# robotseu/ORB_Line_SLAM

Hardware: AMD Instinct MI355X
Metric: stereo frames/s extract+match (ORB+LBD), KITTI 1242x375 (higher is better)
Workload: dtype u8; 1 GPU; C3: 1242x375 stereo, 2000 ORB + 500 LBD per image, extract + stereo point/line match + f2f LBD match + SearchByBoW vs the previous frame (synthetic k=10 L=6 vocabulary, ComputeBoW included); parallelism=frame-sharded x1, distinct_pairs=512, order=shuffled, scene=default

## Files before the change

include/orbline.h:

```cpp
#ifndef ORBLINE_H
#define ORBLINE_H

#include "orbline_types.h"

#ifdef __cplusplus
extern "C" {
#endif

typedef struct olf_ctx olf_ctx;

const char* olf_last_error(void);
int olf_device_count(void);
int olf_default_params(olf_params* p);

int  olf_ctx_create(const olf_params* p, int width, int height, int max_images, olf_ctx** out);
void olf_ctx_destroy(olf_ctx* ctx);
int  olf_ctx_synchronize(olf_ctx* ctx);
int  olf_ctx_set_input_event(olf_ctx* ctx, void* hip_event);
int  olf_ctx_set_deferred_join(olf_ctx* ctx, int on);
int  olf_stereo_frames_join_dev(olf_ctx* ctx, void* stream);
int  olf_ctx_poll_status(olf_ctx* ctx);

int olf_profile_enable(olf_ctx* ctx, int on);
int olf_profile_reset(olf_ctx* ctx);
int olf_profile_stage_count(void);
const char* olf_profile_stage_name(int stage);
int olf_profile_read(olf_ctx* ctx, double* total_ms, int32_t* calls);

enum { OLF_RGB2GRAY = 0, OLF_BGR2GRAY = 1, OLF_RGBA2GRAY = 2, OLF_BGRA2GRAY = 3 };
int olf_cvt_gray_dev(olf_ctx* ctx, const uint8_t* d_src, int code, int n_images, uint8_t* d_gray, void* stream);
int olf_remap_linear_dev(olf_ctx* ctx, const uint8_t* d_src, int src_w, int src_h, const float* d_mapx, const float* d_mapy, int dst_w,
                         int dst_h, int n_images, uint8_t* d_dst, void* stream);
int olf_init_undistort_rectify_map_dev(olf_ctx* ctx, const double* K, const double* D, int n_dist, const double* R, const double* P, int w, int h,
                                       float* d_map1, float* d_map2, void* stream);
int olf_init_undistort_rectify_map(olf_ctx* ctx, const double* K, const double* D, int n_dist, const double* R, const double* P, int w, int h,
                                   float* map1, float* map2);
int olf_cvt_gray(olf_ctx* ctx, const uint8_t* src, int code, int n_images, uint8_t* gray);
int olf_remap_linear(olf_ctx* ctx, const uint8_t* src, int src_w, int src_h, const float* mapx, const float* mapy, int dst_w, int dst_h,
                     int n_images, uint8_t* dst);

int olf_distinctive_descriptors(olf_ctx* ctx, const uint8_t* desc, const int32_t* offs, int n_points, int32_t* best);

size_t olf_kf_record_bytes(int n_keys, int n_lines);
int olf_kf_record_pack(uint64_t frame_id, uint64_t kf_id, double timestamp, const float* t3, const float* quat4, int n_keys,
                       const olf_keypoint* keys, const float* uright, const float* depth, const uint8_t* desc, const uint64_t* mappoint_ids,
                       int n_lines, const olf_keyline* lines, const float* disparity2, const double* le3, const uint8_t* ldesc,
                       const uint64_t* mapline_ids, uint8_t* out, size_t capacity, size_t* written);
int olf_kf_record_counts(const uint8_t* buf, size_t len, int32_t* n_keys, int32_t* n_lines, size_t* record_bytes);
int olf_kf_record_unpack(const uint8_t* buf, size_t len, uint64_t* frame_id, uint64_t* kf_id, double* timestamp, float* t3, float* quat4,
                         olf_keypoint* keys, float* uright, float* depth, uint8_t* desc, uint64_t* mappoint_ids, olf_keyline* lines,
                         float* disparity2, double* le3, uint8_t* ldesc, uint64_t* mapline_ids);

typedef struct olf_voc olf_voc;
int olf_voc_create(int k, int L, int scoring, int weighting, int n_nodes, const int32_t* parent, const uint8_t* is_leaf, const uint8_t* desc,
                   const double* weight, olf_voc** out);
int olf_voc_load_text(const char* path, olf_voc** out);
void olf_voc_destroy(olf_voc* voc);
int olf_voc_info(const olf_voc* voc, int* k, int* L, int* scoring, int* weighting, int* n_nodes, int* n_words);
int olf_bow_words_dev(olf_ctx* ctx, const olf_voc* voc, const uint8_t* d_desc, int n, int levelsup, int32_t* d_word, double* d_weight,
                      int32_t* d_node, void* stream);
int olf_bow_assemble(const olf_voc* voc, const int32_t* word, const double* weight, const int32_t* node, int n, int32_t* bow_ids,
                     double* bow_vals, int* n_bow, int32_t* fv_nodes, int32_t* fv_offs, int32_t* fv_idx, int* n_fv);
int olf_bow_transform(olf_ctx* ctx, const olf_voc* voc, const uint8_t* desc, int n, int levelsup, int32_t* bow_ids, double* bow_vals,
                      int* n_bow, int32_t* fv_nodes, int32_t* fv_offs, int32_t* fv_idx, int* n_fv);
int olf_search_by_bow_batch_dev(olf_ctx* ctx, const olf_voc* voc, int n_frames, int img_stride, const olf_keypoint* d_kps, const uint8_t* d_desc,
                                const int32_t* d_counts, const uint8_t* d_mp_valid, const uint8_t* d_mp_bad, float nnratio, int check_orientation,
                                int levelsup, int32_t* d_matches, int32_t* d_nmatches, void* stream);

int olf_orb_scale_tables(const olf_ctx* ctx, float* scale, float* inv_scale, float* sigma2, float* inv_sigma2,
                         int32_t* features_per_level);
int olf_orb_level_sizes(const olf_ctx* ctx, int32_t* widths, int32_t* heights);
int olf_orb_capacity(const olf_ctx* ctx);
int olf_orb_extract_strided(olf_ctx* ctx, const uint8_t* image, size_t row_stride, olf_keypoint* kps, uint8_t* desc, int32_t* count);
int olf_orb_extract_dev(olf_ctx* ctx, const uint8_t* d_images, int n_images, olf_keypoint* d_kps, uint8_t* d_desc,
                        int32_t* d_counts, void* stream);
int olf_orb_extract(olf_ctx* ctx, const uint8_t* images, int n_images, olf_keypoint* kps, uint8_t* desc, int32_t* counts);
int olf_orb_pyramid_level(olf_ctx* ctx, int image, int level, int blurred, uint8_t* dst);
int olf_orb_debug_candidates(olf_ctx* ctx, int image, int level, int32_t* xys, int cap, int32_t* count);
int olf_debug_status(olf_ctx* ctx, int32_t* out64);
int olf_debug_status_n(olf_ctx* ctx, int32_t* out, int n);
int olf_debug_lsd_owner(olf_ctx* ctx, int image, uint32_t* out);
int olf_debug_lsd_regions(olf_ctx* ctx, int image, int32_t* start_n, double* angle, int cap, int32_t* count);
int olf_debug_lsd_waves(olf_ctx* ctx, int waves_per_image, int rob_entries);
int olf_debug_lsd_groups(olf_ctx* ctx, int groups);
int olf_debug_lsd_scatter(olf_ctx* ctx, int on);
int olf_debug_lsd_log_cap(olf_ctx* ctx, int entries);
int olf_debug_seed_sort(olf_ctx* ctx, const uint32_t* keys, int n, int kthr, int depth_limit, uint32_t* out, int32_t* out_n);
int olf_debug_seed_sort_mode(olf_ctx* ctx, int mode);
int olf_debug_seed_sort_wide(olf_ctx* ctx, const uint64_t* keys, int n, int64_t kthr, int depth_limit, int full, uint32_t* out, int32_t* out_n);
int olf_debug_lsd_pool(olf_ctx* ctx, int pool_chunks);
int olf_debug_fdiv_sweep(olf_ctx* ctx, uint64_t seed, int blocks, int per_thread, uint64_t* mismatches);
int olf_debug_sqrtq_sweep(olf_ctx* ctx, int count, uint64_t* mismatches);
int olf_debug_align_sweep(olf_ctx* ctx, uint64_t seed, int blocks, int per_thread, uint64_t* out3);

int olf_stereo_points_dev(olf_ctx* ctx, int n_pairs, const olf_keypoint* d_kps, const uint8_t* d_desc, const int32_t* d_counts,
                          float* d_uright, float* d_depth, void* stream);
int olf_stereo_points(olf_ctx* ctx, const uint8_t* images, int n_pairs, olf_keypoint* kps, uint8_t* desc, int32_t* counts,
                      float* uright, float* depth);

int olf_match_bf_dev(olf_ctx* ctx, const uint8_t* d_descA, const int32_t* d_nA, int strideA, int a_step, const uint8_t* d_descB,
                     const int32_t* d_nB, int strideB, int b_step, int n_sets, float nnr, int best_lr, int32_t* d_m12, void* stream);
int olf_match_bf(olf_ctx* ctx, const uint8_t* descA, int nA, const uint8_t* descB, int nB, float nnr, int best_lr, int32_t* m12);
int olf_knn2(olf_ctx* ctx, const uint8_t* descQ, int nQ, const uint8_t* descT, int nT, int32_t* idx0, int32_t* dist0, int32_t* dist1);
int olf_match_candidates_dev(olf_ctx* ctx, const uint8_t* d_descQ, int nQ, const uint8_t* d_descT, int nT, const int32_t* d_cand_offsets,
                             const int32_t* d_cand_idx, uint16_t* d_dist, void* stream);
int olf_match_candidates(olf_ctx* ctx, const uint8_t* descQ, int nQ, const uint8_t* descT, int nT, const int32_t* cand_offsets,
                         const int32_t* cand_idx, uint16_t* dist);
typedef struct olf_frame_view {
    const olf_keypoint* keys;
    const uint8_t* desc;
    const float*   uright;
    int32_t        n;
    uint8_t*       mp_valid;
    uint8_t*       mp_obs;
    const uint8_t* mp_bad;
    const float*   mp_world;
    const uint8_t* mp_desc;
    const uint8_t* outlier;
    const float*   Tcw;
    float fx, fy, cx, cy, mbf, minX, maxX, minY, maxY;
    const float*   scale_factors;
    int32_t        n_levels;
    const float*   mp_maxd;
    const float*   mp_mind;
    const int32_t* fv_nodes;
    const int32_t* fv_offsets;
    const int32_t* fv_features;
    int32_t        fv_n;
    const int32_t* grid_offsets;
    const int32_t* grid_index;
} olf_frame_view;
int olf_search_by_projection(olf_ctx* ctx, const olf_frame_view* cur, const olf_frame_view* last, float th, int bMono, int check_orientation,
                             int32_t* matches, int32_t* nmatches);
int olf_search_by_projection_match12(olf_ctx* ctx, const olf_frame_view* cur, const olf_frame_view* last, float th, int bMono, int check_orientation,
                                     int32_t* matches, int32_t* match12, int32_t* nmatches);
int olf_search_for_initialization(olf_ctx* ctx, const olf_frame_view* f1, const olf_frame_view* f2, float* prev_matched, int window_size,
                                  float nnratio, int check_orientation, int32_t* matches12, int32_t* nmatches);
int olf_search_by_bow(olf_ctx* ctx, const olf_frame_view* kf, const olf_frame_view* f, float nnratio, int check_orientation, int32_t* matched,
                      int32_t* nmatches);
int olf_search_local_map(olf_ctx* ctx, const olf_frame_view* f, int n_mp, const uint8_t* track_in_view, const uint8_t* bad,
                         const int32_t* track_scale_level, const float* track_view_cos, const float* track_proj3, const uint8_t* mp_desc,
                         const uint8_t* mp_obs, float th, float nnratio, int32_t* matches, int32_t* nmatches);

int olf_is_in_frustum(const olf_frame_view* f, int n_mp, const float* world, const float* normal, const float* maxd, const float* mind,
                      float viewing_cos_limit, uint8_t* track_in_view, int32_t* track_scale_level, float* track_view_cos, float* track_proj3);

int olf_search_by_projection_kf(olf_ctx* ctx, const olf_frame_view* cur, const olf_frame_view* kf, const uint8_t* already_found, float th,
                                int orb_dist, int check_orientation, int32_t* matches, int32_t* nmatches);
int olf_search_by_bow_kf(olf_ctx* ctx, const olf_frame_view* kf1, const olf_frame_view* kf2, float nnratio, int check_orientation,
                         int32_t* matches12, int32_t* nmatches);
int olf_search_for_triangulation(olf_ctx* ctx, const olf_frame_view* kf1, const olf_frame_view* kf2, const float* F12, const float* Cw,
                                 int only_stereo, int check_orientation, int32_t* matches12, int32_t* nmatches);
int olf_fuse_search(olf_ctx* ctx, const olf_frame_view* kf, int n_mp, const uint8_t* skip, const float* world, const float* normal,
                    const float* maxd, const float* mind, const uint8_t* desc, float th, const float* Ow, int32_t* best_idx, int32_t* best_dist);
int olf_fuse_search_sim3(olf_ctx* ctx, const olf_frame_view* kf, const float* Scw, int n_mp, const uint8_t* skip, const float* world,
                         const float* normal, const float* maxd, const float* mind, const uint8_t* desc, float th, int32_t* best_idx,
                         int32_t* best_dist);
int olf_search_by_projection_sim3(olf_ctx* ctx, const olf_frame_view* kf, const float* Scw, int n_mp, const uint8_t* skip, const float* world,
                                  const float* normal, const float* maxd, const float* mind, const uint8_t* desc, float th, uint8_t* matched,
                                  int32_t* matches, int32_t* nmatches);
int olf_search_by_sim3(olf_ctx* ctx, const olf_frame_view* kf1, const olf_frame_view* kf2, int32_t* matches12, float s12, const float* R12,
                       const float* t12, float th, int32_t* vn_match1, int32_t* vn_match2, int32_t* nfound);

int olf_hamming_matrix(olf_ctx* ctx, const uint8_t* descA, int nA, const uint8_t* descB, int nB, uint16_t* out);

int olf_line_capacity(const olf_ctx* ctx);
int olf_line_extract_strided(olf_ctx* ctx, const uint8_t* image, size_t row_stride, olf_keyline* kls, uint8_t* ldesc, int32_t* lcount);
int olf_line_extract_dev(olf_ctx* ctx, const uint8_t* d_images, int n_images, olf_keyline* d_kls, uint8_t* d_ldesc, int32_t* d_lcounts,
                         void* stream);
int olf_line_extract(olf_ctx* ctx, const uint8_t* images, int n_images, olf_keyline* kls, uint8_t* ldesc, int32_t* lcounts);
int olf_lbd_compute(olf_ctx* ctx, const uint8_t* images, int n_images, const olf_keyline* kls, const int32_t* lcounts, uint8_t* ldesc);
int olf_lsd_debug_scaled(olf_ctx* ctx, int image, uint8_t* dst, int32_t* ws, int32_t* hs);

int olf_stereo_lines_dev(olf_ctx* ctx, int n_pairs, const olf_keyline* d_kls, const uint8_t* d_ldesc, const int32_t* d_lcounts,
                         int32_t* d_matches12, float* d_disp, double* d_le, void* stream);
int olf_stereo_lines(olf_ctx* ctx, int n_pairs, const olf_keyline* kls, const uint8_t* ldesc, const int32_t* lcounts, int32_t* matches12,
                     float* disp, double* le);

typedef struct olf_frame_buffers {
    olf_keypoint* kps;
    uint8_t*  desc;
    int32_t*  counts;
    float*    uright;
    float*    depth;
    olf_keyline* kls;
    uint8_t*  ldesc;
    int32_t*  lcounts;
    int32_t*  lmatches12;
    float*    ldisp;
    double*   lle;
} olf_frame_buffers;
int olf_stereo_frames_dev(olf_ctx* ctx, const uint8_t* d_images, int n_pairs, const olf_frame_buffers* out, void* stream);
int olf_stereo_frames(olf_ctx* ctx, const uint8_t* images, int n_pairs, const olf_frame_buffers* out);

int olf_frame_grid_dev(olf_ctx* ctx, int n_frames, int img_stride, const olf_keypoint* d_kps, const int32_t* d_counts, float minX, float maxX,
                       float minY, float maxY, int32_t* d_cell_offsets, int32_t* d_cell_index, void* stream);
int olf_frame_grid(olf_ctx* ctx, const olf_keypoint* keys, int n, float minX, float maxX, float minY, float maxY, int32_t* cell_offsets,
                   int32_t* cell_index);
int olf_features_in_area_dev(olf_ctx* ctx, const olf_keypoint* d_keys, const int32_t* d_cell_offsets, const int32_t* d_cell_index, float minX, float maxX,
                             float minY, float maxY, int n_queries, const olf_area_query* d_queries, int32_t* d_cand_offsets, int32_t* d_cand_idx,
                             int cand_capacity, void* stream);
int olf_features_in_area(olf_ctx* ctx, const olf_keypoint* keys, int n_keys, const int32_t* cell_offsets, const int32_t* cell_index, float minX,
                         float maxX, float minY, float maxY, int n_queries, const olf_area_query* queries, int32_t* cand_offsets, int32_t* cand_idx,
                         int cand_capacity);
int olf_ctx_device_buffers(const olf_ctx* ctx, olf_frame_buffers* out);

int olf_line_coords(double x1, double y1, double x2, double y2, int32_t* xy, int cap, int32_t* n);

size_t olf_frames_pack_bound(const olf_ctx* ctx, int n_pairs);
int olf_frames_pack_dev(olf_ctx* ctx, const olf_frame_buffers* out, int n_pairs, uint8_t* d_dst, size_t dst_capacity, uint64_t* d_bytes, void* stream);
int olf_stereo_points_mask_dev(olf_ctx* ctx, const float* d_depth, size_t n, uint8_t* d_mask, void* stream);

typedef struct olf_track_batch {
    const olf_keypoint* kps; const uint8_t* desc; const int32_t* counts; int32_t img_stride;
    const float*   uright;
    const int32_t* cell_offsets;
    const int32_t* cell_index;
    const float*   Tcw;
    const float*   mp_world;
    const uint8_t* mp_valid;
    const uint8_t* mp_obs;
    const uint8_t* outlier;
    const uint8_t* mp_desc;
    float fx, fy, cx, cy, mbf, minX, maxX, minY, maxY;
} olf_track_batch;
int olf_search_by_projection_batch_dev(olf_ctx* ctx, const olf_track_batch* in, int n_frames, float th, const float* d_th, int bMono,
                                       int check_orientation, int32_t* d_matches, int32_t* d_match12, int32_t* d_nmatches, void* stream);
int olf_unproject_stereo_dev(olf_ctx* ctx, int n_frames, int img_stride, const olf_keypoint* d_kps, const int32_t* d_counts, const float* d_depth,
                             float fx, float fy, float cx, float cy, const float* d_Twc, float* d_world, void* stream);

typedef struct olf_local_map {
    const float*   world;
    const float*   normal;
    const float*   maxd;
    const float*   mind;
    const uint8_t* desc;
    const uint8_t* obs;
    const uint8_t* bad;
    int32_t        n_mp;
    const int32_t* list_offsets;
    const int32_t* list_index;
    int32_t        n_entries;
} olf_local_map;
int olf_predict_scale_thresholds(const float* scale_factors, int n_levels, float* thr);
int olf_is_in_frustum_batch_dev(olf_ctx* ctx, const olf_track_batch* in, int n_frames, const olf_local_map* map, const int32_t* d_frame_mp,
                                float viewing_cos_limit, uint8_t* d_in_view, int32_t* d_level, float* d_view_cos, float* d_proj3, void* stream);
int olf_search_local_map_batch_dev(olf_ctx* ctx, const olf_track_batch* in, int n_frames, const olf_local_map* map, const int32_t* d_frame_mp,
                                   float viewing_cos_limit, float th, const float* d_th, float nnratio, int32_t* d_matches, int32_t* d_nmatches,
                                   void* stream);

int olf_search_for_triangulation_batch_dev(olf_ctx* ctx, const olf_voc* voc, const olf_track_batch* in, int n_frames, int n_pairs,
                                           const int32_t* d_pairs, const float* d_F12, const float* d_Cw, int only_stereo, int check_orientation,
                                           int levelsup, int32_t* d_matches12, int32_t* d_nmatches, void* stream);

#define OLF_BOW_KF_FRAME 0
#define OLF_BOW_KF_KF    1
int olf_search_by_bow_pairs_dev(olf_ctx* ctx, const olf_voc* voc, const olf_track_batch* in, int n_frames, int n_pairs, const int32_t* d_pairs,
                                const uint8_t* d_mp_bad, int form, float nnratio, int check_orientation, int levelsup,
                                int32_t* d_matches, int32_t* d_nmatches, void* stream);

int olf_fuse_search_batch_dev(olf_ctx* ctx, const olf_track_batch* in, int n_frames, const olf_local_map* map, const int32_t* d_frame_mp,
                              const float* d_Scw, const float* d_Ow, float th, int32_t* d_best_idx, int32_t* d_best_dist, int32_t* d_nfused,
                              void* stream);

int olf_search_by_sim3_pairs_dev(olf_ctx* ctx, const olf_track_batch* in, int n_frames, const uint8_t* d_mp_bad, const float* d_mp_maxd,
                                 const float* d_mp_mind, int n_pairs, const int32_t* d_pairs, const float* d_s12, const float* d_R12, const float* d_t12,
                                 float th, int32_t* d_matches12, int32_t* d_vn_match1, int32_t* d_vn_match2, int32_t* d_nfound, void* stream);

int olf_is_in_frustum_l(const olf_frame_view* f, int n_ml, const float* world6, uint8_t* in_view, float* proj4);
int olf_local_lines_assign(int n_in_view, int32_t* m12, const int32_t* map_index, const float* proj4, const olf_keyline* kls, int n_lines, const float* ldisp,
                           float minX, float maxX, float minY, float maxY, int n_ml, const uint8_t* obs, int32_t* frame_ml, int32_t* n_inliers);
int olf_track_lines_assign(int n_last, int32_t* m12, const olf_keyline* kls_last, const int32_t* last_ml, int n_cur, const olf_keyline* kls_cur,
                           const float* ldisp_cur, float minX, float maxX, float minY, float maxY, int skip_null, int gates, double delta_angle, double pos_frac,
                           int32_t* cur_ml, int32_t* n_inliers);

typedef struct olf_line_batch {
    const olf_keyline* kls; const uint8_t* ldesc; const int32_t* lcounts; int32_t img_stride;
    const float*   ldisp;
    const float*   Tcw;
    float fx, fy, cx, cy, minX, maxX, minY, maxY;
} olf_line_batch;
typedef struct olf_local_line_map {
    const float*   world;
    const uint8_t* desc;
    const uint8_t* obs;
    const uint8_t* bad;
    int32_t        n_ml;
    const int32_t* list_offsets;
    const int32_t* list_index;
    int32_t        n_entries;
} olf_local_line_map;
int olf_is_in_frustum_l_batch_dev(olf_ctx* ctx, const olf_line_batch* in, int n_frames, const olf_local_line_map* map, const int32_t* d_frame_ml,
                                  uint8_t* d_in_view, float* d_proj4, void* stream);
int olf_search_local_lines_batch_dev(olf_ctx* ctx, const olf_line_batch* in, int n_frames, const olf_local_line_map* map, const int32_t* d_frame_ml, float nnr,
                                     uint8_t* d_in_view, float* d_proj4, int32_t* d_m12, int32_t* d_frame_ml_out, int32_t* d_ninliers, void* stream);
int olf_track_lines_batch_dev(olf_ctx* ctx, const olf_line_batch* in, int n_frames, const int32_t* d_last_ml, float nnr, int best_lr, int skip_null, int gates,
                              double delta_angle, double pos_frac, const int32_t* d_enable, int32_t* d_m12, int32_t* d_cur_ml, int32_t* d_ninliers, void* stream);

int olf_debug_copy_bandwidth(olf_ctx* ctx, size_t bytes, int reps, double* gbytes_per_s);

#ifdef __cplusplus
}
#endif
#endif
```

orb_line_slam_amd/_lib.py:

```python
import ctypes as C
import os
import numpy as np

_HERE = os.path.dirname(os.path.abspath(__file__))
LIB_PATH = os.environ.get("OLF_LIB_PATH", os.path.join(_HERE, "csrc", "liborbline_hip.so"))
SYNTH_PATH = os.path.join(_HERE, "csrc", "libolf_synth.so")

OLF_OK, OLF_ERR_INVALID, OLF_ERR_CAPACITY, OLF_ERR_HIP, OLF_ERR_NODEVICE = 0, -1, -2, -3, -4
DESC_BYTES = 32

KEYPOINT_DTYPE = np.dtype([("x", "<f4"), ("y", "<f4"), ("size", "<f4"), ("angle", "<f4"), ("response", "<f4"),
                           ("octave", "<i4"), ("class_id", "<i4")])
KEYLINE_DTYPE = np.dtype([("angle", "<f4"), ("class_id", "<i4"), ("octave", "<i4"), ("pt_x", "<f4"), ("pt_y", "<f4"),
                          ("response", "<f4"), ("size", "<f4"), ("startPointX", "<f4"), ("startPointY", "<f4"),
                          ("endPointX", "<f4"), ("endPointY", "<f4"), ("sPointInOctaveX", "<f4"),
                          ("sPointInOctaveY", "<f4"), ("ePointInOctaveX", "<f4"), ("ePointInOctaveY", "<f4"),
                          ("lineLength", "<f4"), ("numOfPixels", "<i4")])
assert KEYPOINT_DTYPE.itemsize == 28 and KEYLINE_DTYPE.itemsize == 68


class OrbParams(C.Structure):
    _fields_ = [("nfeatures", C.c_int32), ("scale_factor", C.c_float), ("nlevels", C.c_int32),
                ("ini_th_fast", C.c_int32), ("min_th_fast", C.c_int32), ("conv_gauss_sum256", C.c_int32)]


class LineParams(C.Structure):
    _fields_ = [("lsd_nfeatures", C.c_int32), ("min_line_length", C.c_double), ("lsd_refine", C.c_int32),
                ("lsd_scale", C.c_double), ("lsd_sigma_scale", C.c_double), ("lsd_quant", C.c_double),
                ("lsd_ang_th", C.c_double), ("lsd_log_eps", C.c_double), ("lsd_density_th", C.c_double),
                ("lsd_n_bins", C.c_int32), ("conv_gauss_sum256", C.c_int32), ("conv_resize_exact", C.c_int32), ("conv_seed_order", C.c_int32),
                ("conv_libm_float", C.c_int32)]


class StereoParams(C.Structure):
    _fields_ = [("fx", C.c_float), ("bf", C.c_float), ("matching_s_ws", C.c_int32), ("line_sim_th", C.c_double),
                ("min_ratio_12_l", C.c_double), ("min_disp", C.c_double), ("line_horiz_th", C.c_double),
                ("stereo_overlap_th", C.c_double), ("ls_min_disp_ratio", C.c_double), ("best_lr_matches", C.c_int32),
                ("conv_eigen_recip", C.c_int32)]


class OlfParams(C.Structure):
    _fields_ = [("abi_version", C.c_uint32), ("struct_size", C.c_uint32), ("orb", OrbParams), ("line", LineParams), ("stereo", StereoParams)]


class FrameBuffers(C.Structure):
    _fields_ = [(n, C.c_void_p) for n in ("kps", "desc", "counts", "uright", "depth", "kls", "ldesc", "lcounts", "lmatches12",
                                          "ldisp", "lle")]


class FrameViewC(C.Structure):
    _fields_ = ([(n, C.c_void_p) for n in ("keys", "desc", "uright")] + [("n", C.c_int32)] +
                [(n, C.c_void_p) for n in ("mp_valid", "mp_obs", "mp_bad", "mp_world", "mp_desc", "outlier", "Tcw")] +
                [(n, C.c_float) for n in ("fx", "fy", "cx", "cy", "mbf", "minX", "maxX", "minY", "maxY")] +
                [("scale_factors", C.c_void_p), ("n_levels", C.c_int32)] +
                [(n, C.c_void_p) for n in ("mp_maxd", "mp_mind", "fv_nodes", "fv_offsets", "fv_features")] + [("fv_n", C.c_int32)] +
                [(n, C.c_void_p) for n in ("grid_offsets", "grid_index")])


class TrackBatchC(C.Structure):
    _fields_ = ([(n, C.c_void_p) for n in ("kps", "desc", "counts")] + [("img_stride", C.c_int32)] +
                [(n, C.c_void_p) for n in ("uright", "cell_offsets", "cell_index", "Tcw", "mp_world", "mp_valid", "mp_obs", "outlier", "mp_desc")] +
                [(n, C.c_float) for n in ("fx", "fy", "cx", "cy", "mbf", "minX", "maxX", "minY", "maxY")])


class LocalMapC(C.Structure):
    _fields_ = ([(n, C.c_void_p) for n in ("world", "normal", "maxd", "mind", "desc", "obs", "bad")] + [("n_mp", C.c_int32)] +
                [(n, C.c_void_p) for n in ("list_offsets", "list_index")] + [("n_entries", C.c_int32)])


class LineBatchC(C.Structure):
    _fields_ = ([(n, C.c_void_p) for n in ("kls", "ldesc", "lcounts")] + [("img_stride", C.c_int32)] + [(n, C.c_void_p) for n in ("ldisp", "Tcw")] +
                [(n, C.c_float) for n in ("fx", "fy", "cx", "cy", "minX", "maxX", "minY", "maxY")])


class LocalLineMapC(C.Structure):
    _fields_ = ([(n, C.c_void_p) for n in ("world", "desc", "obs", "bad")] + [("n_ml", C.c_int32)] +
                [(n, C.c_void_p) for n in ("list_offsets", "list_index")] + [("n_entries", C.c_int32)])


GRID_COLS, GRID_ROWS, GRID_CELLS, GRID_MAX_KEYS = 64, 48, 3072, 8192
AREA_QUERY_DTYPE = np.dtype([("x", "<f4"), ("y", "<f4"), ("r", "<f4"), ("min_level", "<i4"), ("max_level", "<i4")])
assert AREA_QUERY_DTYPE.itemsize == 20


class OlfError(RuntimeError):
    def __init__(self, code, where):
        self.code = code
        super().__init__(f"{where}: status {code}: {last_error()}")


_lib = None


def _torch_runtime_first():
    import importlib.util
    if os.environ.get("OLF_NO_TORCH") or importlib.util.find_spec("torch") is None:
        return
    try:
        import torch
        if torch.cuda.is_available():
            torch.cuda.init()
    except Exception:
        pass


def lib():
    global _lib
    if _lib is None:
        if not os.path.exists(LIB_PATH):
            raise ImportError(f"{LIB_PATH} is missing: build it with `make -C orb_line_slam_amd/csrc` "
                              "(python -c 'import __graft_entry__ as g; g.build()'). There is no CPU fallback.")
        _torch_runtime_first()
        L = C.CDLL(LIB_PATH)
        L.olf_last_error.restype = C.c_char_p
        L.olf_ctx_create.argtypes = [C.POINTER(OlfParams), C.c_int, C.c_int, C.c_int, C.POINTER(C.c_void_p)]
        L.olf_ctx_destroy.argtypes = [C.c_void_p]
        L.olf_ctx_destroy.restype = None
        L.olf_ctx_synchronize.argtypes = [C.c_void_p]
        L.olf_ctx_poll_status.argtypes = [C.c_void_p]
        L.olf_orb_scale_tables.argtypes = [C.c_void_p] + [C.c_void_p] * 5
        L.olf_orb_level_sizes.argtypes = [C.c_void_p, C.c_void_p, C.c_void_p]
        L.olf_orb_capacity.argtypes = [C.c_void_p]
        L.olf_orb_extract_dev.argtypes = [C.c_void_p, C.c_void_p, C.c_int, C.c_void_p, C.c_void_p, C.c_void_p, C.c_void_p]
        L.olf_orb_extract.argtypes = [C.c_void_p, C.c_void_p, C.c_int, C.c_void_p, C.c_void_p, C.c_void_p]
        L.olf_orb_pyramid_level.argtypes = [C.c_void_p, C.c_int, C.c_int, C.c_int, C.c_void_p]
        L.olf_orb_debug_candidates.argtypes = [C.c_void_p, C.c_int, C.c_int, C.c_void_p, C.c_int, C.c_void_p]
        L.olf_stereo_points_dev.argtypes = [C.c_void_p, C.c_int] + [C.c_void_p] * 6
        L.olf_stereo_points.argtypes = [C.c_void_p, C.c_void_p, C.c_int] + [C.c_void_p] * 5
        L.olf_match_bf_dev.argtypes = [C.c_void_p, C.c_void_p, C.c_void_p, C.c_int, C.c_int, C.c_void_p, C.c_void_p, C.c_int, C.c_int,
                                       C.c_int, C.c_float, C.c_int, C.c_void_p, C.c_void_p]
        L.olf_match_bf.argtypes = [C.c_void_p, C.c_void_p, C.c_int, C.c_void_p, C.c_int, C.c_float, C.c_int, C.c_void_p]
        L.olf_knn2.argtypes = [C.c_void_p, C.c_void_p, C.c_int, C.c_void_p, C.c_int, C.c_void_p, C.c_void_p, C.c_void_p]
        L.olf_hamming_matrix.argtypes = [C.c_void_p, C.c_void_p, C.c_int, C.c_void_p, C.c_int, C.c_void_p]
        L.olf_line_capacity.argtypes = [C.c_void_p]
        L.olf_line_extract_dev.argtypes = [C.c_void_p, C.c_void_p, C.c_int] + [C.c_void_p] * 4
        L.olf_line_extract.argtypes = [C.c_void_p, C.c_void_p, C.c_int] + [C.c_void_p] * 3
        L.olf_lbd_compute.argtypes = [C.c_void_p, C.c_void_p, C.c_int] + [C.c_void_p] * 3
        L.olf_lsd_debug_scaled.argtypes = [C.c_void_p, C.c_int] + [C.c_void_p] * 3
        L.olf_stereo_lines_dev.argtypes = [C.c_void_p, C.c_int] + [C.c_void_p] * 7
        L.olf_stereo_lines.argtypes = [C.c_void_p, C.c_int] + [C.c_void_p] * 6
        L.olf_stereo_frames_dev.argtypes = [C.c_void_p, C.c_void_p, C.c_int, C.POINTER(FrameBuffers), C.c_void_p]
        L.olf_stereo_frames.argtypes = [C.c_void_p, C.c_void_p, C.c_int, C.POINTER(FrameBuffers)]
        L.olf_match_candidates.argtypes = [C.c_void_p, C.c_void_p, C.c_int, C.c_void_p, C.c_int, C.c_void_p, C.c_void_p, C.c_void_p]
        L.olf_search_by_projection.argtypes = [C.c_void_p, C.POINTER(FrameViewC), C.POINTER(FrameViewC), C.c_float, C.c_int, C.c_int, C.c_void_p, C.c_void_p]
        L.olf_search_by_projection_match12.argtypes = [C.c_void_p, C.POINTER(FrameViewC), C.POINTER(FrameViewC), C.c_float, C.c_int, C.c_int, C.c_void_p, C.c_void_p, C.c_void_p]
        L.olf_search_by_bow.argtypes = [C.c_void_p, C.POINTER(FrameViewC), C.POINTER(FrameViewC), C.c_float, C.c_int, C.c_void_p, C.c_void_p]
        L.olf_search_for_initialization.argtypes = [C.c_void_p, C.POINTER(FrameViewC), C.POINTER(FrameViewC), C.c_void_p, C.c_int, C.c_float, C.c_int,
                                                    C.c_void_p, C.c_void_p]
        V = C.POINTER(FrameViewC)
        L.olf_is_in_frustum.argtypes = [V, C.c_int, C.c_void_p, C.c_void_p, C.c_void_p, C.c_void_p, C.c_float] + [C.c_void_p] * 4
        L.olf_search_by_projection_kf.argtypes = [C.c_void_p, V, V, C.c_void_p, C.c_float, C.c_int, C.c_int, C.c_void_p, C.c_void_p]
        L.olf_search_by_bow_kf.argtypes = [C.c_void_p, V, V, C.c_float, C.c_int, C.c_void_p, C.c_void_p]
        L.olf_search_for_triangulation.argtypes = [C.c_void_p, V, V, C.c_void_p, C.c_void_p, C.c_int, C.c_int, C.c_void_p, C.c_void_p]
        L.olf_fuse_search.argtypes = [C.c_void_p, V, C.c_int] + [C.c_void_p] * 6 + [C.c_float, C.c_void_p, C.c_void_p, C.c_void_p]
        L.olf_fuse_search_sim3.argtypes = [C.c_void_p, V, C.c_void_p, C.c_int] + [C.c_void_p] * 6 + [C.c_float, C.c_void_p, C.c_void_p]
        L.olf_search_by_projection_sim3.argtypes = [C.c_void_p, V, C.c_void_p, C.c_int] + [C.c_void_p] * 6 + [C.c_float, C.c_void_p, C.c_void_p, C.c_void_p]
        L.olf_search_by_sim3.argtypes = [C.c_void_p, V, V, C.c_void_p, C.c_float, C.c_void_p, C.c_void_p, C.c_float, C.c_void_p, C.c_void_p, C.c_void_p]
        L.olf_search_local_map.argtypes = [C.c_void_p, C.POINTER(FrameViewC), C.c_int, C.c_void_p, C.c_void_p, C.c_void_p, C.c_void_p, C.c_void_p,
                                           C.c_void_p, C.c_void_p, C.c_float, C.c_float, C.c_void_p, C.c_void_p]
        L.olf_match_candidates_dev.argtypes = [C.c_void_p, C.c_void_p, C.c_int, C.c_void_p, C.c_int, C.c_void_p, C.c_void_p, C.c_void_p, C.c_void_p]
        L.olf_frame_grid_dev.argtypes = [C.c_void_p, C.c_int, C.c_int, C.c_void_p, C.c_void_p] + [C.c_float] * 4 + [C.c_void_p] * 3
        L.olf_frame_grid.argtypes = [C.c_void_p, C.c_void_p, C.c_int] + [C.c_float] * 4 + [C.c_void_p] * 2
        L.olf_features_in_area_dev.argtypes = ([C.c_void_p] * 4 + [C.c_float] * 4 + [C.c_int, C.c_void_p, C.c_void_p, C.c_void_p, C.c_int, C.c_void_p])
        L.olf_features_in_area.argtypes = ([C.c_void_p, C.c_void_p, C.c_int, C.c_void_p, C.c_void_p] + [C.c_float] * 4 +
                                           [C.c_int, C.c_void_p, C.c_void_p, C.c_void_p, C.c_int])
        L.olf_ctx_device_buffers.argtypes = [C.c_void_p, C.POINTER(FrameBuffers)]
        L.olf_cvt_gray.argtypes = [C.c_void_p, C.c_void_p, C.c_int, C.c_int, C.c_void_p]
        L.olf_remap_linear.argtypes = [C.c_void_p, C.c_void_p, C.c_int, C.c_int, C.c_void_p, C.c_void_p, C.c_int, C.c_int, C.c_int, C.c_void_p]
        L.olf_debug_lsd_waves.argtypes = [C.c_void_p, C.c_int, C.c_int]
        L.olf_debug_lsd_pool.argtypes = [C.c_void_p, C.c_int]
        L.olf_debug_lsd_groups.argtypes = [C.c_void_p, C.c_int]
        L.olf_debug_lsd_scatter.argtypes = [C.c_void_p, C.c_int]
        L.olf_debug_lsd_log_cap.argtypes = [C.c_void_p, C.c_int]
        L.olf_debug_seed_sort_mode.argtypes = [C.c_void_p, C.c_int]
        L.olf_debug_seed_sort.argtypes = [C.c_void_p, C.c_void_p, C.c_int, C.c_int, C.c_int, C.c_void_p, C.POINTER(C.c_int32)]
        L.olf_frames_pack_bound.argtypes = [C.c_void_p, C.c_int]
        L.olf_frames_pack_bound.restype = C.c_size_t
        L.olf_frames_pack_dev.argtypes = [C.c_void_p, C.POINTER(FrameBuffers), C.c_int, C.c_void_p, C.c_size_t, C.c_void_p, C.c_void_p]
        L.olf_ctx_set_input_event.argtypes = [C.c_void_p, C.c_void_p]
        L.olf_ctx_set_deferred_join.argtypes = [C.c_void_p, C.c_int]
        L.olf_stereo_frames_join_dev.argtypes = [C.c_void_p, C.c_void_p]
        L.olf_stereo_points_mask_dev.argtypes = [C.c_void_p, C.c_void_p, C.c_size_t, C.c_void_p, C.c_void_p]
        L.olf_search_by_projection_batch_dev.argtypes = [C.c_void_p, C.POINTER(TrackBatchC), C.c_int, C.c_float, C.c_void_p, C.c_int, C.c_int,
                                                         C.c_void_p, C.c_void_p, C.c_void_p, C.c_void_p]
        L.olf_unproject_stereo_dev.argtypes = [C.c_void_p, C.c_int, C.c_int, C.c_void_p, C.c_void_p, C.c_void_p] + [C.c_float] * 4 + [C.c_void_p] * 3
        L.olf_predict_scale_thresholds.argtypes = [C.c_void_p, C.c_int, C.c_void_p]
        L.olf_is_in_frustum_batch_dev.argtypes = [C.c_void_p, C.POINTER(TrackBatchC), C.c_int, C.POINTER(LocalMapC), C.c_void_p, C.c_float] + [C.c_void_p] * 5
        L.olf_search_local_map_batch_dev.argtypes = [C.c_void_p, C.POINTER(TrackBatchC), C.c_int, C.POINTER(LocalMapC), C.c_void_p, C.c_float, C.c_float,
                                                     C.c_void_p, C.c_float, C.c_void_p, C.c_void_p, C.c_void_p]
        L.olf_is_in_frustum_l.argtypes = [V, C.c_int, C.c_void_p, C.c_void_p, C.c_void_p]
        L.olf_local_lines_assign.argtypes = ([C.c_int, C.c_void_p, C.c_void_p, C.c_void_p, C.c_void_p, C.c_int, C.c_void_p] + [C.c_float] * 4 +
                                             [C.c_int, C.c_void_p, C.c_void_p, C.c_void_p])
        L.olf_track_lines_assign.argtypes = ([C.c_int, C.c_void_p, C.c_void_p, C.c_void_p, C.c_int, C.c_void_p, C.c_void_p] + [C.c_float] * 4 +
                                             [C.c_int, C.c_int, C.c_double, C.c_double, C.c_void_p, C.c_void_p])
        L.olf_is_in_frustum_l_batch_dev.argtypes = [C.c_void_p, C.POINTER(LineBatchC), C.c_int, C.POINTER(LocalLineMapC)] + [C.c_void_p] * 4
        L.olf_search_local_lines_batch_dev.argtypes = [C.c_void_p, C.POINTER(LineBatchC), C.c_int, C.POINTER(LocalLineMapC), C.c_void_p, C.c_float] + [C.c_void_p] * 6
        L.olf_track_lines_batch_dev.argtypes = ([C.c_void_p, C.POINTER(LineBatchC), C.c_int, C.c_void_p, C.c_float, C.c_int, C.c_int, C.c_int, C.c_double, C.c_double] +
                                                [C.c_void_p] * 5)
        L.olf_debug_copy_bandwidth.argtypes =[C.c_void_p, C.c_size_t, C.c_int, C.POINTER(C.c_double)]
        L.olf_debug_fdiv_sweep.argtypes = [C.c_void_p, C.c_uint64, C.c_int, C.c_int, C.POINTER(C.c_uint64)]
        L.olf_debug_sqrtq_sweep.argtypes = [C.c_void_p, C.c_int, C.POINTER(C.c_uint64)]
        L.olf_debug_align_sweep.argtypes = [C.c_void_p, C.c_uint64, C.c_int, C.c_int, C.POINTER(C.c_uint64)]
        L.olf_debug_seed_sort_wide.argtypes = [C.c_void_p, C.c_void_p, C.c_int, C.c_int64, C.c_int, C.c_int, C.c_void_p, C.POINTER(C.c_int32)]
        L.olf_distinctive_descriptors.argtypes = [C.c_void_p, C.c_void_p, C.c_void_p, C.c_int, C.c_void_p]
        L.olf_voc_create.argtypes = [C.c_int, C.c_int, C.c_int, C.c_int, C.c_int, C.c_void_p, C.c_void_p, C.c_void_p, C.c_void_p, C.POINTER(C.c_void_p)]
        L.olf_voc_load_text.argtypes = [C.c_char_p, C.POINTER(C.c_void_p)]
        L.olf_voc_destroy.argtypes = [C.c_void_p]
        L.olf_voc_destroy.restype = None
        L.olf_voc_info.argtypes = [C.c_void_p] + [C.POINTER(C.c_int)] * 6
        L.olf_bow_words_dev.argtypes = [C.c_void_p, C.c_void_p, C.c_void_p, C.c_int, C.c_int, C.c_void_p, C.c_void_p, C.c_void_p, C.c_void_p]
        L.olf_bow_assemble.argtypes = [C.c_void_p, C.c_void_p, C.c_void_p, C.c_void_p, C.c_int, C.c_void_p, C.c_void_p, C.POINTER(C.c_int), C.c_void_p,
                                       C.c_void_p, C.c_void_p, C.POINTER(C.c_int)]
        L.olf_search_by_bow_batch_dev.argtypes = [C.c_void_p, C.c_void_p, C.c_int, C.c_int, C.c_void_p, C.c_void_p, C.c_void_p, C.c_void_p, C.c_void_p, C.c_float, C.c_int, C.c_int, C.c_void_p, C.c_void_p, C.c_void_p]
        L.olf_search_for_triangulation_batch_dev.argtypes = ([C.c_void_p, C.c_void_p, C.POINTER(TrackBatchC), C.c_int, C.c_int] + [C.c_void_p] * 3 + [C.c_int] * 3 +
                                                             [C.c_void_p] * 3)
        L.olf_search_by_bow_pairs_dev.argtypes = ([C.c_void_p, C.c_void_p, C.POINTER(TrackBatchC), C.c_int, C.c_int, C.c_void_p, C.c_void_p, C.c_int, C.c_float,
                                                   C.c_int, C.c_int] + [C.c_void_p] * 3)
        L.olf_fuse_search_batch_dev.argtypes = ([C.c_void_p, C.POINTER(TrackBatchC), C.c_int, C.POINTER(LocalMapC)] + [C.c_void_p] * 3 + [C.c_float] +
                                                [C.c_void_p] * 4)
        L.olf_search_by_sim3_pairs_dev.argtypes = ([C.c_void_p, C.POINTER(TrackBatchC), C.c_int] + [C.c_void_p] * 3 + [C.c_int] + [C.c_void_p] * 4 + [C.c_float] +
                                                   [C.c_void_p] * 5)
        L.olf_bow_transform.argtypes = [C.c_void_p, C.c_void_p, C.c_void_p, C.c_int, C.c_int, C.c_void_p, C.c_void_p, C.POINTER(C.c_int), C.c_void_p,
                                        C.c_void_p, C.c_void_p, C.POINTER(C.c_int)]
        L.olf_profile_enable.argtypes = [C.c_void_p, C.c_int]
        L.olf_profile_reset.argtypes = [C.c_void_p]
        L.olf_profile_stage_name.restype = C.c_char_p
        L.olf_profile_stage_name.argtypes = [C.c_int]
        L.olf_profile_read.argtypes = [C.c_void_p, C.c_void_p, C.c_void_p]
        _lib = L
    return _lib


def last_error():
    return lib().olf_last_error().decode()


def device_count():
    return int(lib().olf_device_count())


def default_params():
    p = OlfParams()
    rc = lib().olf_default_params(C.byref(p))
    if rc != OLF_OK:
        raise OlfError(rc, "olf_default_params")
    return p


def check(rc, where):
    if rc != OLF_OK:
        raise OlfError(rc, where)


def ptr(a):
    if a is None:
        return None
    assert a.flags["C_CONTIGUOUS"]
    return a.ctypes.data_as(C.c_void_p)


class Context:

    def __init__(self, params, width, height, max_images):
        self.params, self.width, self.height, self.max_images = params, int(width), int(height), int(max_images)
        h = C.c_void_p()
        check(lib().olf_ctx_create(C.byref(params), self.width, self.height, self.max_images, C.byref(h)), "olf_ctx_create")
        self.handle = h
        self.nlevels = params.orb.nlevels
        self.orb_capacity = int(lib().olf_orb_capacity(self.handle))
        self.line_capacity = int(lib().olf_line_capacity(self.handle))

    def close(self):
        if getattr(self, "handle", None):
            lib().olf_ctx_destroy(self.handle)
            self.handle = None

    def __del__(self):
        try:
            self.close()
        except Exception:
            pass

    def profile(self, on=True):
        check(lib().olf_profile_enable(self.handle, int(on)), "olf_profile_enable")
        check(lib().olf_profile_reset(self.handle), "olf_profile_reset")

    def profile_read(self):
        n = lib().olf_profile_stage_count()
        ms = np.zeros(n, np.float64)
        calls = np.zeros(n, np.int32)
        check(lib().olf_profile_read(self.handle, ptr(ms), ptr(calls)), "olf_profile_read")
        return {lib().olf_profile_stage_name(i).decode(): (float(ms[i]), int(calls[i])) for i in range(n)}

    def synchronize(self):
        check(lib().olf_ctx_synchronize(self.handle), "olf_ctx_synchronize")

    def set_input_event(self, event):
        check(lib().olf_ctx_set_input_event(self.handle, C.c_void_p(event.cuda_event) if event is not None else None), "olf_ctx_set_input_event")

    def poll_status(self):
        check(lib().olf_ctx_poll_status(self.handle), "olf_ctx_poll_status")
```

orb_line_slam_amd/csrc/api_debug.cpp:

```cpp
#include "ctx.hpp"
#include "staging.hpp"

namespace olf {
int launch_copy16(const void* src, void* dst, size_t bytes, hipStream_t s);
}

using namespace olf;

static int sweep_counters(HostCall& h, unsigned long long** st, int n)
{
    h.add(st, n);
    OLF_TRY(h.bind(SCRATCH_STAGE));
    OLF_HIP_CHECK(hipMemsetAsync(*st, 0, (size_t)n * 8, h.stream()));
    return OLF_OK;
}

extern "C" {

int olf_orb_pyramid_level(olf_ctx* c, int image, int level, int blurred, uint8_t* dst)
{
    if (!c || !dst || image < 0 || image >= c->max_images || level < 0 || level >= c->orb.geom.nlevels) return OLF_ERR_INVALID;
    const LevelGeom& L = c->orb.geom.lv[level];
    const uint8_t* src = (blurred ? c->ob.blur : c->ob.pyr) + (size_t)image * c->orb.geom.pyrBytes + L.offset;
    OLF_HIP_CHECK(hipStreamSynchronize(c->stream));
    OLF_HIP_CHECK(hipMemcpy2D(dst, L.w, src, L.pitch, L.w, L.h, hipMemcpyDeviceToHost));
    return OLF_OK;
}

int olf_debug_status(olf_ctx* c, int32_t* out64)
{
    if (!c || !out64) return OLF_ERR_INVALID;
    OLF_HIP_CHECK(hipDeviceSynchronize());
    OLF_HIP_CHECK(hipMemcpy(out64, c->ob.status, 256, hipMemcpyDeviceToHost));
    return OLF_OK;
}

int olf_debug_copy_bandwidth(olf_ctx* c, size_t bytes, int reps, double* gbytes_per_s)
{
    if (!c || !gbytes_per_s || bytes < 16 || reps < 1) { set_error("olf_debug_copy_bandwidth: bad argument"); return OLF_ERR_INVALID; }
    OLF_TRY(check_device(c, "olf_debug_copy_bandwidth"));
    void *a = nullptr, *b = nullptr;
    OLF_HIP_CHECK(hipMalloc(&a, bytes));
    if (hipMalloc(&b, bytes) != hipSuccess) { (void)hipFree(a); set_error("olf_debug_copy_bandwidth: hipMalloc failed"); return OLF_ERR_HIP; }
    hipEvent_t e0, e1;
    (void)hipEventCreate(&e0); (void)hipEventCreate(&e1);
    (void)hipMemsetAsync(a, 1, bytes, c->stream);
    int rc = olf::launch_copy16(a, b, bytes, c->stream);
    (void)hipEventRecord(e0, c->stream);
    for (int i = 0; i < reps && rc == OLF_OK; ++i) rc = olf::launch_copy16(i & 1 ? b : a, i & 1 ? a : b, bytes, c->stream);
    (void)hipEventRecord(e1, c->stream);
    const hipError_t se = hipEventSynchronize(e1);
    float ms = 0.f;
    (void)hipEventElapsedTime(&ms, e0, e1);
    (void)hipEventDestroy(e0); (void)hipEventDestroy(e1); (void)hipFree(a); (void)hipFree(b);
    if (rc != OLF_OK || se != hipSuccess || !(ms > 0)) { set_error("olf_debug_copy_bandwidth: copy failed"); return OLF_ERR_HIP; }
    *gbytes_per_s = 2.0 * (double)(bytes / 16 * 16) * reps / (ms * 1e-3) / 1e9;
    return OLF_OK;
}

int olf_debug_lsd_waves(olf_ctx* c, int waves_per_image, int rob_entries)
{
    const bool pow2 = rob_entries > 0 && (rob_entries & (rob_entries - 1)) == 0;
    if (!c || waves_per_image > 16 || waves_per_image < -1 || (rob_entries != 0 && (!pow2 || rob_entries < 128 || rob_entries > 1024))) {
        set_error("olf_debug_lsd_waves: bad argument"); return OLF_ERR_INVALID;
    }
    c->lsd_force.waves = waves_per_image;
    c->lsd_force.robEntries = rob_entries;
    return OLF_OK;
}

int olf_debug_lsd_groups(olf_ctx* c, int groups)
{
    if (!c || !(groups == 0 || groups == 1 || groups == 2 || groups == 4)) { set_error("olf_debug_lsd_groups: bad argument"); return OLF_ERR_INVALID; }
    c->lsd_force.groups = groups > 0 ? groups : -1;
    return OLF_OK;
}

int olf_debug_lsd_log_cap(olf_ctx* c, int entries)
{
    if (!c || entries < 0) { set_error("olf_debug_lsd_log_cap: bad argument"); return OLF_ERR_INVALID; }
    OLF_TRY(check_device(c, "olf_debug_lsd_log_cap"));
    LineGeom& g = c->line.geom;
    if (entries > 0 && !g.spillArena) {
        const size_t blocks = std::max<size_t>(2, (size_t)c->max_images - (size_t)c->max_images / 4);
        void* q = nullptr;
        OLF_HIP_CHECK(hipMalloc(&q, blocks * 8 * (size_t)g.Ps));
        c->allocs.push_back(q);
        g.spillArena = static_cast<uint32_t*>(q); g.spillBlocks = (int)blocks;
    }
    g.logCap = entries > 0 ? std::min(entries, g.regionStride / 2) : g.regionStride / 2;
    OLF_HIP_CHECK(hipDeviceSynchronize());
    OLF_HIP_CHECK(hipMemcpy(c->lb.geom, &g, sizeof(LineGeom), hipMemcpyHostToDevice));
    return OLF_OK;
}

int olf_debug_lsd_scatter(olf_ctx* c, int on)
{
    if (!c) { set_error("olf_debug_lsd_scatter: bad argument"); return OLF_ERR_INVALID; }
    c->lsd_force.scatter = on ? 1 : 0;
    return OLF_OK;
}

int olf_debug_seed_sort(olf_ctx* c, const uint32_t* keys, int n, int kthr, int depth_limit, uint32_t* out, int32_t* out_n)
{
    if (!c || !keys || !out || !out_n || n < 0 || n > c->line.geom.Ps || kthr < 0 || kthr > 1023) { set_error("olf_debug_seed_sort: bad argument"); return OLF_ERR_INVALID; }
    HostCall h(c, "olf_debug_seed_sort");
    OLF_TRY(h.begin());
    OLF_TRY(h.up(c->lb.keysA, keys, (size_t)n * 4));
    OLF_TRY(launch_lsd_seedsort(c->line.geom, c->lb, lsd_plan(c->line.geom, c->lb, c->lsd_force, c->limits, 1), 1, h.stream(), n, kthr, depth_limit));
    OLF_TRY(h.down_counted(out_n, c->lb.keyCount, 1, out, c->lb.keysB, n, out_n));
    OLF_TRY(h.finish());
    if (*out_n < 0 || *out_n > n) { set_error("olf_debug_seed_sort: count out of range"); return OLF_ERR_HIP; }
    return OLF_OK;
}

int olf_debug_seed_sort_wide(olf_ctx* c, const uint64_t* keys, int n, int64_t kthr, int depth_limit, int full, uint32_t* out, int32_t* out_n)
{
    if (!c || !keys || !out || !out_n || n < 0 || n > c->line.geom.Ps || kthr < 0 || kthr > 0xffffffffll || !c->line.geom.wide) {
        set_error("olf_debug_seed_sort_wide: bad argument (the context must be a wide one: lsd_n_bins > 1024 or 2^22 pixels and more)"); return OLF_ERR_INVALID; }
    HostCall h(c, "olf_debug_seed_sort_wide");
    OLF_TRY(h.begin());
    OLF_TRY(h.up(c->lb.keysA, keys, (size_t)n * 8));
    OLF_TRY(launch_lsd_sort_wide(c->line.geom, c->lb, 1, h.stream(), n, (long long)kthr, depth_limit, full ? 1 : 0));
    OLF_TRY(h.down_counted(out_n, c->lb.keyCount, 1, out, c->lb.keysB, n, out_n));
    OLF_TRY(h.finish());
    if (*out_n < 0 || *out_n > n) { set_error("olf_debug_seed_sort_wide: count out of range"); return OLF_ERR_HIP; }
    return check_status(c);
}

int olf_debug_seed_sort_mode(olf_ctx* c, int mode)
{
    if (!c || mode < -1 || mode == 3 || mode == 4 || mode > 5) { set_error("olf_debug_seed_sort_mode: bad argument"); return OLF_ERR_INVALID; }
    c->lsd_force.sortMode = mode;
    return OLF_OK;
}

int olf_debug_lsd_pool(olf_ctx* c, int pool_chunks)
{
    if (!c || pool_chunks < 0) { set_error("olf_debug_lsd_pool: bad argument"); return OLF_ERR_INVALID; }
    c->lsd_force.poolChunks = pool_chunks;
    return OLF_OK;
}

int olf_debug_lsd_regions(olf_ctx* c, int image, int32_t* start_n , double* angle, int cap, int32_t* count)
{
    if (!c || !start_n || !angle || !count || image < 0 || image >= c->max_images) return OLF_ERR_INVALID;
    OLF_HIP_CHECK(hipDeviceSynchronize());
    int nr = 0;
    OLF_HIP_CHECK(hipMemcpy(&nr, c->lb.regCount + image, sizeof(int), hipMemcpyDeviceToHost));
    *count = nr;
    struct Rec { int start, n; double angle; };
    std::vector<Rec> r((size_t)std::min(nr, cap));
    if (!r.empty())
        OLF_HIP_CHECK(hipMemcpy(r.data(), reinterpret_cast<const Rec*>(c->lb.keysA) + (size_t)image * c->line.geom.maxRegions, r.size() * sizeof(Rec), hipMemcpyDeviceToHost));
    for (size_t i = 0; i < r.size(); ++i) { start_n[2 * i] = r[i].start; start_n[2 * i + 1] = r[i].n; angle[i] = r[i].angle; }
    return OLF_OK;
}

int olf_debug_lsd_owner(olf_ctx* c, int image, uint32_t* out)
{
    if (!c || !out || image < 0 || image >= c->lb.ownerImages) return OLF_ERR_INVALID;
    OLF_HIP_CHECK(hipDeviceSynchronize());
    OLF_HIP_CHECK(hipMemcpy(out, c->lb.owner + (size_t)image * c->line.geom.Ps, (size_t)c->line.geom.Ps * 4, hipMemcpyDeviceToHost));
    return OLF_OK;
}

int olf_debug_status_n(olf_ctx* c, int32_t* out, int n)
{
    if (!c || !out || n < 1 || n > 256) return OLF_ERR_INVALID;
    OLF_HIP_CHECK(hipDeviceSynchronize());
    OLF_HIP_CHECK(hipMemcpy(out, c->ob.status, (size_t)n * 4, hipMemcpyDeviceToHost));
    return OLF_OK;
}

int olf_debug_fdiv_sweep(olf_ctx* c, uint64_t seed, int blocks, int per_thread, uint64_t* mismatches)
{
    if (!c || !mismatches || blocks < 1 || per_thread < 1) { set_error("olf_debug_fdiv_sweep: bad argument"); return OLF_ERR_INVALID; }
    HostCall h(c, "olf_debug_fdiv_sweep");
    unsigned long long* st;
    OLF_TRY(sweep_counters(h, &st, 1));
    OLF_TRY(launch_fdiv_sweep((unsigned long long)seed, blocks, per_thread, st, h.stream()));
    OLF_TRY(h.down(mismatches, st, 8));
    return h.finish();
}

int olf_debug_sqrtq_sweep(olf_ctx* c, int count, uint64_t* mismatches)
{
    if (!c || !mismatches || count < 1) { set_error("olf_debug_sqrtq_sweep: bad argument"); return OLF_ERR_INVALID; }
    HostCall h(c, "olf_debug_sqrtq_sweep");
    unsigned long long* st;
    OLF_TRY(sweep_counters(h, &st, 1));
    OLF_TRY(launch_sqrtq_sweep(count, st, h.stream()));
    OLF_TRY(h.down(mismatches, st, 8));
    return h.finish();
}

int olf_debug_align_sweep(olf_ctx* c, uint64_t seed, int blocks, int per_thread, uint64_t* out3)
{
    if (!c || !out3 || blocks < 1 || per_thread < 1) { set_error("olf_debug_align_sweep: bad argument"); return OLF_ERR_INVALID; }
    if (c->line.geom.alignTanLo < 0.f) { set_error("olf_debug_align_sweep: the cheap alignment test is off for lsd_ang_th > 80 degrees"); return OLF_ERR_INVALID; }
    HostCall h(c, "olf_debug_align_sweep");
    unsigned long long* st;
    OLF_TRY(sweep_counters(h, &st, 3));
    OLF_TRY(launch_align_sweep(c->lb, (unsigned long long)seed, blocks, per_thread, st, h.stream()));
    OLF_TRY(h.down(out3, st, 24));
    return h.finish();
}

int olf_orb_debug_candidates(olf_ctx* c, int image, int level, int32_t* xys, int cap, int32_t* count)
{
    if (!c || !xys || !count || image < 0 || image >= c->max_images || level < 0 || level >= c->orb.geom.nlevels) return OLF_ERR_INVALID;
    const OrbGeom& g = c->orb.geom;
    OLF_HIP_CHECK(hipStreamSynchronize(c->stream));
    int n = 0;
    OLF_HIP_CHECK(hipMemcpy(&n, c->ob.candCount + image * g.nlevels + level, sizeof(int), hipMemcpyDeviceToHost));
    *count = n;
    std::vector<uint32_t> tmp(std::max(n, 1));
    OLF_HIP_CHECK(hipMemcpy(tmp.data(), c->ob.cand + (size_t)image * g.candTotal + g.lv[level].candBase, n * sizeof(uint32_t), hipMemcpyDeviceToHost));
    for (int i = 0; i < std::min(n, cap); ++i) {
        xys[3 * i] = tmp[i] >> 20; xys[3 * i + 1] = (tmp[i] >> 8) & 0xfff; xys[3 * i + 2] = tmp[i] & 0xff;
    }
    return OLF_OK;
}

int olf_lsd_debug_scaled(olf_ctx* c, int image, uint8_t* dst, int32_t* ws, int32_t* hs)
{
    if (!c || !dst || image < 0 || image >= c->max_images) return OLF_ERR_INVALID;
    if (c->scaled_aliased) { set_error("olf_lsd_debug_scaled: a batch context does not keep the enlarged image (use a context of at most 2048 images)"); return OLF_ERR_INVALID; }
    const LineGeom& g = c->line.geom;
    OLF_HIP_CHECK(hipDeviceSynchronize());
    OLF_HIP_CHECK(hipMemcpy2D(dst, g.Ws, c->lb.scaled + (size_t)image * g.pitchS * g.Hs, g.pitchS, g.Ws, g.Hs, hipMemcpyDeviceToHost));
    if (ws) *ws = g.Ws;
    if (hs) *hs = g.Hs;
    return OLF_OK;
}

}
```

orb_line_slam_amd/csrc/filters.hip:

```cpp
#include "olf_internal.hpp"
#include <algorithm>

namespace olf {

constexpr int SF_TW = 128, SF_TH = 32;
constexpr int SF_INW = (SF_TW + 8) / 4;
constexpr int SF_INH = SF_TH + 6;

__device__ __forceinline__ int sf_reflect(int p, int n)
{
    if (p < 0) p = -p;
    if (p >= n) p = 2 * (n - 1) - p;
    return p;
}

__global__ __launch_bounds__(256) void k_sep7(const uint8_t* __restrict__ src, size_t srcImgStride, int srcPitch, uint8_t* __restrict__ dst,
                                              size_t dstImgStride, int dstPitch, int W, int H, Taps7 taps)
{
    __shared__ uint32_t s_in[SF_INH * SF_INW];
    constexpr int HS = (SF_INH + 1) / 2 + ((((SF_INH + 1) / 2) & 1) ? 0 : 1);
    __shared__ uint32_t s_h[SF_TW * HS];
    const int img = blockIdx.z, x0 = blockIdx.x * SF_TW, y0 = blockIdx.y * SF_TH;
    const uint8_t* s = src + (size_t)img * srcImgStride;
    const bool plain = x0 >= 4 && x0 + SF_TW + 4 <= W && y0 >= 3 && y0 + SF_TH + 3 <= H && ((srcPitch | (int)srcImgStride) & 3) == 0 &&
                       (reinterpret_cast<uintptr_t>(src) & 3) == 0;
    const uint8_t* tile = s + (ptrdiff_t)(y0 - 3) * srcPitch + (x0 - 4);
    for (int i = threadIdx.x; i < SF_INH * SF_INW; i += 256) {
        const int r = i / SF_INW, j = i - r * SF_INW;
        uint32_t v;
        if (plain) v = *reinterpret_cast<const uint32_t*>(tile + (size_t)r * srcPitch + 4 * j);
        else {
            const int gy = sf_reflect(min(y0 - 3 + r, H + 2), H);
            const int xw = x0 - 4 + 4 * j;
            const uint8_t* row = s + (size_t)gy * srcPitch;
            const uintptr_t addr = reinterpret_cast<uintptr_t>(row + xw);
            const int sh = (int)(addr & 3) * 8;
            if (xw >= 0 && (sh ? xw + 7 < W : xw + 3 < W)) {
                const uint32_t* p4 = reinterpret_cast<const uint32_t*>(row + xw - (int)(addr & 3));
                v = sh ? __funnelshift_r(p4[0], p4[1], sh) : p4[0];
            } else {
                v = 0;
#pragma unroll
                for (int b = 0; b < 4; ++b) v |= (uint32_t)row[sf_reflect(min(xw + b, W + 2), W)] << (8 * b);
            }
        }
        s_in[i] = v;
    }
    __syncthreads();
    const uint32_t tlo = (uint32_t)taps.t[0] | ((uint32_t)taps.t[1] << 8) | ((uint32_t)taps.t[2] << 16) | ((uint32_t)taps.t[3] << 24);
    const uint32_t thi = (uint32_t)taps.t[4] | ((uint32_t)taps.t[5] << 8) | ((uint32_t)taps.t[6] << 16);
    uint16_t* s_h16 = reinterpret_cast<uint16_t*>(s_h);
    for (int i = threadIdx.x; i < SF_INH * (SF_TW / 4); i += 256) {
        const int r = i / (SF_TW / 4), q = i - r * (SF_TW / 4);
        const uint32_t w0 = s_in[r * SF_INW + q], w1 = s_in[r * SF_INW + q + 1], w2 = s_in[r * SF_INW + q + 2];
        const uint32_t o0 = __builtin_amdgcn_udot4(__builtin_amdgcn_alignbyte(w2, w1, 1u), thi, __builtin_amdgcn_udot4(__builtin_amdgcn_alignbyte(w1, w0, 1u), tlo, 0u, false), false);
        const uint32_t o1 = __builtin_amdgcn_udot4(__builtin_amdgcn_alignbyte(w2, w1, 2u), thi, __builtin_amdgcn_udot4(__builtin_amdgcn_alignbyte(w1, w0, 2u), tlo, 0u, false), false);
        const uint32_t o2 = __builtin_amdgcn_udot4(__builtin_amdgcn_alignbyte(w2, w1, 3u), thi, __builtin_amdgcn_udot4(__builtin_amdgcn_alignbyte(w1, w0, 3u), tlo, 0u, false), false);
        const uint32_t o3 = __builtin_amdgcn_udot4(w2, thi, __builtin_amdgcn_udot4(w1, tlo, 0u, false), false);
        uint16_t* col = s_h16 + (size_t)(4 * q) * (2 * HS) + r;
        col[0] = (uint16_t)o0; col[2 * HS] = (uint16_t)o1; col[4 * HS] = (uint16_t)o2; col[6 * HS] = (uint16_t)o3;
    }
    __syncthreads();
    const int q = threadIdx.x & 31, ry0 = (threadIdx.x >> 5) * 4;
    const int gx = x0 + 4 * q;
    if (gx >= W) return;
    const uint32_t t01 = (uint32_t)taps.t[0] | ((uint32_t)taps.t[1] << 16), t23 = (uint32_t)taps.t[2] | ((uint32_t)taps.t[3] << 16);
    const uint32_t t45 = (uint32_t)taps.t[4] | ((uint32_t)taps.t[5] << 16), t6lo = (uint32_t)taps.t[6], t6hi = (uint32_t)taps.t[6] << 16;
    typedef unsigned short us2 __attribute__((ext_vector_type(2)));
    auto dot2 = [](uint32_t a, uint32_t b, uint32_t c) -> uint32_t {
        us2 va, vb;
        __builtin_memcpy(&va, &a, 4); __builtin_memcpy(&vb, &b, 4);
        return __builtin_amdgcn_udot2(va, vb, c, false);
    };
    uint32_t res[4][4];
#pragma unroll
    for (int c = 0; c < 4; ++c) {
        const uint32_t* hp = s_h + (size_t)(4 * q + c) * HS + (ry0 >> 1);
        const uint32_t D0 = hp[0], D1 = hp[1], D2 = hp[2], D3 = hp[3], D4 = hp[4];
        const uint32_t E0 = __builtin_amdgcn_alignbyte(D1, D0, 2u), E1 = __builtin_amdgcn_alignbyte(D2, D1, 2u);
        const uint32_t E2 = __builtin_amdgcn_alignbyte(D3, D2, 2u), E3 = __builtin_amdgcn_alignbyte(D4, D3, 2u);
        res[0][c] = dot2(D3, t6lo, dot2(D2, t45, dot2(D1, t23, dot2(D0, t01, 32768u))));
        res[1][c] = dot2(D3, t6hi, dot2(E2, t45, dot2(E1, t23, dot2(E0, t01, 32768u))));
        res[2][c] = dot2(D4, t6lo, dot2(D3, t45, dot2(D2, t23, dot2(D1, t01, 32768u))));
        res[3][c] = dot2(D4, t6hi, dot2(E3, t45, dot2(E2, t23, dot2(E1, t01, 32768u))));
    }
    uint8_t* d = dst + (size_t)img * dstImgStride;
#pragma unroll
    for (int rr = 0; rr < 4; ++rr) {
        const int gy = y0 + ry0 + rr;
        if (gy >= H) break;
        const uint32_t a0 = min(res[rr][0] >> 16, 255u), a1 = min(res[rr][1] >> 16, 255u), a2 = min(res[rr][2] >> 16, 255u), a3 = min(res[rr][3] >> 16, 255u);
        uint8_t* o = d + (size_t)gy * dstPitch + gx;
        if (gx + 3 < W && ((reinterpret_cast<uintptr_t>(o) & 3) == 0))
            *reinterpret_cast<uint32_t*>(o) = a0 | (a1 << 8) | (a2 << 16) | (a3 << 24);
        else {
            o[0] = (uint8_t)a0;
            if (gx + 1 < W) o[1] = (uint8_t)a1;
            if (gx + 2 < W) o[2] = (uint8_t)a2;
            if (gx + 3 < W) o[3] = (uint8_t)a3;
        }
    }
}

constexpr int SS_ROWS = 16;
constexpr int SS_BROWS = 8;

__device__ __forceinline__ int ss_reflect(int p, int n) { p = p < 0 ? -p : p; return p >= n ? 2 * (n - 1) - p : p; }

template <bool BORDER, int ROWS>
__device__ __forceinline__ void sep7_strip_body(const int t, const uint8_t* __restrict__ src, size_t srcImgStride, int srcPitch, uint8_t* __restrict__ dst,
                                                size_t dstImgStride, int dstPitch, int W, int H, const Taps7& taps, int nsx, int nsy)
{
    const int nb = BORDER ? 1 + ((W + 3) / 4 - (nsx + 1)) : nsx;
    if (t >= nb * nsy) return;
    const int sy = t / nb, si = t - sy * nb;
    const int sx = BORDER ? (si == 0 ? 0 : nsx + si) : si + 1;
    const int x0 = 4 * sx, y0 = sy * ROWS;
    const uint8_t* s = src + (size_t)blockIdx.y * srcImgStride + (x0 - 4);
    uint8_t* d = dst + (size_t)blockIdx.y * dstImgStride + x0;
    const uint32_t tlo = (uint32_t)taps.t[0] | ((uint32_t)taps.t[1] << 8) | ((uint32_t)taps.t[2] << 16) | ((uint32_t)taps.t[3] << 24);
    const uint32_t thi = (uint32_t)taps.t[4] | ((uint32_t)taps.t[5] << 8) | ((uint32_t)taps.t[6] << 16);
    const uint32_t t01 = (uint32_t)taps.t[0] | ((uint32_t)taps.t[1] << 16), t23 = (uint32_t)taps.t[2] | ((uint32_t)taps.t[3] << 16);
    const uint32_t t45 = (uint32_t)taps.t[4] | ((uint32_t)taps.t[5] << 16), t6lo = (uint32_t)taps.t[6], t6hi = (uint32_t)taps.t[6] << 16;
    typedef unsigned short us2 __attribute__((ext_vector_type(2)));
    auto dot2 = [](uint32_t a, uint32_t b, uint32_t c) -> uint32_t {
        us2 va, vb;
        __builtin_memcpy(&va, &a, 4); __builtin_memcpy(&vb, &b, 4);
        return __builtin_amdgcn_udot2(va, vb, c, false);
    };
    struct Raw { uint32_t w[3]; };
    auto load_row = [&](int y) -> Raw {
        Raw r;
        const uint8_t* row = s + (size_t)ss_reflect(min(y, H + 2), H) * srcPitch;
        if (!BORDER) __builtin_memcpy(r.w, row, 12);
        else {
#pragma unroll
            for (int k = 0; k < 3; ++k) {
                uint32_t v = 0;
#pragma unroll
                for (int b = 0; b < 4; ++b) {
                    const int x = x0 - 4 + 4 * k + b;
                    v |= (uint32_t)row[ss_reflect(min(x, W + 2), W) - (x0 - 4)] << (8 * b);
                }
                r.w[k] = v;
            }
        }
        return r;
    };
    auto hrow = [&](const Raw& r, uint32_t* o) {
        const uint32_t* w = r.w;
        o[0] = __builtin_amdgcn_udot4(__builtin_amdgcn_alignbyte(w[2], w[1], 1u), thi, __builtin_amdgcn_udot4(__builtin_amdgcn_alignbyte(w[1], w[0], 1u), tlo, 0u, false), false);
        o[1] = __builtin_amdgcn_udot4(__builtin_amdgcn_alignbyte(w[2], w[1], 2u), thi, __builtin_amdgcn_udot4(__builtin_amdgcn_alignbyte(w[1], w[0], 2u), tlo, 0u, false), false);
        o[2] = __builtin_amdgcn_udot4(__builtin_amdgcn_alignbyte(w[2], w[1], 3u), thi, __builtin_amdgcn_udot4(__builtin_amdgcn_alignbyte(w[1], w[0], 3u), tlo, 0u, false), false);
        o[3] = __builtin_amdgcn_udot4(w[2], thi, __builtin_amdgcn_udot4(w[1], tlo, 0u, false), false);
    };
    auto pair = [&](const Raw& ra, const Raw& rb, uint32_t* Pj) {
        uint32_t a[4], b[4];
        hrow(ra, a); hrow(rb, b);
#pragma unroll
        for (int c = 0; c < 4; ++c) Pj[c] = a[c] | (b[c] << 16);
    };
    uint32_t P[ROWS / 2 + 3][4];
    Raw nx[4];
    {
        Raw r0 = load_row(y0 - 3), r1 = load_row(y0 - 2), r2 = load_row(y0 - 1), r3 = load_row(y0), r4 = load_row(y0 + 1), r5 = load_row(y0 + 2);
#pragma unroll
        for (int k = 0; k < 4; ++k) nx[k] = load_row(y0 + 3 + k);
        pair(r0, r1, P[0]); pair(r2, r3, P[1]); pair(r4, r5, P[2]);
    }
#pragma unroll
    for (int g = 0; g < ROWS / 4; ++g) {
        const Raw c0 = nx[0], c1 = nx[1], c2 = nx[2], c3 = nx[3];
        if (g + 1 < ROWS / 4) {
#pragma unroll
            for (int k = 0; k < 4; ++k) nx[k] = load_row(y0 + 4 * (g + 1) + 3 + k);
            __builtin_amdgcn_sched_barrier(0);
        }
        pair(c0, c1, P[2 * g + 3]); pair(c2, c3, P[2 * g + 4]);
        uint32_t res[4][4];
#pragma unroll
        for (int c = 0; c < 4; ++c) {
            const uint32_t D0 = P[2 * g][c], D1 = P[2 * g + 1][c], D2 = P[2 * g + 2][c], D3 = P[2 * g + 3][c], D4 = P[2 * g + 4][c];
            const uint32_t E0 = __builtin_amdgcn_alignbyte(D1, D0, 2u), E1 = __builtin_amdgcn_alignbyte(D2, D1, 2u);
            const uint32_t E2 = __builtin_amdgcn_alignbyte(D3, D2, 2u), E3 = __builtin_amdgcn_alignbyte(D4, D3, 2u);
            res[0][c] = dot2(D3, t6lo, dot2(D2, t45, dot2(D1, t23, dot2(D0, t01, 32768u))));
            res[1][c] = dot2(D3, t6hi, dot2(E2, t45, dot2(E1, t23, dot2(E0, t01, 32768u))));
            res[2][c] = dot2(D4, t6lo, dot2(D3, t45, dot2(D2, t23, dot2(D1, t01, 32768u))));
            res[3][c] = dot2(D4, t6hi, dot2(E3, t45, dot2(E2, t23, dot2(E1, t01, 32768u))));
        }
#pragma unroll
        for (int rr = 0; rr < 4; ++rr) {
            const int gy = y0 + 4 * g + rr;
            if (gy < H) {
                const uint32_t a0 = min(res[rr][0] >> 16, 255u), a1 = min(res[rr][1] >> 16, 255u), a2 = min(res[rr][2] >> 16, 255u), a3 = min(res[rr][3] >> 16, 255u);
                const uint32_t v = a0 | (a1 << 8) | (a2 << 16) | (a3 << 24);
                if (!BORDER) __builtin_memcpy(d + (size_t)gy * dstPitch, &v, 4);
                else {
#pragma unroll
                    for (int b = 0; b < 4; ++b) if (x0 + b < W) d[(size_t)gy * dstPitch + b] = (uint8_t)(v >> (8 * b));
                }
            }
        }
    }
}

template <bool BORDER>
__global__ __launch_bounds__(256) void k_sep7_strip(const uint8_t* __restrict__ src, size_t srcImgStride, int srcPitch, uint8_t* __restrict__ dst,
                                                    size_t dstImgStride, int dstPitch, int W, int H, Taps7 taps, int nsx, int nsy)
{
    sep7_strip_body<BORDER, BORDER ? SS_BROWS : SS_ROWS>(blockIdx.x * 256 + threadIdx.x, src, srcImgStride, srcPitch, dst, dstImgStride, dstPitch, W, H, taps, nsx, nsy);
}

int launch_sep7(const uint8_t* src, size_t srcImgStride, int srcPitch, uint8_t* dst, size_t dstImgStride, int dstPitch, int W, int H,
                const int* taps7, int n_images, hipStream_t s)
{
    Taps7 t;
    for (int i = 0; i < 7; ++i) t.t[i] = taps7[i];
    if (t.t[3] == 256) {
        for (int i = 0; i < n_images; ++i)
            OLF_HIP_CHECK(hipMemcpy2DAsync(dst + (size_t)i * dstImgStride, dstPitch, src + (size_t)i * srcImgStride, srcPitch, W, H, hipMemcpyDeviceToDevice, s));
        return OLF_OK;
    }
    for (int i = 0; i < 7; ++i)
        if (t.t[i] < 0 || t.t[i] > 255) { set_error("launch_sep7: taps must be 8-bit fractions"); return OLF_ERR_INVALID; }
    if (W >= 16 && H >= 8 && (dstPitch & 3) == 0 && (dstImgStride & 3) == 0 && (reinterpret_cast<uintptr_t>(dst) & 3) == 0) {
        const int nsx = (W - 7) / 4, nsy = (H + SS_ROWS - 1) / SS_ROWS, nb = 1 + ((W + 3) / 4 - (nsx + 1));
        const int nsyB = (H + SS_BROWS - 1) / SS_BROWS;
        hipLaunchKernelGGL(k_sep7_strip<false>, dim3((nsx * nsy + 255) / 256, n_images), dim3(256), 0, s, src, srcImgStride, srcPitch, dst, dstImgStride, dstPitch, W, H, t, nsx, nsy);
        hipLaunchKernelGGL(k_sep7_strip<true>, dim3((nb * nsyB + 255) / 256, n_images), dim3(256), 0, s, src, srcImgStride, srcPitch, dst, dstImgStride, dstPitch, W, H, t, nsx, nsyB);
        OLF_HIP_CHECK(hipGetLastError());
        return OLF_OK;
    }
    hipLaunchKernelGGL(k_sep7, dim3((W + SF_TW - 1) / SF_TW, (H + SF_TH - 1) / SF_TH, n_images), dim3(256), 0, s, src, srcImgStride, srcPitch,
                       dst, dstImgStride, dstPitch, W, H, t);
    OLF_HIP_CHECK(hipGetLastError());
    return OLF_OK;
}

struct TapsWide { int r; int t[15]; };
__global__ __launch_bounds__(256) void k_sep_wide(const uint8_t* __restrict__ src, size_t srcImgStride, int srcPitch, uint8_t* __restrict__ dst,
                                                  size_t dstImgStride, int dstPitch, int W, int H, TapsWide taps)
{
    constexpr int TW = 64, TH = 16, RMAX = 7;
    __shared__ uint32_t s_h[TH + 2 * RMAX][TW];
    const int r = taps.r, n = 2 * r + 1;
    const int x0 = blockIdx.x * TW, y0 = blockIdx.y * TH;
    const uint8_t* in = src + (size_t)blockIdx.z * srcImgStride;
    uint8_t* out = dst + (size_t)blockIdx.z * dstImgStride;
    for (int i = threadIdx.x; i < (TH + 2 * r) * TW; i += 256) {
        const int ry = i / TW, cx = i - ry * TW, x = x0 + cx;
        int yy = y0 - r + ry;
        if (yy < 0) yy = -yy;
        if (yy >= H) yy = 2 * (H - 1) - yy;
        int acc = 0;
        if (x < W && yy >= 0 && yy < H) {
            const uint8_t* row = in + (size_t)yy * srcPitch;
            for (int k = 0; k < n; ++k) {
                int xx = x + k - r;
                if (xx < 0) xx = -xx;
                if (xx >= W) xx = 2 * (W - 1) - xx;
                acc += taps.t[k] * (int)row[xx];
            }
        }
        s_h[ry][cx] = (uint32_t)acc;
    }
    __syncthreads();
    for (int i = threadIdx.x; i < TH * TW; i += 256) {
        const int ty = i / TW, cx = i - ty * TW, x = x0 + cx, y = y0 + ty;
        if (x >= W || y >= H) continue;
        int acc = 0;
        for (int k = 0; k < n; ++k) acc += taps.t[k] * (int)s_h[ty + k][cx];
        const int v = (acc + 32768) >> 16;
        out[(size_t)y * dstPitch + x] = (uint8_t)(v > 255 ? 255 : v);
    }
}

int launch_sep_wide(const uint8_t* src, size_t srcImgStride, int srcPitch, uint8_t* dst, size_t dstImgStride, int dstPitch, int W, int H,
                    const int* taps, int r, int n_images, hipStream_t s)
{
    if (r < 1 || r > 7 || 2 * r >= W || 2 * r >= H) { set_error("launch_sep_wide: radius"); return OLF_ERR_INVALID; }
    TapsWide t; t.r = r;
    for (int i = 0; i < 15; ++i) t.t[i] = i < 2 * r + 1 ? taps[i] : 0;
    hipLaunchKernelGGL(k_sep_wide, dim3((W + 63) / 64, (H + 15) / 16, n_images), dim3(256), 0, s, src, srcImgStride, srcPitch, dst, dstImgStride,
                       dstPitch, W, H, t);
    OLF_HIP_CHECK(hipGetLastError());
    return OLF_OK;
}

constexpr int RZ_TW = 256, RZ_TH = 8, RZ_SW = 96 , RZ_SH = 16;

__global__ __launch_bounds__(256) void k_resize_tiled(const uint8_t* __restrict__ src, size_t srcImgStride, int srcPitch, int sw, int sh,
                                                      uint8_t* __restrict__ dst, size_t dstImgStride, int dstPitch, int dw, int dh,
                                                      const ResizeCoef* __restrict__ rx, const ResizeCoef* __restrict__ ry)
{
    __shared__ uint32_t s_src[RZ_SH * RZ_SW];
    __shared__ uint16_t s_h[RZ_SH * RZ_TW];
    __shared__ ResizeCoef s_rx[RZ_TW];
    const int img = blockIdx.z, dx0 = blockIdx.x * RZ_TW, dy0 = blockIdx.y * RZ_TH;
    const int nx = min(RZ_TW, dw - dx0), ny = min(RZ_TH, dh - dy0);
    const uint8_t* s = src + (size_t)img * srcImgStride;
    const int ry0 = min(max((int)ry[dy0].ofs, 0), sh - 1), ry1 = min(max((int)ry[dy0 + ny - 1].ofs + 1, 0), sh - 1);
    const int cx0 = ((int)rx[dx0].ofs) & ~3;
    const int cx1 = min((int)rx[dx0 + nx - 1].ofs + 1, sw - 1);
    const int nrows = ry1 - ry0 + 1, nwords = (cx1 - cx0) / 4 + 1;
    if (threadIdx.x < nx) s_rx[threadIdx.x] = rx[dx0 + threadIdx.x];
    for (int i = threadIdx.x; i < nrows * nwords; i += 256) {
        const int r = i / nwords, j = i - r * nwords;
        s_src[r * RZ_SW + j] = *reinterpret_cast<const uint32_t*>(s + (size_t)(ry0 + r) * srcPitch + cx0 + 4 * j);
    }
    __syncthreads();
    const uint8_t* sb = reinterpret_cast<const uint8_t*>(s_src);
    if ((int)threadIdx.x < nx) {
        const int x = threadIdx.x;
        const ResizeCoef c = s_rx[x];
        const int o0 = (int)c.ofs - cx0, o1 = min((int)c.ofs + 1, sw - 1) - cx0;
        const int a0 = c.a0, a1 = c.a1;
        for (int r = 0; r < nrows; ++r) {
            const int h = (int)sb[r * RZ_SW * 4 + o0] * a0 + (int)sb[r * RZ_SW * 4 + o1] * a1;
            s_h[r * RZ_TW + x] = (uint16_t)(h >> 4);
        }
    }
    __syncthreads();
    uint8_t* d = dst + (size_t)img * dstImgStride;
    for (int i = threadIdx.x; i < ny * (RZ_TW / 4); i += 256) {
        const int yy = i >> 6, q = i & 63;
        if (4 * q >= nx) continue;
        const ResizeCoef cy = ry[dy0 + yy];
        const int r0 = min(max((int)cy.ofs, 0), sh - 1) - ry0, r1 = min(max((int)cy.ofs + 1, 0), sh - 1) - ry0;
        const int b0 = cy.a0, b1 = cy.a1;
        uint32_t out = 0;
#pragma unroll
        for (int k = 0; k < 4; ++k) {
            const int h0 = s_h[r0 * RZ_TW + 4 * q + k], h1 = s_h[r1 * RZ_TW + 4 * q + k];
            const int v = (((b0 * h0) >> 16) + ((b1 * h1) >> 16) + 2) >> 2;
            out |= (uint32_t)(v & 0xff) << (8 * k);
        }
        *reinterpret_cast<uint32_t*>(d + (size_t)(dy0 + yy) * dstPitch + dx0 + 4 * q) = out;
    }
}

constexpr int RS_ROWS = 8;

__global__ __launch_bounds__(64) void k_resize_strip(const uint8_t* __restrict__ src, size_t srcImgStride, int srcPitch, int sw, int sh,
                                                     uint8_t* __restrict__ dst, size_t dstImgStride, int dstPitch, int dw, int dh,
                                                     const ResizeCoef* __restrict__ rx, const ResizeCoef* __restrict__ ry, int nsx)
{
    const int q = blockIdx.x * 64 + threadIdx.x;
    if (q >= nsx) return;
    const int dx0 = 4 * q, dy0 = blockIdx.y * RS_ROWS;
    const uint8_t* s = src + (size_t)blockIdx.z * srcImgStride;
    uint8_t* d = dst + (size_t)blockIdx.z * dstImgStride + dx0;
    typedef unsigned short us2 __attribute__((ext_vector_type(2)));
    uint32_t sel[4], coef[4];
    const int base = min((int)rx[dx0].ofs, srcPitch - 8);
#pragma unroll
    for (int k = 0; k < 4; ++k) {
        const ResizeCoef c = rx[min(dx0 + k, dw - 1)];
        const int o0 = (int)c.ofs - base, o1 = min((int)c.ofs + 1, sw - 1) - base;
        sel[k] = (uint32_t)o0 | 0x0c00u | ((uint32_t)o1 << 16) | 0x0c000000u;
        coef[k] = (uint32_t)(uint16_t)c.a0 | ((uint32_t)(uint16_t)c.a1 << 16);
    }
    struct Raw { uint32_t w[2]; };
    auto load_row = [&](int r) -> Raw { Raw v; __builtin_memcpy(v.w, s + (size_t)r * srcPitch + base, 8); return v; };
    auto hrow = [&](const Raw& v, uint32_t* h) {
#pragma unroll
        for (int k = 0; k < 4; ++k) {
            const uint32_t pr = __builtin_amdgcn_perm(v.w[1], v.w[0], sel[k]);
            us2 va, vb;
            __builtin_memcpy(&va, &pr, 4); __builtin_memcpy(&vb, &coef[k], 4);
            h[k] = __builtin_amdgcn_udot2(va, vb, 0u, false) >> 4;
        }
    };
    auto rows_of = [&](int dy, int& r0, int& r1, uint32_t& b0, uint32_t& b1) {
        const ResizeCoef cy = ry[min(dy, dh - 1)];
        r0 = min(max((int)cy.ofs, 0), sh - 1); r1 = min(max((int)cy.ofs + 1, 0), sh - 1);
        b0 = (uint32_t)cy.a0; b1 = (uint32_t)cy.a1;
    };
    int r0, r1, ra = -1, rb = -1;
    uint32_t b0, b1;
    rows_of(dy0, r0, r1, b0, b1);
    Raw p0 = load_row(r0), p1 = load_row(r1);
    uint32_t hA[4] = {0, 0, 0, 0}, hB[4] = {0, 0, 0, 0};
#pragma unroll
    for (int rr = 0; rr < RS_ROWS; ++rr) {
        const int dy = dy0 + rr;
        if (dy >= dh) break;
        int n0, n1;
        uint32_t c0, c1;
        rows_of(dy + 1, n0, n1, c0, c1);
        Raw q0 = p0, q1 = p1;
        if (rr + 1 < RS_ROWS) {
            if (n0 != r0 && n0 != r1) q0 = load_row(n0);
            if (n1 != n0 && n1 != r1) q1 = load_row(n1);
            __builtin_amdgcn_sched_barrier(0);
        }
        uint32_t h0[4], h1[4];
        if (r0 == ra) { for (int k = 0; k < 4; ++k) h0[k] = hA[k]; }
        else if (r0 == rb) { for (int k = 0; k < 4; ++k) h0[k] = hB[k]; }
        else hrow(p0, h0);
        if (r1 == r0) { for (int k = 0; k < 4; ++k) h1[k] = h0[k]; }
        else if (r1 == rb) { for (int k = 0; k < 4; ++k) h1[k] = hB[k]; }
        else hrow(p1, h1);
        uint32_t out = 0;
#pragma unroll
        for (int k = 0; k < 4; ++k) {
            const uint32_t v = (((b0 * h0[k]) >> 16) + ((b1 * h1[k]) >> 16) + 2u) >> 2;
            out |= (v & 0xffu) << (8 * k);
        }
        __builtin_memcpy(d + (size_t)dy * dstPitch, &out, 4);
        ra = r0; rb = r1;
#pragma unroll
        for (int k = 0; k < 4; ++k) { hA[k] = h0[k]; hB[k] = h1[k]; }
        r0 = n0; r1 = n1; b0 = c0; b1 = c1; p0 = q0; p1 = q1;
    }
}

bool resize_strip_fits(const ResizeCoef* rx, int sw, int dw, int ncols)
{
    for (int x0 = 0; x0 < dw; x0 += 4) {
        const int last = std::min(x0 + ncols - 1, dw - 1);
        if (std::min((int)rx[last].ofs + 1, sw - 1) - (int)rx[x0].ofs > 7) return false;
    }
    return sw >= 8;
}

bool resize_tiled_fits(const ResizeCoef* rx, const ResizeCoef* ry, int sw, int sh, int dw, int dh)
{
    for (int x0 = 0; x0 < dw; x0 += RZ_TW) {
        const int nx = std::min(RZ_TW, dw - x0);
        const int c0 = ((int)rx[x0].ofs) & ~3, c1 = std::min((int)rx[x0 + nx - 1].ofs + 1, sw - 1);
        if ((c1 - c0) / 4 + 1 > RZ_SW) return false;
    }
    for (int y0 = 0; y0 < dh; y0 += RZ_TH) {
        const int ny = std::min(RZ_TH, dh - y0);
        const int r0 = std::min(std::max((int)ry[y0].ofs, 0), sh - 1), r1 = std::min(std::max((int)ry[y0 + ny - 1].ofs + 1, 0), sh - 1);
        if (r1 - r0 + 1 > RZ_SH) return false;
    }
    return true;
}

int launch_resize_tiled(const uint8_t* src, size_t srcImgStride, int srcPitch, int sw, int sh, uint8_t* dst, size_t dstImgStride, int dstPitch,
                        int dw, int dh, const ResizeCoef* d_rx, const ResizeCoef* d_ry, int n_images, hipStream_t s, bool strip)
{
    strip = strip && (dstPitch & 3) == 0 && (dstImgStride & 3) == 0 && srcPitch >= 8;
    if (strip) {
        const int nsx = (dw + 3) / 4;
        hipLaunchKernelGGL(k_resize_strip, dim3((nsx + 63) / 64, (dh + RS_ROWS - 1) / RS_ROWS, n_images), dim3(64), 0, s, src, srcImgStride, srcPitch, sw, sh,
                           dst, dstImgStride, dstPitch, dw, dh, d_rx, d_ry, nsx);
        OLF_HIP_CHECK(hipGetLastError());
        return OLF_OK;
    }
    hipLaunchKernelGGL(k_resize_tiled, dim3((dw + RZ_TW - 1) / RZ_TW, (dh + RZ_TH - 1) / RZ_TH, n_images), dim3(256), 0, s, src, srcImgStride,
                       srcPitch, sw, sh, dst, dstImgStride, dstPitch, dw, dh, d_rx, d_ry);
    OLF_HIP_CHECK(hipGetLastError());
    return OLF_OK;
}

}
```

orb_line_slam_amd/csrc/line_internal.hpp:

```cpp
#pragma once
#include "olf_internal.hpp"

namespace olf {

struct LineGeom {
    int W, H, pitchW;
    int Ws, Hs, pitchS, Ps;
    int nThr;
    int nBins;
    int wide;
    int minRegSize;
    double prec;
    double precWrap;
    double scale;
    double minLength;
    int maxDetect;
    int rectGrid;
    int maxRegions;
    int nFeatures;
    int outCap;
    int pitchD;
    int lsdTaps[7];
    int lsdWideR;
    int lsdWide[15];
    int lbdTaps[7];
    float gaussCoefL[21];
    float gaussCoefG[63];
    int resizeTabX, resizeTabY;
    int resizeTiled;
    int seedOrder;
    int refine;
    double densityTh;
    double logNT, logEps, pProb;
    int libmFloat;
    uint32_t divWsM; int divWsS;
    float alignTanLo, alignTanHi;
    float alignDeg;
    int regionStride;
    int resizeExact;
    int logCap;
    int spillBlocks;
    uint32_t* spillArena;
    int* spillCtl;
    int* spillOf;
};

struct LineDeviceBufs {
    uint8_t* lsdBlur = nullptr;
    uint8_t* scaled = nullptr;
    uint32_t* grad = nullptr;
    uint32_t* keysA = nullptr;
    uint32_t* keysB = nullptr;
    int* keyCount = nullptr;
    int* maxN = nullptr;
    int* chunkCnt = nullptr;
    uint32_t* region = nullptr;
    olf_keyline* rawLines = nullptr;
    int* rawCount = nullptr;
    int* regCount = nullptr;
    uint8_t* lbdBlur = nullptr;
    uint32_t* dxdy = nullptr;
    float* rowSums = nullptr;
    float* lbdStarts = nullptr;
    ResizeCoef* rx = nullptr;
    ResizeCoef* ry = nullptr;
    LineGeom* geom = nullptr;
    uint32_t* sortHist = nullptr;
    uint32_t* sortBase = nullptr;
    int* status = nullptr;
    float* angDeg = nullptr;
    void* angEnt = nullptr;
    int ownerImages = 0;
    uint32_t* owner = nullptr;
    int* links = nullptr;
    int nChunks = 0;
    int* growFmt = nullptr;
    int* topBuf = nullptr;
    unsigned char* mg = nullptr;
    size_t mgStride = 0;
    int mgImages = 0;
};

struct LsdOverrides {
    int sortMode = -1;
    int waves = -1, robEntries = 0;
    int groups = -1;
    int poolChunks = 0;
    int scatter = 0;
};

struct DeviceLimits { int nCU = 64, maxLds = 64 * 1024; };

struct LsdPlan {
    enum Resize { Upgrad, Tiled, Upsample } resize;
    enum Sort { Radix, Seed, Wide } sort;
    bool keysOwner, keysAll;
    int sortWaves;
    bool sortTop; int sortGroups;
    int growWaves;
    int robEntries, growGroups, poolChunks, scatter;
    int agentRefine, agentPF, agentLaunches;
    enum Rect { Emit, Mixed, Plain } rect;
};
LsdPlan lsd_plan(const LineGeom& g, const LineDeviceBufs& b, const LsdOverrides& o, const DeviceLimits& d, int n_images);

constexpr int kBatchCtxImages = 2048;

struct LineHostTables {
    LineGeom geom;
    std::vector<ResizeCoef> rx, ry;
    int build(const olf_line_params& p, int W, int H, int max_images = 2);
};

int launch_lsd_dense(const LineGeom& g, const LineDeviceBufs& b, const LsdPlan& p, const uint8_t* d_in, int in_pitch, int n_images, hipStream_t s, bool writeScaled);
int launch_lsd_seed_order(const LineGeom& g, const LineDeviceBufs& b, const LsdPlan& p, int n_images, hipStream_t s);
int launch_lsd_grow(const LineGeom& g, const LineDeviceBufs& b, const LsdPlan& p, int n_images, hipStream_t s);
int launch_lsd_rect(const LineGeom& g, const LineDeviceBufs& b, const LsdPlan& p, int n_images, hipStream_t s);
int launch_line_select(const LineGeom& g, const LineDeviceBufs& b, int n_images, olf_keyline* d_kls, int* d_counts, hipStream_t s);
int launch_lbd_dense(const LineGeom& g, const LineDeviceBufs& b, const uint8_t* d_in, int in_pitch, int n_images, hipStream_t s);
int launch_lbd_desc(const LineGeom& g, const LineDeviceBufs& b, int n_images, const olf_keyline* d_kls, uint8_t* d_desc, const int* d_counts, hipStream_t s);
int launch_gauss7_img(const uint8_t* src, int srcPitch, size_t srcStride, uint8_t* dst, int dstPitch, size_t dstStride, int W, int H,
                      const LineGeom& g, int which, int n_images, hipStream_t s);
int launch_lsd_angle_table(LineDeviceBufs& b, int libmFloat, hipStream_t s);
int launch_fdiv_sweep(unsigned long long seed, int blocks, int per_thread, unsigned long long* d_mismatches, hipStream_t s);
int launch_sqrtq_sweep(int count, unsigned long long* d_mismatches, hipStream_t s);
int launch_align_sweep(const LineDeviceBufs& b, unsigned long long seed, int blocks, int per_thread, unsigned long long* d_out, hipStream_t s);
int lsd_sort_max_chunks(int Ps);
size_t lsd_grow_mg_stride(int maxRegions);
constexpr int kMwMaxImages = 3072;
constexpr int kMgMaxImages = 64;
int launch_lsd_grow_mw(const LineGeom& g, const LineDeviceBufs& b, const LsdPlan& p, int n_images, hipStream_t s);
int lsd_seedsort_top_words();
int launch_lsd_sort(const LineGeom& g, const LineDeviceBufs& b, int n_images, hipStream_t s);
int launch_lsd_seedsort(const LineGeom& g, const LineDeviceBufs& b, const LsdPlan& p, int n_images, hipStream_t s, int nOverride, int kthrOverride, int depthOverride);
int launch_lsd_sort_wide(const LineGeom& g, const LineDeviceBufs& b, int n_images, hipStream_t s, int nOverride, long long kthrOverride, int depthOverride, int fullOverride);

size_t stereo_lines_prep_bytes(int n_images, int cap);
int launch_stereo_lines(int W, int H, const olf_stereo_params& P, int n_pairs, const olf_keyline* d_kls, const uint8_t* d_desc,
                        const int* d_counts, int cap, void* d_prep, uint16_t* d_dist , int* d_m21, int* d_m12,
                        float* d_disp, double* d_le, hipStream_t s);

}
```

orb_line_slam_amd/csrc/lsd.hip:

```cpp
#include "lsd_device.hpp"

namespace olf {


__device__ __forceinline__ int refl101(int p, int n)
{
    if (p < 0) p = -p;
    if (p >= n) p = 2 * (n - 1) - p;
    return p;
}

int launch_gauss7_img(const uint8_t* src, int srcPitch, size_t srcStride, uint8_t* dst, int dstPitch, size_t dstStride, int W, int H,
                      const LineGeom& g, int which, int n_images, hipStream_t s)
{
    if (!which && g.lsdWideR > 3) return launch_sep_wide(src, srcStride, srcPitch, dst, dstStride, dstPitch, W, H, g.lsdWide, g.lsdWideR, n_images, s);
    return launch_sep7(src, srcStride, srcPitch, dst, dstStride, dstPitch, W, H, which ? g.lbdTaps : g.lsdTaps, n_images, s);
}

__global__ __launch_bounds__(256) void k_lsd_upsample(const uint8_t* __restrict__ src, uint8_t* __restrict__ dst,
                                                      const LineGeom* __restrict__ gp, const ResizeCoef* __restrict__ rx,
                                                      const ResizeCoef* __restrict__ ry)
{
    const LineGeom& g = *gp;
    const int img = blockIdx.y;
    const int quads = (g.Ws + 3) >> 2;
    const int idx = blockIdx.x * 256 + threadIdx.x;
    if (idx >= quads * g.Hs) return;
    const int dy = idx / quads, dx0 = (idx - dy * quads) * 4;
    const uint8_t* s = src + (size_t)img * g.pitchW * g.H;
    const ResizeCoef cy = ry[dy];
    const int y0 = min(max((int)cy.ofs, 0), g.H - 1), y1 = min(max((int)cy.ofs + 1, 0), g.H - 1);
    const uint8_t* S0 = s + (size_t)y0 * g.pitchW;
    const uint8_t* S1 = s + (size_t)y1 * g.pitchW;
    const int b0 = cy.a0, b1 = cy.a1;
    uint32_t out = 0;
#pragma unroll
    for (int k = 0; k < 4; ++k) {
        const int dx = dx0 + k;
        if (dx < g.Ws) {
            const ResizeCoef cx = rx[dx];
            const int sx = cx.ofs, sx1 = min(sx + 1, g.W - 1);
            const int h0 = S0[sx] * cx.a0 + S0[sx1] * cx.a1;
            const int h1 = S1[sx] * cx.a0 + S1[sx1] * cx.a1;
            const int v = g.resizeExact ? (h0 * b0 + h1 * b1 + 32768) >> 16 : (((b0 * (h0 >> 4)) >> 16) + ((b1 * (h1 >> 4)) >> 16) + 2) >> 2;
            out |= (uint32_t)(v & 0xff) << (8 * k);
        }
    }
    *reinterpret_cast<uint32_t*>(dst + (size_t)img * g.pitchS * g.Hs + (size_t)dy * g.pitchS + dx0) = out;
}

constexpr int LG_CHUNK = 4096;
__global__ __launch_bounds__(256) void k_lsd_grad(const uint8_t* __restrict__ scaled, uint32_t* __restrict__ grad,
                                                  const LineGeom* __restrict__ gp, int* __restrict__ maxN, int* __restrict__ chunkCnt)
{
    __shared__ int s_max[4], s_def[4];
    const LineGeom& g = *gp;
    const int img = blockIdx.y;
    int n = 0, ndef = 0;
    const uint8_t* sc = scaled + (size_t)img * g.pitchS * g.Hs;
    uint32_t* gout = grad + (size_t)img * g.Ps;
#pragma unroll 2
    for (int k = 0; k < LG_CHUNK / 1024; ++k) {
        const int idx0 = blockIdx.x * LG_CHUNK + (k * 256 + threadIdx.x) * 4;
        if (idx0 >= g.Ps) break;
        const int y = idx0 / g.Ws, x = idx0 - y * g.Ws;
        uint32_t packed[4] = {kNotDef, kNotDef, kNotDef, kNotDef};
        if (idx0 + 3 < g.Ps && x + 8 <= g.Ws && y < g.Hs - 1) {
            const uint8_t* r0 = sc + (size_t)y * g.pitchS + x;
            unsigned long long w0, w1;
            __builtin_memcpy(&w0, r0, 8);
            __builtin_memcpy(&w1, r0 + g.pitchS, 8);
#pragma unroll
            for (int p = 0; p < 4; ++p) {
                const int A = (int)((w0 >> (8 * p)) & 0xff), B = (int)((w0 >> (8 * p + 8)) & 0xff);
                const int C = (int)((w1 >> (8 * p)) & 0xff), D = (int)((w1 >> (8 * p + 8)) & 0xff);
                const int DA = D - A, BC = B - C;
                const int gx = DA + BC, gy = DA - BC;
                const int nn = gx * gx + gy * gy;
                if (nn >= g.nThr) { packed[p] = pack_g(gx, gy); n = max(n, nn); ++ndef; }
                else packed[p] = pack_g(gx, gy) | kNotDef;
            }
        } else {
            int yy = y, xx = x;
            for (int p = 0; p < 4; ++p, ++xx) {
                if (xx >= g.Ws) { xx -= g.Ws; ++yy; }
                if (idx0 + p < g.Ps && xx < g.Ws - 1 && yy < g.Hs - 1) {
                    const uint8_t* r0 = sc + (size_t)yy * g.pitchS + xx;
                    const uint8_t* r1 = r0 + g.pitchS;
                    const int DA = (int)r1[1] - (int)r0[0], BC = (int)r0[1] - (int)r1[0];
                    const int gx = DA + BC, gy = DA - BC;
                    const int nn = gx * gx + gy * gy;
                    if (nn >= g.nThr) { packed[p] = pack_g(gx, gy); n = max(n, nn); ++ndef; }
                    else packed[p] = pack_g(gx, gy) | kNotDef;
                }
            }
        }
        if (idx0 + 3 < g.Ps && ((reinterpret_cast<uintptr_t>(gout + idx0) & 15) == 0))
            *reinterpret_cast<uint4*>(gout + idx0) = make_uint4(packed[0], packed[1], packed[2], packed[3]);
        else
            for (int p = 0; p < 4 && idx0 + p < g.Ps; ++p) gout[idx0 + p] = packed[p];
    }
#pragma unroll
    for (int o = 32; o > 0; o >>= 1) { n = max(n, __shfl_xor(n, o)); ndef += __shfl_xor(ndef, o); }
    if ((threadIdx.x & 63) == 0) { s_max[threadIdx.x >> 6] = n; s_def[threadIdx.x >> 6] = ndef; }
    __syncthreads();
    if (threadIdx.x == 0) {
        n = max(max(s_max[0], s_max[1]), max(s_max[2], s_max[3]));
        if (n > 0) atomicMax(&maxN[img * 32], n);
        chunkCnt[(size_t)img * gridDim.x + blockIdx.x] = s_def[0] + s_def[1] + s_def[2] + s_def[3];
    }
}

constexpr int UG_ROWS = 8;
__global__ __launch_bounds__(64) void k_lsd_upgrad(const uint8_t* __restrict__ src, uint8_t* __restrict__ scaled, uint32_t* __restrict__ grad,
                                                   const LineGeom* __restrict__ gp, const ResizeCoef* __restrict__ rx, const ResizeCoef* __restrict__ ry,
                                                   int* __restrict__ maxN, int nsx, int writeScaled)
{
    const LineGeom& g = *gp;
    const int q = blockIdx.x * 64 + threadIdx.x;
    const int img = blockIdx.z;
    const int sw = g.W, sh = g.H, dw = g.Ws, dh = g.Hs, srcPitch = g.pitchW;
    int nmax = 0;
    if (q < nsx) {
        const int dx0 = 4 * q, dy0 = blockIdx.y * UG_ROWS;
        const uint8_t* s = src + (size_t)img * g.pitchW * g.H;
        uint8_t* d = scaled + (size_t)img * g.pitchS * g.Hs + dx0;
        uint32_t* gout = grad + (size_t)img * g.Ps;
        typedef unsigned short us2 __attribute__((ext_vector_type(2)));
        uint32_t sel[5], coef[5];
        const int base = min((int)rx[dx0].ofs, srcPitch - 8);
#pragma unroll
        for (int k = 0; k < 5; ++k) {
            const ResizeCoef c = rx[min(dx0 + k, dw - 1)];
            const int o0 = (int)c.ofs - base, o1 = min((int)c.ofs + 1, sw - 1) - base;
            sel[k] = (uint32_t)o0 | 0x0c00u | ((uint32_t)o1 << 16) | 0x0c000000u;
            coef[k] = (uint32_t)(uint16_t)c.a0 | ((uint32_t)(uint16_t)c.a1 << 16);
        }
        struct Raw { uint32_t w[2]; };
        auto load_row = [&](int r) -> Raw { Raw v; __builtin_memcpy(v.w, s + (size_t)r * srcPitch + base, 8); return v; };
        auto hrow = [&](const Raw& v, uint32_t* h) {
#pragma unroll
            for (int k = 0; k < 5; ++k) {
                const uint32_t pr = __builtin_amdgcn_perm(v.w[1], v.w[0], sel[k]);
                us2 va, vb;
                __builtin_memcpy(&va, &pr, 4); __builtin_memcpy(&vb, &coef[k], 4);
                h[k] = __builtin_amdgcn_udot2(va, vb, 0u, false) >> 4;
            }
        };
        auto rows_of = [&](int dy, int& r0, int& r1, uint32_t& b0, uint32_t& b1) {
            const ResizeCoef cy = ry[min(dy, dh - 1)];
            r0 = min(max((int)cy.ofs, 0), sh - 1); r1 = min(max((int)cy.ofs + 1, 0), sh - 1);
            b0 = (uint32_t)cy.a0; b1 = (uint32_t)cy.a1;
        };
        int r0, r1, ra = -1, rb = -1;
        uint32_t b0, b1;
        rows_of(dy0, r0, r1, b0, b1);
        Raw p0 = load_row(r0), p1 = load_row(r1);
        uint32_t hA[5] = {0, 0, 0, 0, 0}, hB[5] = {0, 0, 0, 0, 0};
        int prev[5] = {0, 0, 0, 0, 0};
#pragma unroll
        for (int rr = 0; rr <= UG_ROWS; ++rr) {
            const int dy = dy0 + rr;
            if (dy > dh || (rr > 0 && dy - 1 >= dh)) break;
            int n0, n1;
            uint32_t c0, c1;
            rows_of(dy + 1, n0, n1, c0, c1);
            Raw q0 = p0, q1 = p1;
            if (rr < UG_ROWS) {
                if (n0 != r0 && n0 != r1) q0 = load_row(n0);
                if (n1 != n0 && n1 != r1) q1 = load_row(n1);
                __builtin_amdgcn_sched_barrier(0);
            }
            uint32_t h0[5], h1[5];
            if (r0 == ra) { for (int k = 0; k < 5; ++k) h0[k] = hA[k]; }
            else if (r0 == rb) { for (int k = 0; k < 5; ++k) h0[k] = hB[k]; }
            else hrow(p0, h0);
            if (r1 == r0) { for (int k = 0; k < 5; ++k) h1[k] = h0[k]; }
            else if (r1 == rb) { for (int k = 0; k < 5; ++k) h1[k] = hB[k]; }
            else hrow(p1, h1);
            int cur[5];
#pragma unroll
            for (int k = 0; k < 5; ++k) cur[k] = (int)(((((b0 * h0[k]) >> 16) + ((b1 * h1[k]) >> 16) + 2u) >> 2) & 0xffu);
            if (writeScaled && rr < UG_ROWS && dy < dh) {
                const uint32_t out = (uint32_t)cur[0] | ((uint32_t)cur[1] << 8) | ((uint32_t)cur[2] << 16) | ((uint32_t)cur[3] << 24);
                __builtin_memcpy(d + (size_t)dy * g.pitchS, &out, 4);
            }
            if (rr > 0) {
                const int y = dy - 1;
                uint32_t packed[4];
#pragma unroll
                for (int k = 0; k < 4; ++k) {
                    const int A = prev[k], B = prev[k + 1], Cc = cur[k], D = cur[k + 1];
                    const int DA = D - A, BC = B - Cc;
                    const int gx = DA + BC, gy = DA - BC;
                    const int nn = gx * gx + gy * gy;
                    const bool inside = dx0 + k < dw - 1 && y < dh - 1;
                    packed[k] = inside ? (pack_g(gx, gy) | (nn >= g.nThr ? 0u : kNotDef)) : kNotDef;
                    if (inside && nn >= g.nThr) nmax = max(nmax, nn);
                }
                uint32_t* o = gout + (size_t)y * dw + dx0;
                const uintptr_t oa = reinterpret_cast<uintptr_t>(o);
                if (dx0 + 3 < dw && (oa & 15) == 0) *reinterpret_cast<uint4*>(o) = make_uint4(packed[0], packed[1], packed[2], packed[3]);
                else if (dx0 + 3 < dw && (oa & 7) == 0) {
                    reinterpret_cast<uint2*>(o)[0] = make_uint2(packed[0], packed[1]); reinterpret_cast<uint2*>(o)[1] = make_uint2(packed[2], packed[3]);
                } else {
#pragma unroll
                    for (int k = 0; k < 4; ++k) if (dx0 + k < dw) o[k] = packed[k];
                }
            }
#pragma unroll
            for (int k = 0; k < 5; ++k) prev[k] = cur[k];
            ra = r0; rb = r1;
#pragma unroll
            for (int k = 0; k < 5; ++k) { hA[k] = h0[k]; hB[k] = h1[k]; }
            r0 = n0; r1 = n1; b0 = c0; b1 = c1; p0 = q0; p1 = q1;
        }
    }
#pragma unroll
    for (int o = 32; o > 0; o >>= 1) nmax = max(nmax, __shfl_xor(nmax, o));
    if (threadIdx.x == 0 && nmax > 0) atomicMax(&maxN[img * 32], nmax);
}

constexpr int KEYS_THREADS = 512;
__device__ __forceinline__ int lsd_bin(int n, double bin_coef, float bin_coef_half_f)
{
    const float tf = __builtin_amdgcn_sqrtf((float)n) * bin_coef_half_f;
    const int b = (int)tf;
    const float fr = tf - (float)b;
    if (n != 0 && (fr < 1e-3f || fr > 0.999f)) return (int)(sqrt_quarter(n) * bin_coef);
    return b;
}

template <bool OWNER, bool ALLKEYS, int CH, bool WIDE = false>
__global__ __launch_bounds__(KEYS_THREADS) void k_lsd_keys(uint32_t* __restrict__ gradAll, const LineGeom* __restrict__ gp,
                                                  const int* __restrict__ maxN, const int* __restrict__ chunkCnt, uint32_t* __restrict__ keys,
                                                  int* __restrict__ keyCount, uint32_t* __restrict__ owner, const float* __restrict__ angDeg,
                                                  int nChunks, int total)
{
    constexpr int NWV = KEYS_THREADS / 64, SPAN = CH / NWV;
    extern __shared__ float s_deg[];
    __shared__ uint16_t s_list[CH];
    __shared__ int s_wcnt[NWV], s_base;
    const LineGeom& g = *gp;
    const int lane = threadIdx.x & 63, wv = threadIdx.x >> 6;
    const int L = blockIdx.x, per = total >> 3;
    const int V = L < per * 8 ? (L & 7) * per + (L >> 3) : L;
    const int img = V / nChunks, chunk = V - img * nChunks;
    const int Ws = g.Ws, Hs = g.Hs, Ps = g.Ps, nBins1 = g.nBins - 1;
    const uint32_t divM = g.divWsM, divS = g.divWsS;
    const float alignDeg = g.alignDeg;
    const double precG = g.prec;
    uint32_t* grad = gradAll + (size_t)img * Ps;
    const int c0 = chunk * CH;
    const int lo = c0 - Ws - 1, hi = c0 + CH + Ws + 1;
    const float kNaN = __builtin_nanf("");
    if (threadIdx.x == 0) s_base = 0;
    const double max_grad = sqrt((double)maxN[img * 32] / 4.0);
    const double bin_coef = (max_grad > 0) ? (double)nBins1 / max_grad : 0;
    const float bin_coef_half_f = 0.5f * (float)bin_coef;
    constexpr int NB = 8;
    constexpr bool SPLIT = ALLKEYS && !WIDE && CH == NB * KEYS_THREADS;
    if (SPLIT) {
        uint32_t* kall = keys + (size_t)img * Ps;
        const int keyEnd = min(Ps, (Hs - 1) * Ws);
        {
            uint32_t p[NB];
            float d[NB];
#pragma unroll
            for (int u = 0; u < NB; ++u) { const int idx = c0 + (int)threadIdx.x + u * KEYS_THREADS; p[u] = idx < Ps ? grad[idx] : kNotDef; }
#pragma unroll
            for (int u = 0; u < NB; ++u) d[u] = (p[u] & kNotDef) ? kNaN : angDeg[p[u] & 0x3fffffu];
#pragma unroll
            for (int u = 0; u < NB; ++u) s_deg[Ws + 1 + (int)threadIdx.x + u * KEYS_THREADS] = d[u];
#pragma unroll
            for (int u = 0; u < NB; ++u) {
                const int idx = c0 + (int)threadIdx.x + u * KEYS_THREADS;
                const int y = (int)(__umulhi((uint32_t)idx, divM) >> divS), x = idx - y * Ws;
                const int gx = unpack_gx(p[u]), gy = unpack_gy(p[u]);
                const int n = gx * gx + gy * gy;
                const float tf = __builtin_amdgcn_sqrtf((float)n) * bin_coef_half_f;
                int bin = (int)tf;
                const float fr = tf - (float)bin;
                const bool valid = (idx < keyEnd) & (x < Ws - 1);
                if (valid & (n != 0) & ((fr < 1e-3f) | (fr > 0.999f))) bin = (int)(sqrt_quarter(n) * bin_coef);
                if (valid) kall[(uint32_t)(idx - y)] = ((uint32_t)(nBins1 - bin) << 22) | (uint32_t)idx;
            }
        }
#pragma unroll
        for (int side = 0; side < 2; ++side) {
            const int first = side ? c0 + CH : lo, qBase = side ? CH + Ws + 1 : 0;
            constexpr int NH = 4;
            for (int h0 = (int)threadIdx.x; h0 < Ws + 1; h0 += NH * KEYS_THREADS) {
                uint32_t p[NH];
                float d[NH];
#pragma unroll
                for (int u = 0; u < NH; ++u) { const int h = h0 + u * KEYS_THREADS, idx = first + h; p[u] = (h < Ws + 1) & ((unsigned)idx < (unsigned)Ps) ? grad[idx] : kNotDef; }
#pragma unroll
                for (int u = 0; u < NH; ++u) d[u] = (p[u] & kNotDef) ? kNaN : angDeg[p[u] & 0x3fffffu];
#pragma unroll
                for (int u = 0; u < NH; ++u) if (h0 + u * KEYS_THREADS < Ws + 1) s_deg[qBase + h0 + u * KEYS_THREADS] = d[u];
            }
        }
    } else
    for (int i0 = lo + (int)threadIdx.x; i0 < hi; i0 += NB * KEYS_THREADS) {
        uint32_t p[NB];
        float d[NB];
#pragma unroll
        for (int u = 0; u < NB; ++u) { const int idx = i0 + u * KEYS_THREADS; p[u] = (unsigned)idx < (unsigned)Ps && idx < hi ? grad[idx] : kNotDef; }
#pragma unroll
        for (int u = 0; u < NB; ++u) d[u] = (p[u] & kNotDef) ? kNaN : angDeg[p[u] & 0x3fffffu];
#pragma unroll
        for (int u = 0; u < NB; ++u) if (i0 + u * KEYS_THREADS < hi) s_deg[i0 + u * KEYS_THREADS - lo] = d[u];
        if (ALLKEYS) {
            uint32_t* kall = keys + (size_t)img * Ps;
            unsigned long long* kallW = reinterpret_cast<unsigned long long*>(keys) + (size_t)img * Ps;
#pragma unroll
            for (int u = 0; u < NB; ++u) {
                const int idx = i0 + u * KEYS_THREADS;
                if (idx >= c0 && idx < min(Ps, c0 + CH)) {
                    const int y = WIDE ? idx / Ws : (int)(__umulhi((uint32_t)idx, divM) >> divS), x = idx - y * Ws;
                    if (x < Ws - 1 && y < Hs - 1) {
                        const int gx = unpack_gx(p[u]), gy = unpack_gy(p[u]);
                        if (WIDE) {
                            const int bin = (int)(sqrt_quarter(gx * gx + gy * gy) * bin_coef);
                            kallW[(size_t)y * (Ws - 1) + x] = ((unsigned long long)(uint32_t)(nBins1 - bin) << 32) | (unsigned long long)(uint32_t)idx;
                        } else {
                        const int bin = lsd_bin(gx * gx + gy * gy, bin_coef, bin_coef_half_f);
                        kall[y * (Ws - 1) + x] = ((uint32_t)(nBins1 - bin) << 22) | (uint32_t)idx;
                        }
                    }
                }
            }
        }
    }
    __syncthreads();
    if (!ALLKEYS) {
        int part = 0;
        for (int c = threadIdx.x; c < chunk; c += KEYS_THREADS) part += chunkCnt[(size_t)img * nChunks + c];
#pragma unroll
        for (int o = 32; o > 0; o >>= 1) part += __shfl_xor(part, o);
        if (lane == 0 && part) atomicAdd(&s_base, part);
    }
    unsigned long long defM[SPAN / 64];
    {
        int wc = 0;
#pragma unroll
        for (int k = 0; k < SPAN / 64; ++k) {
            const float dv = s_deg[c0 + wv * SPAN + k * 64 + lane - lo];
            defM[k] = wave_vote(dv == dv);
            wc += __popcll(defM[k]);
        }
        if (lane == 0) s_wcnt[wv] = wc;
    }
    __syncthreads();
    int n3 = 0, wbase = 0;
#pragma unroll
    for (int v = 0; v < NWV; ++v) { const int cv = s_wcnt[v]; if (v < wv) wbase += cv; n3 += cv; }
#pragma unroll
    for (int k = 0; k < SPAN / 64; ++k) {
        if (wave_bit(defM[k])) s_list[wbase + wave_rank_below(defM[k])] = (uint16_t)(wv * SPAN + k * 64 + lane);
        wbase += __popcll(defM[k]);
    }
    __syncthreads();
    uint32_t* kout = keys + (size_t)img * Ps + s_base;
    unsigned long long* koutW = reinterpret_cast<unsigned long long*>(keys) + (size_t)img * Ps + s_base;
    for (int t = threadIdx.x; t < n3; t += KEYS_THREADS) {
        const int li = s_list[t];
        const int idx = c0 + li;
        uint32_t p = 0;
        int bin = 0;
        if (!ALLKEYS) {
            p = grad[idx];
            const int gx = unpack_gx(p), gy = unpack_gy(p);
            bin = (int)(sqrt_quarter(gx * gx + gy * gy) * bin_coef);
        }
        const float* sd = s_deg + (idx - lo);
        const float deg0 = sd[0];
        float dmax = -1.f, margin = 1.0f;
#pragma unroll
        for (int q = 0; q < 9; ++q) {
            if (q == 4) continue;
            const float dn = sd[((q / 3) - 1) * Ws + (q % 3) - 1];
            const float dd = f_sub(fabsf(f_sub(fabsf(f_sub(deg0, dn)), 180.f)), alignDeg);
            dmax = fmaxf(dmax, dd);
            margin = fminf(margin, fabsf(dd));
        }
        bool iso = !(dmax >= 0.f);
        if (margin < 1e-3f || alignDeg < 0.f) {
            const double a0 = d_mul((double)deg0, kDegToRads);
            iso = true;
#pragma unroll
            for (int q = 0; q < 9; ++q) {
                if (q == 4) continue;
                const float dn = sd[((q / 3) - 1) * Ws + (q % 3) - 1];
                if (dn != dn) continue;
                double n_theta = d_sub(a0, d_mul((double)dn, kDegToRads));
                if (n_theta < 0) n_theta = -n_theta;
                if (n_theta > kM32PI) { n_theta = d_sub(n_theta, kM2PI); if (n_theta < 0) n_theta = -n_theta; }
                if (n_theta <= precG) iso = false;
            }
        }
        if (iso) grad[idx] = (ALLKEYS ? grad[idx] : p) | kIso;
        if (OWNER) owner[(size_t)img * Ps + idx] = 0xffffffffu;
        if (!ALLKEYS) { if (WIDE) koutW[t] = ((unsigned long long)(uint32_t)(nBins1 - bin) << 32) | (unsigned long long)(uint32_t)idx;
                        else kout[t] = ((uint32_t)(nBins1 - bin) << 22) | (uint32_t)idx; }
    }
    if (!ALLKEYS && chunk == nChunks - 1 && threadIdx.x == 0) keyCount[img * 32] = s_base + n3;
}


__device__ __forceinline__ double grad_angle(int gx, int gy) { return d_mul((double)dev_fastAtan2((float)gx, (float)(-gy)), kDegToRads); }

__device__ __forceinline__ bool is_aligned(double a, double theta, double prec)
{
    double n_theta = fabs(d_sub(theta, a));
    if (n_theta > kM32PI) n_theta = fabs(d_sub(n_theta, kM2PI));
    return n_theta <= prec;
}

__device__ __forceinline__ void sincos_2pi(double x, double* sn, double* cs)
{
    const int k = (int)__fma_rn(x, 0.63661977236758134308, 0.5);
    double r = __fma_rn(-(double)k, 1.57079632679489655800e+00, x);
    r = __fma_rn(-(double)k, 6.12323399573676603587e-17, r);
    const double z = r * r;
    double ps = __fma_rn(z, 1.58969099521155010221e-10, -2.50507602534068634195e-08);
    ps = __fma_rn(z, ps, 2.75573137070700676789e-06);
    ps = __fma_rn(z, ps, -1.98412698298579493134e-04);
    ps = __fma_rn(z, ps, 8.33333333332248946124e-03);
    ps = __fma_rn(z, ps, -1.66666666666666324348e-01);
    const double s0 = __fma_rn(r * z, ps, r);
    double pc = __fma_rn(z, -1.13596475577881948265e-11, 2.08757232129817482790e-09);
    pc = __fma_rn(z, pc, -2.75573143513906633035e-07);
    pc = __fma_rn(z, pc, 2.48015872894767294178e-05);
    pc = __fma_rn(z, pc, -1.38888888888741095749e-03);
    pc = __fma_rn(z, pc, 4.16666666666666019037e-02);
    const double hz = 0.5 * z;
    const double w = 1.0 - hz;
    const double c0 = w + (((1.0 - w) - hz) + z * z * pc);
    const bool sw = k & 1;
    double so = sw ? c0 : s0, co = sw ? s0 : c0;
    if (k & 2) so = -so;
    if ((k + 1) & 2) co = -co;
    *sn = so; *cs = co;
}

__global__ __launch_bounds__(256) void k_lsd_angle_table(float* __restrict__ angDeg, AngEnt* __restrict__ ent, int libmFloat)
{
    const uint32_t i = blockIdx.x * 256 + threadIdx.x;
    const int gx = unpack_gx(i), gy = unpack_gy(i);
    const float deg = dev_fastAtan2((float)gx, (float)(-gy));
    const double ang = d_mul((double)deg, kDegToRads);
    double sn, cs;
    sincos_2pi((double)(float)ang, &sn, &cs);
    if (libmFloat) { cs = (double)glibc_cosf((float)ang); sn = (double)glibc_sinf((float)ang); }
    angDeg[i] = deg;
    double s0, c0;
    sincos_2pi(ang, &s0, &c0);
    AngEnt e; e.cs = cs; e.sn = sn; e.ang = ang; e.seed = make_float2((float)c0, (float)s0);
    ent[i] = e;
}

int launch_lsd_angle_table(LineDeviceBufs& b, int libmFloat, hipStream_t s)
{
    hipLaunchKernelGGL(k_lsd_angle_table, dim3((1u << 22) / 256), dim3(256), 0, s, b.angDeg, reinterpret_cast<AngEnt*>(b.angEnt), libmFloat);
    OLF_HIP_CHECK(hipGetLastError());
    return OLF_OK;
}


__global__ __launch_bounds__(256) void k_fdiv_sweep(unsigned long long seed, int per_thread, unsigned long long* __restrict__ mismatches)
{
    unsigned long long st = seed ^ (0x9E3779B97F4A7C15ull * (unsigned long long)(blockIdx.x * 256 + threadIdx.x + 1));
    unsigned long long bad = 0;
    for (int i = 0; i < per_thread; ++i) {
        st ^= st >> 12; st ^= st << 25; st ^= st >> 27;
        const unsigned long long r = st * 0x2545F4914F6CDD1Dull;
        const int eb = (int)(r & 63) - 45;
        float b = ldexpf(1.0f + (float)((r >> 8) & 0x7fffff) * 1.1920929e-7f, eb);
        float a = ldexpf(1.0f + (float)((r >> 32) & 0x7fffff) * 1.1920929e-7f, eb - (int)((r >> 56) & 31));
        if (((r >> 61) & 7) == 0) a = b;
        if (((r >> 61) & 7) == 1) a = 0.f;
        if (a > b) a = b;
        b = __fadd_rn(b, (float)2.2204460492503131e-16);
        const float q0 = __fdiv_rn(a, b), q1 = fdiv_unscaled(a, b);
        bad += __float_as_uint(q0) != __float_as_uint(q1);
    }
    if (bad) atomicAdd(mismatches, bad);
}

__global__ __launch_bounds__(256) void k_sqrtq_sweep(int count, unsigned long long* __restrict__ mismatches)
{
    const int n = blockIdx.x * 256 + threadIdx.x;
    if (n >= count) return;
    const double a = sqrt((double)n / 4.0), b = sqrt_quarter(n);
    if (__double_as_longlong(a) != __double_as_longlong(b)) atomicAdd(mismatches, 1ull);
    int bad = 0;
    for (int c = 0; c < 97; ++c) {
        const int mN = 36 + c * 5418;
        if (n > mN) continue;
        const double bin_coef = 1023.0 / sqrt((double)mN / 4.0);
        bad += lsd_bin(n, bin_coef, 0.5f * (float)bin_coef) != (int)(a * bin_coef);
    }
    if (bad) atomicAdd(mismatches, (unsigned long long)bad);
}

__global__ __launch_bounds__(256) void k_align_sweep(const LineGeom* __restrict__ gp, const AngEnt* __restrict__ ent, unsigned long long seed, int per_thread,
                                                     unsigned long long* __restrict__ out)
{
    const LineGeom& g = *gp;
    const float tanLo = g.alignTanLo, tanHi = g.alignTanHi;
    const double prec = g.prec, precWrap = g.precWrap;
    unsigned long long x = seed ^ ((unsigned long long)(blockIdx.x * 256 + threadIdx.x) * 0x9E3779B97F4A7C15ull);
    auto next = [&]() { x ^= x << 13; x ^= x >> 7; x ^= x << 17; return x; };
    next(); next();
    unsigned long long bad = 0, und = 0;
    for (int k = 0; k < per_thread; ++k) {
        const unsigned long long r = next(), r2 = next();
        const int span = (r & 3) ? 40 : 510;
        const int gx = (int)((r >> 2) % (2 * span + 1)) - span, gy = (int)((r >> 24) % (2 * span + 1)) - span;
        const AngEnt e = ent[pack_g(gx, gy)];
        const double u = (double)(r2 & 0xfffff) / 1048576.0;
        const double len = 0.6 * exp(9.2 * (double)((r2 >> 20) & 0xfffff) / 1048576.0);
        double th;
        if ((r2 >> 40) & 3) th = e.ang + (((r2 >> 42) & 1) ? prec : -prec) + (u - 0.5) * 6e-3;
        else th = u * kM2PI;
        const float sx = (float)(len * cos(th)), sy = (float)(len * sin(th));
        const double reg_angle = d_mul((double)agent_fastAtan2(sy, sx), kDegToRads);
        const double nth = fabs(d_sub(reg_angle, e.ang));
        const bool exact = nth <= prec || nth >= precWrap;
        const float dot = __fmaf_rn(sy, e.seed.y, __fmul_rn(sx, e.seed.x));
        const float crs = __fmaf_rn(sx, e.seed.y, -__fmul_rn(sy, e.seed.x));
        const bool sa = fabsf(crs) <= __fmaf_rn(tanLo, dot, -1e-4f), sn = fabsf(crs) >= __fmaf_rn(tanHi, dot, 1e-4f);
        if (sa && sn) ++bad;
        else if (sa || sn) bad += sa != exact;
        else ++und;
    }
    atomicAdd(out, bad); atomicAdd(out + 1, und); atomicAdd(out + 2, (unsigned long long)per_thread);
}

int launch_align_sweep(const LineDeviceBufs& b, unsigned long long seed, int blocks, int per_thread, unsigned long long* d_out, hipStream_t s)
{
    hipLaunchKernelGGL(k_align_sweep, dim3(blocks), dim3(256), 0, s, b.geom, reinterpret_cast<const AngEnt*>(b.angEnt), seed, per_thread, d_out);
    OLF_HIP_CHECK(hipGetLastError());
    return OLF_OK;
}

int launch_sqrtq_sweep(int count, unsigned long long* d_mismatches, hipStream_t s)
{
    hipLaunchKernelGGL(k_sqrtq_sweep, dim3((count + 255) / 256), dim3(256), 0, s, count, d_mismatches);
    OLF_HIP_CHECK(hipGetLastError());
    return OLF_OK;
}

int launch_fdiv_sweep(unsigned long long seed, int blocks, int per_thread, unsigned long long* d_mismatches, hipStream_t s)
{
    hipLaunchKernelGGL(k_fdiv_sweep, dim3(blocks), dim3(256), 0, s, seed, per_thread, d_mismatches);
    OLF_HIP_CHECK(hipGetLastError());
    return OLF_OK;
}

struct SegCand { float e0, e1, e2, e3, length; int keep; };

__device__ __forceinline__ SegCand rect_to_cand(const LineGeom& g, double x1, double y1, double x2, double y2)
{
    x1 = d_add(x1, 0.5); y1 = d_add(y1, 0.5); x2 = d_add(x2, 0.5); y2 = d_add(y2, 0.5);
    if (g.scale != 1) { x1 = x1 / g.scale; y1 = y1 / g.scale; x2 = x2 / g.scale; y2 = y2 / g.scale; }
    float e0 = (float)x1, e1 = (float)y1, e2 = (float)x2, e3 = (float)y2;
    const int cols = g.W, rows = g.H;
    if (e0 < 0) e0 = 0;
    if (e0 >= cols) e0 = (float)cols - 1.0f;
    if (e2 < 0) e2 = 0;
    if (e2 >= cols) e2 = (float)cols - 1.0f;
    if (e1 < 0) e1 = 0;
    if (e1 >= rows) e1 = (float)rows - 1.0f;
    if (e3 < 0) e3 = 0;
    if (e3 >= rows) e3 = (float)rows - 1.0f;
    const double dxe = (double)f_sub(e0, e2), dye = (double)f_sub(e1, e3);
    const double length = (double)(float)sqrt(d_add(d_mul(dxe, dxe), d_mul(dye, dye)));
    SegCand c; c.e0 = e0; c.e1 = e1; c.e2 = e2; c.e3 = e3; c.length = (float)length; c.keep = length > g.minLength;
    return c;
}

struct AgentRect { double x1, y1, x2, y2, width, theta, dx, dy, prec, p; };

__device__ __forceinline__ double log_modgrad(uint32_t w) { const int gx = unpack_gx(w), gy = unpack_gy(w); return sqrt((double)(gx * gx + gy * gy) / 4.0); }

__device__ __forceinline__ AgentRect agent_region2rect(const uint2* lg, int n, double reg_angle, double prec)
{
    AgentRect rec;
    double x = 0, y = 0, sum = 0;
    for (int q = 0; q < n; ++q) {
        const uint2 e = lg[q];
        const double wt = log_modgrad(e.y);
        x = d_add(x, d_mul((double)(int)(e.x & 0xffffu), wt));
        y = d_add(y, d_mul((double)(int)(e.x >> 16), wt));
        sum = d_add(sum, wt);
    }
    x = x / sum; y = y / sum;
    double Ixx = 0, Iyy = 0, Ixy = 0;
    for (int q = 0; q < n; ++q) {
        const uint2 e = lg[q];
        const double wt = log_modgrad(e.y);
        const double ex = d_sub((double)(int)(e.x & 0xffffu), x), ey = d_sub((double)(int)(e.x >> 16), y);
        Ixx = d_add(Ixx, d_mul(d_mul(ey, ey), wt));
        Iyy = d_add(Iyy, d_mul(d_mul(ex, ex), wt));
        Ixy = d_sub(Ixy, d_mul(d_mul(ex, ey), wt));
    }
    const double dI = d_sub(Ixx, Iyy);
    const double lambda = d_mul(0.5, d_sub(d_add(Ixx, Iyy), sqrt(d_add(d_mul(dI, dI), d_mul(d_mul(4.0, Ixy), Ixy)))));
    double theta = (fabs(Ixx) > fabs(Iyy)) ? (double)dev_fastAtan2((float)d_sub(lambda, Ixx), (float)Ixy)
                                           : (double)dev_fastAtan2((float)Ixy, (float)d_sub(lambda, Iyy));
    theta = d_mul(theta, kDegToRads);
    {
        double diff = d_sub(theta, reg_angle);
        while (diff <= -kPI) diff = d_add(diff, kM2PI);
        while (diff > kPI) diff = d_sub(diff, kM2PI);
        if (fabs(diff) > prec) theta = d_add(theta, kPI);
    }
    double ddx, ddy;
    sincos(theta, &ddy, &ddx);
    double l_min = 0, l_max = 0, w_min = 0, w_max = 0;
    for (int q = 0; q < n; ++q) {
        const uint32_t pk = lg[q].x;
        const double rdx = d_sub((double)(int)(pk & 0xffffu), x), rdy = d_sub((double)(int)(pk >> 16), y);
        const double lq = d_add(d_mul(rdx, ddx), d_mul(rdy, ddy));
        const double wq = d_add(d_mul(-rdx, ddy), d_mul(rdy, ddx));
        l_max = fmax(l_max, lq); l_min = fmin(l_min, lq);
        w_max = fmax(w_max, wq); w_min = fmin(w_min, wq);
    }
    rec.x1 = d_add(x, d_mul(l_min, ddx)); rec.y1 = d_add(y, d_mul(l_min, ddy));
    rec.x2 = d_add(x, d_mul(l_max, ddx)); rec.y2 = d_add(y, d_mul(l_max, ddy));
    rec.width = d_sub(w_max, w_min);
    if (rec.width < 1.0) rec.width = 1.0;
    rec.theta = theta; rec.dx = ddx; rec.dy = ddy; rec.prec = prec; rec.p = 0;
    return rec;
}

__device__ __forceinline__ double agent_log_gamma(double x)
{
    if (x > 15.0) return 0.918938533204673 + (x - 0.5) * log(x) - x + 0.5 * x * log(x * sinh(1 / x) + 1 / (810.0 * pow(x, 6.0)));
    const double q[7] = {75122.6331530, 80916.6278952, 36308.2951477, 8687.24529705, 1168.92649479, 83.8676043424, 2.50662827511};
    double a = (x + 0.5) * log(x + 5.5) - (x + 5.5);
    double b = 0;
    for (int n = 0; n < 7; ++n) {
        a -= log(x + (double)n);
        b += q[n] * pow(x, (double)n);
    }
    return a + log(b);
}

__device__ __forceinline__ double agent_nfa(int n, int k, double p, double LOG_NT)
{
    if (n == 0 || k == 0) return -LOG_NT;
    if (n == k) return -LOG_NT - (double)n * log10(p);
    const double p_term = p / (1 - p);
    const double log1term = agent_log_gamma((double)n + 1) - agent_log_gamma((double)k + 1) - agent_log_gamma((double)(n - k) + 1) + (double)k * log(p) +
                            (double)(n - k) * log(1.0 - p);
    double term = exp(log1term);
    {
        bool eq = term == 0.0;
        if (!eq) { double am = fabs(term); if (am < 2.2250738585072014e-308) am = 2.2250738585072014e-308; eq = (fabs(term) / am) <= (100.0 * 2.2204460492503131e-16); }
        if (eq) {
            if (k > n * p) return -log1term / 2.30258509299404568402 - LOG_NT;
            return -LOG_NT;
        }
    }
    double bin_tail = term;
    for (int i = k + 1; i <= n; ++i) {
        const double bin_term = (double)(n - i + 1) / (double)i;
        const double mult_term = bin_term * p_term;
        term *= mult_term;
        bin_tail += term;
        if (bin_term < 1) {
            const double err = term * ((1 - pow(mult_term, (double)(n - i + 1))) / (1 - mult_term) - 1);
            if (err < 0.1 * fabs(-log10(bin_tail) - LOG_NT) * bin_tail) break;
        }
    }
    return -log10(bin_tail) - LOG_NT;
}

__device__ __forceinline__ double agent_rect_nfa(const LineGeom& g, const uint32_t* __restrict__ grad, const AngEnt* __restrict__ ent, const AgentRect& rec, int lane)
{
    const double half_width = rec.width / 2.0;
    const double dyhw = rec.dy * half_width, dxhw = rec.dx * half_width;
    int ex[4], ey[4];
    ex[0] = (int)(rec.x1 - dyhw); ey[0] = (int)(rec.y1 + dxhw);
    ex[1] = (int)(rec.x2 - dyhw); ey[1] = (int)(rec.y2 + dxhw);
    ex[2] = (int)(rec.x2 + dyhw); ey[2] = (int)(rec.y2 - dxhw);
    ex[3] = (int)(rec.x1 + dyhw); ey[3] = (int)(rec.y1 - dxhw);
    for (int i = 1; i < 4; ++i)
        for (int j = i; j > 0 && (ex[j] == ex[j - 1] ? ey[j] < ey[j - 1] : ex[j] < ex[j - 1]); --j) {
            const int tx = ex[j], ty = ey[j]; ex[j] = ex[j - 1]; ey[j] = ey[j - 1]; ex[j - 1] = tx; ey[j - 1] = ty;
        }
    int imin = 0, imax = 0;
    for (int i = 1; i < 4; ++i) {
        if (ey[imin] > ey[i]) imin = i;
        if (ey[imax] < ey[i]) imax = i;
    }
    unsigned taken = 1u << imin;
    int il = -1;
    for (int i = 0; i < 4; ++i)
        if (!((taken >> i) & 1u)) { if (il < 0) il = i; else if (ex[il] > ex[i]) il = i; }
    taken |= 1u << il;
    int ir = -1;
    for (int i = 0; i < 4; ++i)
        if (!((taken >> i) & 1u)) { if (ir < 0) ir = i; else if (ex[ir] < ex[i]) ir = i; }
    taken |= 1u << ir;
    int it = -1;
    for (int i = 0; i < 4; ++i)
// ... 544 lines not shown
            __threadfence_block();
            rec = agent_region2rect(lg, n, reg_angle, prec);
            double density = agent_density(n, rec);
            if (density >= g.densityTh) { accept = true; break; }
            {
                uint2* lw = reg + rbase;
                const uint2 e0 = lw[0];
                const double xc = (double)(int)(e0.x & 0xffffu), yc = (double)(int)(e0.x >> 16);
                const double ra1 = d_sub(rec.x1, xc), rb1 = d_sub(rec.y1, yc), ra2 = d_sub(rec.x2, xc), rb2 = d_sub(rec.y2, yc);
                const double radSq1 = d_add(d_mul(ra1, ra1), d_mul(rb1, rb1)), radSq2 = d_add(d_mul(ra2, ra2), d_mul(rb2, rb2));
                double radSq = radSq1 > radSq2 ? radSq1 : radSq2;
                bool ok = true;
                while (density < g.densityTh) {
                    radSq = d_mul(radSq, 0.5625);
                    for (int q = 0; q < n; ++q) {
                        const uint2 e = lw[q];
                        const double ax = d_sub((double)(int)(e.x & 0xffffu), xc), ay = d_sub((double)(int)(e.x >> 16), yc);
                        if (d_add(d_mul(ax, ax), d_mul(ay, ay)) > radSq) {
                            const uint2 last = lw[n - 1];
                            if (lane == 0) { grad[(int)(e.x >> 16) * Ws + (int)(e.x & 0xffffu)] = e.y; lw[q] = last; }
                            __threadfence_block();
                            --n; --q;
                        }
                    }
                    if (n < 2) { ok = false; break; }
                    rec = agent_region2rect(lw, n, reg_angle, prec);
                    density = agent_density(n, rec);
                }
                PEND_FLUSH();
                accept = ok;
            }
            break;
          }
            if (REFINE) {
                if (REFINE >= 2 && accept) {
                    rec.p = g.pProb;
                    __threadfence_block();
                    if (agent_rect_improve(g, grad, ent, rec, lane) <= g.logEps) accept = false;
                }
                if (accept) {
                    if (nreg < maxRegions) {
                        const SegCand cnd = rect_to_cand(g, rec.x1, rec.y1, rec.x2, rec.y2);
                        if (lane == 0) {
                            candAll[(size_t)img * maxRegions + nreg] = cnd;
                        }
                        ++nreg;
                    } else if (lane == 0) atomicOr(status, 8);
                }
            }
            if (!REFINE && n >= minRegSize) {
                if (nreg < maxRegions) {
                    if (lane == 0) {
                        RegionRec rr; rr.start = rbase; rr.n = n; rr.angle = reg_angle;
                        recs[nreg] = rr;
                    }
                    ++nreg;
                    rbase += n;
                } else if (lane == 0) atomicOr(status, 8);
            }
#ifdef OLF_STATS
            st_acc += n; if (n >= minRegSize) st_logged += n; if (n > 1) st_regl += __popcll(wave_vote(valid && lane > l));
#endif
            if (REFINE && maskEpoch != flushEpoch) {
                const uint32_t wnow = valid ? grad[addr] : kUsed;
                mask = wave_vote(valid && lane > l && !(wnow & (kUsed | kNotDef)) && s_pend[addr & (PEND - 1)] != addr);
                if (wave_bit(mask)) wseed = wnow;
                if (wave_bit(mask & ~tabM) && !isoSeed) { const AngEnt* t = ent + (wseed & 0x3fffffu); seedAng = t->ang; seedSum = t->seed; }
                tabM |= mask;
                maskEpoch = flushEpoch;
            }
            else if (n == 1) mask &= mask - 1;
            else if (PIPE || maskEpoch == flushEpoch) {
                mask &= ~((2ull << l) - 1ull) & wave_vote(s_pend[addr & (PEND - 1)] != addr);
            } else {
                mask = wave_vote(valid && lane > l && !(grad[addr] & (kUsed | kNotDef)) && s_pend[addr & (PEND - 1)] != addr);
                maskEpoch = flushEpoch;
            }
        }
        if (PFSEED) asm volatile("" :: "v"(pfA), "v"(pfB));
    }
#undef ALIGN_CHEAP
#undef ENSURE_ANGLE
#undef LOG_ROOM
#undef LOG_AT
#undef MARK_USED
#undef PEND_FLUSH
#undef PEND_CLEAR
#ifdef OLF_STATS
    if (lane == 0 && img == 0) { long long* o = reinterpret_cast<long long*>(status + 16); o[0] = st_rounds; o[1] = st_k; o[2] = st_t; o[3] = st_full; o[4] = st_single; o[5] = st_rounds_big; o[6] = st_k_big; o[7] = st_t_big;
        o[8] = st_flush; o[9] = st_iters; o[10] = st_deep1; o[11] = st_deep2; o[12] = st_cand; o[13] = st_regions; o[14] = st_mem;
        o[15] = nkeys; o[16] = st_win; o[17] = st_seedl; o[18] = st_regl; o[19] = st_acc; o[20] = st_isos; o[21] = st_logged; o[22] = st_winLive; o[23] = st_first; o[24] = st_cand1;
        o[25] = st_acc1; o[26] = st_wentries; o[27] = st_whand; o[28] = st_wdone; o[29] = st_wpend; }
#endif
    if (lane == 0) { regCount[img] = over ? 0 : nreg; if (growFmt) growFmt[img] = 1; if (g.spillOf && !retry) g.spillOf[img] = over ? -1 : 0; }
}


template <bool CHAINED>
__device__ __forceinline__ void lsd_rect_region(const LineGeom& g, int img, int r, const uint32_t* __restrict__ gradAll,
                                                const uint32_t* __restrict__ regionAll, const RegionRec* __restrict__ recsAll,
                                                SegCand* __restrict__ candAll, const int* __restrict__ linksAll, int nChunks, const int* __restrict__ spillOf,
                                                const uint32_t* __restrict__ spillArena)
{
    const uint32_t* grad = gradAll + (size_t)img * g.Ps;
    const RegionRec rr = recsAll[(size_t)img * g.maxRegions + r];
    const uint32_t* px_list = CHAINED ? regionAll + (size_t)img * nChunks * 32 : nullptr;
    const int sblk = CHAINED || !spillOf ? 0 : spillOf[img];
    const uint2* log2 = CHAINED ? nullptr
                      : (sblk > 0 ? reinterpret_cast<const uint2*>(spillArena) + (size_t)(sblk - 1) * g.Ps
                                  : reinterpret_cast<const uint2*>(regionAll + (size_t)img * g.regionStride)) + rr.start;
    const int* links = CHAINED ? linksAll + (size_t)img * nChunks : nullptr;
    const int n = rr.n, Ws = g.Ws;
    int cid = rr.start, nxt = -1;
#define RECT_BLOCK(q0) (px_list + (size_t)cid * 32 + ((q0) & 31))
#define RECT_STEP(q0) do { if (CHAINED) { if (((q0) & 31) == 0) { if (q0) cid = nxt; nxt = links[cid]; } } } while (0)
    constexpr int U = 16;
    double x = 0, y = 0, sum = 0;
    for (int q0 = 0; q0 < n; q0 += U) {
        uint32_t rp[U], p[U];
        if (CHAINED) {
            RECT_STEP(q0);
            const uint32_t* blk = RECT_BLOCK(q0);
#pragma unroll
            for (int u = 0; u < U; ++u) rp[u] = q0 + u < n ? blk[u] : 0u;
#pragma unroll
            for (int u = 0; u < U; ++u) p[u] = grad[(int)(rp[u] >> 16) * Ws + (int)(rp[u] & 0xffffu)];
        } else {
#pragma unroll
            for (int u = 0; u < U; u += 2) {
                uint4 e = make_uint4(0u, 0u, 0u, 0u);
                if (q0 + u + 1 < n) __builtin_memcpy(&e, log2 + q0 + u, 16);
                else if (q0 + u < n) { const uint2 e1 = log2[q0 + u]; e.x = e1.x; e.y = e1.y; }
                rp[u] = e.x; p[u] = e.y; rp[u + 1] = e.z; p[u + 1] = e.w;
            }
        }
#pragma unroll
        for (int u = 0; u < U; ++u) {
            if (q0 + u < n) {
                const int px = (int)(rp[u] & 0xffffu), py = (int)(rp[u] >> 16);
                const int gx = unpack_gx(p[u]), gy = unpack_gy(p[u]);
                const double wt = sqrt_quarter(gx * gx + gy * gy);
                x = d_add(x, d_mul((double)px, wt));
                y = d_add(y, d_mul((double)py, wt));
                sum = d_add(sum, wt);
            }
        }
    }
    x = x / sum; y = y / sum;
    double Ixx = 0, Iyy = 0, Ixy = 0;
    cid = rr.start;
    for (int q0 = 0; q0 < n; q0 += U) {
        uint32_t rp[U], p[U];
        if (CHAINED) {
            RECT_STEP(q0);
            const uint32_t* blk = RECT_BLOCK(q0);
#pragma unroll
            for (int u = 0; u < U; ++u) rp[u] = q0 + u < n ? blk[u] : 0u;
#pragma unroll
            for (int u = 0; u < U; ++u) p[u] = grad[(int)(rp[u] >> 16) * Ws + (int)(rp[u] & 0xffffu)];
        } else {
#pragma unroll
            for (int u = 0; u < U; u += 2) {
                uint4 e = make_uint4(0u, 0u, 0u, 0u);
                if (q0 + u + 1 < n) __builtin_memcpy(&e, log2 + q0 + u, 16);
                else if (q0 + u < n) { const uint2 e1 = log2[q0 + u]; e.x = e1.x; e.y = e1.y; }
                rp[u] = e.x; p[u] = e.y; rp[u + 1] = e.z; p[u + 1] = e.w;
            }
        }
#pragma unroll
        for (int u = 0; u < U; ++u) {
            if (q0 + u < n) {
                const int px = (int)(rp[u] & 0xffffu), py = (int)(rp[u] >> 16);
                const int gx = unpack_gx(p[u]), gy = unpack_gy(p[u]);
                const double wt = sqrt_quarter(gx * gx + gy * gy);
                const double ex = d_sub((double)px, x), ey = d_sub((double)py, y);
                Ixx = d_add(Ixx, d_mul(d_mul(ey, ey), wt));
                Iyy = d_add(Iyy, d_mul(d_mul(ex, ex), wt));
                Ixy = d_sub(Ixy, d_mul(d_mul(ex, ey), wt));
            }
        }
    }
    const double dI = d_sub(Ixx, Iyy);
    const double lambda = d_mul(0.5, d_sub(d_add(Ixx, Iyy), sqrt(d_add(d_mul(dI, dI), d_mul(d_mul(4.0, Ixy), Ixy)))));
    double theta = (fabs(Ixx) > fabs(Iyy)) ? (double)dev_fastAtan2((float)d_sub(lambda, Ixx), (float)Ixy)
                                           : (double)dev_fastAtan2((float)Ixy, (float)d_sub(lambda, Iyy));
    theta = d_mul(theta, kDegToRads);
    {
        double diff = d_sub(theta, rr.angle);
        while (diff <= -kPI) diff = d_add(diff, kM2PI);
        while (diff > kPI) diff = d_sub(diff, kM2PI);
        if (fabs(diff) > g.prec) theta = d_add(theta, kPI);
    }
    double ddx, ddy;
    sincos(theta, &ddy, &ddx);
    double l_min = 0, l_max = 0;
    cid = rr.start;
    for (int q0 = 0; q0 < n; q0 += U) {
        uint32_t rp[U];
        if (CHAINED) {
            RECT_STEP(q0);
            const uint32_t* blk = RECT_BLOCK(q0);
#pragma unroll
            for (int u = 0; u < U; ++u) rp[u] = q0 + u < n ? blk[u] : 0u;
        } else {
#pragma unroll
            for (int u = 0; u < U; u += 2) {
                uint4 e = make_uint4(0u, 0u, 0u, 0u);
                if (q0 + u + 1 < n) __builtin_memcpy(&e, log2 + q0 + u, 16);
                else if (q0 + u < n) e.x = log2[q0 + u].x;
                rp[u] = e.x; rp[u + 1] = e.z;
            }
        }
#pragma unroll
        for (int u = 0; u < U; ++u) {
            if (q0 + u < n) {
                const double rdx = d_sub((double)(int)(rp[u] & 0xffffu), x), rdy = d_sub((double)(int)(rp[u] >> 16), y);
                const double lq = d_add(d_mul(rdx, ddx), d_mul(rdy, ddy));
                l_max = fmax(l_max, lq); l_min = fmin(l_min, lq);
            }
        }
    }
    double x1 = d_add(x, d_mul(l_min, ddx)), y1 = d_add(y, d_mul(l_min, ddy));
    double x2 = d_add(x, d_mul(l_max, ddx)), y2 = d_add(y, d_mul(l_max, ddy));
    const SegCand c = rect_to_cand(g, x1, y1, x2, y2);
    candAll[(size_t)img * g.maxRegions + r] = c;
#undef RECT_BLOCK
#undef RECT_STEP
}

template <bool CHAINED>
__global__ __launch_bounds__(256) void k_lsd_rect(const LineGeom* __restrict__ gp, const uint32_t* __restrict__ gradAll,
                                                  const uint32_t* __restrict__ regionAll, const RegionRec* __restrict__ recsAll,
                                                  const int* __restrict__ regCount, SegCand* __restrict__ candAll,
                                                  const int* __restrict__ linksAll, int nChunks, const int* __restrict__ spillOf, const uint32_t* __restrict__ spillArena)
{
    const int img = blockIdx.y, r = blockIdx.x * 256 + threadIdx.x;
    if (r >= regCount[img]) return;
    lsd_rect_region<CHAINED>(*gp, img, r, gradAll, regionAll, recsAll, candAll, linksAll, nChunks, spillOf, spillArena);
}

__global__ __launch_bounds__(256) void k_lsd_rect_mixed(const LineGeom* __restrict__ gp, const uint32_t* __restrict__ gradAll,
                                                        const uint32_t* __restrict__ regionAll, const RegionRec* __restrict__ recsAll,
                                                        const int* __restrict__ regCount, SegCand* __restrict__ candAll,
                                                        const int* __restrict__ linksAll, int nChunks, const int* __restrict__ growFmt, const int* __restrict__ spillOf,
                                                        const uint32_t* __restrict__ spillArena)
{
    const int img = blockIdx.y, r = blockIdx.x * 256 + threadIdx.x;
    if (r >= regCount[img]) return;
    if (growFmt[img] == 1) lsd_rect_region<false>(*gp, img, r, gradAll, regionAll, recsAll, candAll, linksAll, nChunks, spillOf, spillArena);
    else lsd_rect_region<true>(*gp, img, r, gradAll, regionAll, recsAll, candAll, linksAll, nChunks, spillOf, spillArena);
}

__global__ __launch_bounds__(256) void k_lsd_emit(const LineGeom* __restrict__ gp, const SegCand* __restrict__ candAll, const int* __restrict__ regCount,
                                                  olf_keyline* __restrict__ rawLines, int* __restrict__ rawCount, int* __restrict__ status)
{
    __shared__ int s_wave[4];
    __shared__ int s_base;
    const LineGeom& g = *gp;
    const int img = blockIdx.x, tid = threadIdx.x, lane = tid & 63, wave = tid >> 6;
    const SegCand* cand = candAll + (size_t)img * g.maxRegions;
    olf_keyline* out = rawLines + (size_t)img * g.maxDetect;
    const int nreg = regCount[img];
    if (tid == 0) s_base = 0;
    __syncthreads();
    for (int r0 = 0; r0 < nreg; r0 += 256) {
        const int r = r0 + tid;
        SegCand c; c.keep = 0;
        if (r < nreg) c = cand[r];
        const unsigned long long km = wave_vote(c.keep != 0);
        if (lane == 0) s_wave[wave] = __popcll(km);
        __syncthreads();
        int pos = s_base + wave_rank_below(km);
        for (int w = 0; w < wave; ++w) pos += s_wave[w];
        if (c.keep) {
            if (pos < g.maxDetect) {
                const float e0 = c.e0, e1 = c.e1, e2 = c.e2, e3 = c.e3;
                olf_keyline kl;
                kl.startPointX = e0; kl.startPointY = e1; kl.endPointX = e2; kl.endPointY = e3;
                kl.sPointInOctaveX = e0; kl.sPointInOctaveY = e1; kl.ePointInOctaveX = e2; kl.ePointInOctaveY = e3;
                kl.lineLength = c.length;
                const int rx1 = __float2int_rn(e0), ry1 = __float2int_rn(e1), rx2 = __float2int_rn(e2), ry2 = __float2int_rn(e3);
                kl.numOfPixels = max(abs(rx2 - rx1), abs(ry2 - ry1)) + 1;
                kl.angle = g.libmFloat ? glibc_atan2f(f_sub(e3, e1), f_sub(e2, e0)) : (float)atan2((double)f_sub(e3, e1), (double)f_sub(e2, e0));
                kl.class_id = pos; kl.octave = 0;
                kl.size = f_mul(f_sub(e2, e0), f_sub(e3, e1));
                kl.response = f_div(kl.lineLength, (float)max(g.W, g.H));
                kl.pt_x = f_div(f_add(e2, e0), 2.0f); kl.pt_y = f_div(f_add(e3, e1), 2.0f);
                out[pos] = kl;
            } else atomicOr(status, 8);
        }
        __syncthreads();
        if (tid == 0) s_base += s_wave[0] + s_wave[1] + s_wave[2] + s_wave[3];
        __syncthreads();
    }
    if (tid == 0) rawCount[img] = min(s_base, g.maxDetect);
}

LsdPlan lsd_plan(const LineGeom& g, const LineDeviceBufs& b, const LsdOverrides& o, const DeviceLimits& d, int n)
{
    LsdPlan p{};
    p.resize = (g.resizeTiled & 4) && g.seedOrder == 1 ? LsdPlan::Upgrad : g.resizeTiled ? LsdPlan::Tiled : LsdPlan::Upsample;
    p.sort = g.wide ? LsdPlan::Wide : g.seedOrder == 1 ? LsdPlan::Seed : LsdPlan::Radix;
    p.keysAll = g.seedOrder == 1;

    const int m = o.sortMode;
    p.sortWaves = m < 0 ? (n <= 256 ? 8 : n <= 640 ? 4 : n <= 1536 ? 2 : 1) : m == 2 ? 8 : m == 1 ? 4 : m == 5 ? 2 : 1;
    auto sortLds = [](int w) { return w == 8 ? 104 * 1024 : w == 4 ? 56 * 1024 : w == 2 ? 32 * 1024 : 0; };
    while (sortLds(p.sortWaves) > d.maxLds) p.sortWaves /= 2;
    p.sortTop = p.sortWaves > 1 && b.topBuf && n <= 64;
    p.sortGroups = !p.sortTop ? 1 : n <= 16 ? 8 : 4;

    const int autoWaves = n <= 512 ? 16 : n <= 1024 ? 8
                        : n <= 1536 ? 4
                        : n <= 2048 ? 8 : n <= kMwMaxImages ? 4
                        : 0;
    p.growWaves = (g.refine || g.wide || n > b.ownerImages) ? 0 : o.waves >= 0 ? o.waves : autoWaves;
    p.keysOwner = p.growWaves > 0;
    if (p.growWaves > 0) {
        const int nw = p.growWaves;
        p.robEntries = o.robEntries > 0 ? o.robEntries : (nw >= 16 ? 512 : nw >= 8 ? 256 : 128);
        p.poolChunks = o.poolChunks > 0 ? std::min(o.poolChunks, b.nChunks) : b.nChunks;
        int G = o.groups > 0 ? o.groups : nw >= 16 && n <= kMgMaxImages ? 2 : 1;
        while (G > 1 && (!b.mg || n > b.mgImages || n * G > d.nCU || p.poolChunks / G < p.robEntries + 64)) G >>= 1;
        p.growGroups = G;
        p.scatter = o.scatter;
        p.agentRefine = 0; p.agentPF = 0; p.agentLaunches = 1;
    } else {
        p.agentRefine = g.refine;
        p.agentPF = (g.wide ? 32 : 0) | (g.refine ? 0 : g.alignTanLo < 0.f ? 11 : 27);
        p.agentLaunches = g.logCap < g.Ps ? 2 : 1;
    }
    p.rect = g.refine ? LsdPlan::Emit : p.growWaves > 0 ? LsdPlan::Mixed : LsdPlan::Plain;
    return p;
}

int launch_lsd_dense(const LineGeom& g, const LineDeviceBufs& b, const LsdPlan& p, const uint8_t* d_in, int in_pitch, int n_images, hipStream_t s, bool writeScaled)
{
    OLF_HIP_CHECK(hipMemsetAsync(b.maxN, 0, (size_t)n_images * 32 * sizeof(int), s));
    OLF_HIP_CHECK(hipMemsetAsync(b.keyCount, 0, (size_t)n_images * 32 * sizeof(int), s));
    { int rc = launch_gauss7_img(d_in, in_pitch, (size_t)in_pitch * g.H, b.lsdBlur, g.pitchW, (size_t)g.pitchW * g.H, g.W, g.H, g, 0, n_images, s);
      if (rc != OLF_OK) return rc; }
    if (p.resize == LsdPlan::Upgrad) {
        const int nsx = (g.Ws + 3) / 4;
        hipLaunchKernelGGL(k_lsd_upgrad, dim3((nsx + 63) / 64, (g.Hs + UG_ROWS - 1) / UG_ROWS, n_images), dim3(64), 0, s, b.lsdBlur, b.scaled, b.grad, b.geom, b.rx, b.ry,
                           b.maxN, nsx, writeScaled ? 1 : 0);
    } else if (p.resize == LsdPlan::Tiled) {
        int rc = launch_resize_tiled(b.lsdBlur, (size_t)g.pitchW * g.H, g.pitchW, g.W, g.H, b.scaled, (size_t)g.pitchS * g.Hs, g.pitchS, g.Ws, g.Hs, b.rx,
                                     b.ry, n_images, s, (g.resizeTiled & 2) != 0);
        if (rc != OLF_OK) return rc;
    } else {
        const int quads = ((g.Ws + 3) >> 2) * g.Hs;
        hipLaunchKernelGGL(k_lsd_upsample, dim3((quads + 255) / 256, n_images), dim3(256), 0, s, b.lsdBlur, b.scaled, b.geom, b.rx, b.ry);
    }
    if (p.resize != LsdPlan::Upgrad) hipLaunchKernelGGL(k_lsd_grad, dim3((g.Ps + LG_CHUNK - 1) / LG_CHUNK, n_images), dim3(256), 0, s, b.scaled, b.grad, b.geom, b.maxN, b.chunkCnt);
    {
        const int nChunks = (g.Ps + LG_CHUNK - 1) / LG_CHUNK, total = nChunks * n_images;
        const size_t lds = (size_t)(LG_CHUNK + 2 * g.Ws + 2) * sizeof(float);
        if (lds > 60 * 1024) { set_error("LSD image wider than the key kernel's LDS window"); return OLF_ERR_CAPACITY; }
        const auto keys = p.sort == LsdPlan::Wide ? (p.keysAll ? k_lsd_keys<false, true, LG_CHUNK, true> : k_lsd_keys<false, false, LG_CHUNK, true>)
                        : p.keysAll ? (p.keysOwner ? k_lsd_keys<true, true, LG_CHUNK> : k_lsd_keys<false, true, LG_CHUNK>)
                        : p.keysOwner ? k_lsd_keys<true, false, LG_CHUNK> : k_lsd_keys<false, false, LG_CHUNK>;
        hipLaunchKernelGGL(keys, dim3(total), dim3(KEYS_THREADS), lds, s, b.grad, b.geom, b.maxN, b.chunkCnt, p.sort == LsdPlan::Radix ? b.keysB : b.keysA, b.keyCount,
                           b.owner, b.angDeg, nChunks, total);
    }
    OLF_HIP_CHECK(hipGetLastError());
    return OLF_OK;
}

int launch_lsd_seed_order(const LineGeom& g, const LineDeviceBufs& b, const LsdPlan& p, int n_images, hipStream_t s)
{
    if (p.sort == LsdPlan::Wide) return launch_lsd_sort_wide(g, b, n_images, s, -1, -1, -1, -1);
    if (p.sort == LsdPlan::Seed) return launch_lsd_seedsort(g, b, p, n_images, s, -1, -1, -1);
    return launch_lsd_sort(g, b, n_images, s);
}

int launch_lsd_grow(const LineGeom& g, const LineDeviceBufs& b, const LsdPlan& p, int n_images, hipStream_t s)
{
    static const struct { int refine, pf; decltype(&k_lsd_grow<0, 0>) kernel; } kAgents[] = {
        {0, 0, k_lsd_grow<0, 0>}, {2, 32, k_lsd_grow<2, 32>}, {1, 32, k_lsd_grow<1, 32>}, {0, 32 | 11, k_lsd_grow<0, 32 | 11>}, {0, 32 | 27, k_lsd_grow<0, 32 | 27>},
        {2, 0, k_lsd_grow<2, 0>}, {1, 0, k_lsd_grow<1, 0>}, {0, 11, k_lsd_grow<0, 11>}, {0, 27, k_lsd_grow<0, 27>}};
    decltype(&k_lsd_grow<0, 0>) agent = nullptr;
    for (const auto& a : kAgents) if (a.refine == p.agentRefine && a.pf == p.agentPF) agent = a.kernel;
    if (!agent) { set_error("launch_lsd_grow: no such k_lsd_grow instantiation"); return OLF_ERR_INVALID; }
    if (g.spillCtl) OLF_HIP_CHECK(hipMemsetAsync(g.spillCtl, 0, sizeof(int), s));
    if (p.growWaves > 0) { const int rc = launch_lsd_grow_mw(g, b, p, n_images, s); if (rc != OLF_OK) return rc; }
    for (int retry = 0; retry < p.agentLaunches; ++retry)
        hipLaunchKernelGGL(agent, dim3(n_images), dim3(64), 0, s, b.geom, b.grad, b.keysB, b.keyCount, b.region,
                           p.agentRefine ? (RegionRec*)nullptr : reinterpret_cast<RegionRec*>(b.keysA), b.regCount, b.status, reinterpret_cast<const AngEnt*>(b.angEnt),
                           p.growWaves > 0 ? b.growFmt : (int*)nullptr, p.agentRefine ? reinterpret_cast<SegCand*>(b.keysA) : (SegCand*)nullptr, retry);
    OLF_HIP_CHECK(hipGetLastError());
    return OLF_OK;
}

int launch_lsd_rect(const LineGeom& g, const LineDeviceBufs& b, const LsdPlan& p, int n_images, hipStream_t s)
{
    if (p.rect == LsdPlan::Emit) {
        hipLaunchKernelGGL(k_lsd_emit, dim3(n_images), dim3(256), 0, s, b.geom, reinterpret_cast<const SegCand*>(b.keysA), b.regCount, b.rawLines,
                           b.rawCount, b.status);
        OLF_HIP_CHECK(hipGetLastError());
        return OLF_OK;
    }
    const int* spillOf = g.logCap < g.Ps ? g.spillOf : nullptr;
    if (p.rect == LsdPlan::Mixed)
        hipLaunchKernelGGL(k_lsd_rect_mixed, dim3((g.rectGrid + 255) / 256, n_images), dim3(256), 0, s, b.geom, b.grad, b.region,
                           reinterpret_cast<const RegionRec*>(b.keysA), b.regCount, reinterpret_cast<SegCand*>(b.keysB), b.links, b.nChunks, b.growFmt, spillOf, g.spillArena);
    else
        hipLaunchKernelGGL(k_lsd_rect<false>, dim3((g.rectGrid + 255) / 256, n_images), dim3(256), 0, s, b.geom, b.grad, b.region,
                           reinterpret_cast<const RegionRec*>(b.keysA), b.regCount, reinterpret_cast<SegCand*>(b.keysB), b.links, b.nChunks, spillOf, g.spillArena);
    hipLaunchKernelGGL(k_lsd_emit, dim3(n_images), dim3(256), 0, s, b.geom, reinterpret_cast<const SegCand*>(b.keysB), b.regCount, b.rawLines,
                       b.rawCount, b.status);
    OLF_HIP_CHECK(hipGetLastError());
    return OLF_OK;
}

}
```

Before: 15130 stereo frames/s.

## Rewrite strip resize as rolling source-row walk and add tiled LSD key kernel

Resize strip kernels (ORB pyramid and LSD upgrad) now walk source rows sequentially, computing each horizontal row once and emitting every destination row that falls between the two cached rows. Strip height goes from 8 to 16 rows, and a shared header adds scalar-coefficient multiply-hi blends and perm-based packing. A new 2D-tiled LSD key/isotropy kernel replaces the chunked kernel when seed ordering is used and the image is not wide. The aim is fewer redundant loads and ALU work, with less launch and LDS overhead, at the cost of more complex edge handling and fewer blocks.

```diff
diff --git a/include/orbline.h b/include/orbline.h
--- a/include/orbline.h
+++ b/include/orbline.h
@@ -89,6 +89,9 @@
 int olf_debug_seed_sort_mode(olf_ctx* ctx, int mode);
 int olf_debug_seed_sort_wide(olf_ctx* ctx, const uint64_t* keys, int n, int64_t kthr, int depth_limit, int full, uint32_t* out, int32_t* out_n);
 int olf_debug_lsd_pool(olf_ctx* ctx, int pool_chunks);
+int olf_debug_lsd_keys_general(olf_ctx* ctx, int on);
+int olf_debug_lsd_grad(olf_ctx* ctx, int image, uint32_t* out);
+int olf_debug_front_plan(olf_ctx* ctx, int n_images, int32_t* out);
 int olf_debug_fdiv_sweep(olf_ctx* ctx, uint64_t seed, int blocks, int per_thread, uint64_t* mismatches);
 int olf_debug_sqrtq_sweep(olf_ctx* ctx, int count, uint64_t* mismatches);
 int olf_debug_align_sweep(olf_ctx* ctx, uint64_t seed, int blocks, int per_thread, uint64_t* out3);
diff --git a/orb_line_slam_amd/_lib.py b/orb_line_slam_amd/_lib.py
--- a/orb_line_slam_amd/_lib.py
+++ b/orb_line_slam_amd/_lib.py
@@ -169,6 +169,9 @@
         L.olf_remap_linear.argtypes = [C.c_void_p, C.c_void_p, C.c_int, C.c_int, C.c_void_p, C.c_void_p, C.c_int, C.c_int, C.c_int, C.c_void_p]
         L.olf_debug_lsd_waves.argtypes = [C.c_void_p, C.c_int, C.c_int]
         L.olf_debug_lsd_pool.argtypes = [C.c_void_p, C.c_int]
+        L.olf_debug_lsd_keys_general.argtypes = [C.c_void_p, C.c_int]
+        L.olf_debug_lsd_grad.argtypes = [C.c_void_p, C.c_int, C.c_void_p]
+        L.olf_debug_front_plan.argtypes = [C.c_void_p, C.c_int, C.c_void_p]
         L.olf_debug_lsd_groups.argtypes = [C.c_void_p, C.c_int]
         L.olf_debug_lsd_scatter.argtypes = [C.c_void_p, C.c_int]
         L.olf_debug_lsd_log_cap.argtypes = [C.c_void_p, C.c_int]
diff --git a/orb_line_slam_amd/csrc/api_debug.cpp b/orb_line_slam_amd/csrc/api_debug.cpp
--- a/orb_line_slam_amd/csrc/api_debug.cpp
+++ b/orb_line_slam_amd/csrc/api_debug.cpp
@@ -157,6 +157,36 @@
     return OLF_OK;
 }
 
+int olf_debug_lsd_keys_general(olf_ctx* c, int on)
+{
+    if (!c) { set_error("olf_debug_lsd_keys_general: bad argument"); return OLF_ERR_INVALID; }
+    c->lsd_force.keysGeneral = on ? 1 : 0;
+    return OLF_OK;
+}
+
+int olf_debug_lsd_grad(olf_ctx* c, int image, uint32_t* out)
+{
+    if (!c || !out || image < 0 || image >= c->max_images) return OLF_ERR_INVALID;
+    OLF_HIP_CHECK(hipDeviceSynchronize());
+    OLF_HIP_CHECK(hipMemcpy(out, c->lb.grad + (size_t)image * c->line.geom.Ps, (size_t)c->line.geom.Ps * 4, hipMemcpyDeviceToHost));
+    return OLF_OK;
+}
+
+int olf_debug_front_plan(olf_ctx* c, int n_images, int32_t* out)
+{
+    if (!c || !out || n_images < 1 || n_images > c->max_images) return OLF_ERR_INVALID;
+    const LsdPlan p = lsd_plan(c->line.geom, c->lb, c->lsd_force, c->limits, n_images);
+    out[0] = p.resize == LsdPlan::Upgrad ? 0 : p.resize == LsdPlan::Tiled ? 1 : 2;
+    out[1] = p.keysTiled ? 1 : 0;
+    out[2] = p.growWaves;
+    out[3] = 0;
+    for (int l = 1; l < c->orb.geom.nlevels; ++l) {
+        const LevelGeom &P = c->orb.geom.lv[l - 1], &L = c->orb.geom.lv[l];
+        out[3 + l] = (L.resizeTiled & 2) && (L.pitch & 3) == 0 && (c->orb.geom.pyrBytes & 3) == 0 && P.pitch >= 8 ? 1 : 0;
+    }
+    return OLF_OK;
+}
+
 int olf_debug_lsd_owner(olf_ctx* c, int image, uint32_t* out)
 {
     if (!c || !out || image < 0 || image >= c->lb.ownerImages) return OLF_ERR_INVALID;
diff --git a/orb_line_slam_amd/csrc/filters.hip b/orb_line_slam_amd/csrc/filters.hip
--- a/orb_line_slam_amd/csrc/filters.hip
+++ b/orb_line_slam_amd/csrc/filters.hip
@@ -1,4 +1,5 @@
 #include "olf_internal.hpp"
+#include "resize_strip.hpp"
 #include <algorithm>
 
 namespace olf {
@@ -339,18 +340,15 @@
     }
 }
 
-constexpr int RS_ROWS = 8;
-
 __global__ __launch_bounds__(64) void k_resize_strip(const uint8_t* __restrict__ src, size_t srcImgStride, int srcPitch, int sw, int sh,
                                                      uint8_t* __restrict__ dst, size_t dstImgStride, int dstPitch, int dw, int dh,
                                                      const ResizeCoef* __restrict__ rx, const ResizeCoef* __restrict__ ry, int nsx)
 {
     const int q = blockIdx.x * 64 + threadIdx.x;
     if (q >= nsx) return;
-    const int dx0 = 4 * q, dy0 = blockIdx.y * RS_ROWS;
+    const int dx0 = 4 * q, dy0 = blockIdx.y * RS_ROWS, dyEnd = min(dy0 + RS_ROWS, dh);
     const uint8_t* s = src + (size_t)blockIdx.z * srcImgStride;
-    uint8_t* d = dst + (size_t)blockIdx.z * dstImgStride + dx0;
-    typedef unsigned short us2 __attribute__((ext_vector_type(2)));
+    uint8_t* d = dst + (size_t)blockIdx.z * dstImgStride;
     uint32_t sel[4], coef[4];
     const int base = min((int)rx[dx0].ofs, srcPitch - 8);
 #pragma unroll
@@ -360,59 +358,40 @@
         sel[k] = (uint32_t)o0 | 0x0c00u | ((uint32_t)o1 << 16) | 0x0c000000u;
         coef[k] = (uint32_t)(uint16_t)c.a0 | ((uint32_t)(uint16_t)c.a1 << 16);
     }
-    struct Raw { uint32_t w[2]; };
-    auto load_row = [&](int r) -> Raw { Raw v; __builtin_memcpy(v.w, s + (size_t)r * srcPitch + base, 8); return v; };
-    auto hrow = [&](const Raw& v, uint32_t* h) {
-#pragma unroll
-        for (int k = 0; k < 4; ++k) {
-            const uint32_t pr = __builtin_amdgcn_perm(v.w[1], v.w[0], sel[k]);
-            us2 va, vb;
-            __builtin_memcpy(&va, &pr, 4); __builtin_memcpy(&vb, &coef[k], 4);
-            h[k] = __builtin_amdgcn_udot2(va, vb, 0u, false) >> 4;
-        }
-    };
-    auto rows_of = [&](int dy, int& r0, int& r1, uint32_t& b0, uint32_t& b1) {
-        const ResizeCoef cy = ry[min(dy, dh - 1)];
-        r0 = min(max((int)cy.ofs, 0), sh - 1); r1 = min(max((int)cy.ofs + 1, 0), sh - 1);
-        b0 = (uint32_t)cy.a0; b1 = (uint32_t)cy.a1;
-    };
-    int r0, r1, ra = -1, rb = -1;
-    uint32_t b0, b1;
-    rows_of(dy0, r0, r1, b0, b1);
-    Raw p0 = load_row(r0), p1 = load_row(r1);
-    uint32_t hA[4] = {0, 0, 0, 0}, hB[4] = {0, 0, 0, 0};
-#pragma unroll
-    for (int rr = 0; rr < RS_ROWS; ++rr) {
-        const int dy = dy0 + rr;
-        if (dy >= dh) break;
-        int n0, n1;
-        uint32_t c0, c1;
-        rows_of(dy + 1, n0, n1, c0, c1);
-        Raw q0 = p0, q1 = p1;
-        if (rr + 1 < RS_ROWS) {
-            if (n0 != r0 && n0 != r1) q0 = load_row(n0);
-            if (n1 != n0 && n1 != r1) q1 = load_row(n1);
-            __builtin_amdgcn_sched_barrier(0);
-        }
-        uint32_t h0[4], h1[4];
-        if (r0 == ra) { for (int k = 0; k < 4; ++k) h0[k] = hA[k]; }
-        else if (r0 == rb) { for (int k = 0; k < 4; ++k) h0[k] = hB[k]; }
-        else hrow(p0, h0);
-        if (r1 == r0) { for (int k = 0; k < 4; ++k) h1[k] = h0[k]; }
-        else if (r1 == rb) { for (int k = 0; k < 4; ++k) h1[k] = hB[k]; }
-        else hrow(p1, h1);
-        uint32_t out = 0;
-#pragma unroll
-        for (int k = 0; k < 4; ++k) {
-            const uint32_t v = (((b0 * h0[k]) >> 16) + ((b1 * h1[k]) >> 16) + 2u) >> 2;
-            out |= (v & 0xffu) << (8 * k);
-        }
-        __builtin_memcpy(d + (size_t)dy * dstPitch, &out, 4);
-        ra = r0; rb = r1;
-#pragma unroll
-        for (int k = 0; k < 4; ++k) { hA[k] = h0[k]; hB[k] = h1[k]; }
-        r0 = n0; r1 = n1; b0 = c0; b1 = c1; p0 = q0; p1 = q1;
-    }
+    auto load_row = [&](int v) -> ResizeRaw {
+        ResizeRaw r;
+        __builtin_memcpy(r.w, s + (uint32_t)(min(max(v, 0), sh - 1) * srcPitch + base), 8);
+        return r;
+    };
+    int dy = dy0;
+    ResizeRowCoef cy = resize_row_coef(ry, dy), cn = resize_row_coef(ry, min(dy + 1, dh - 1));
+    int v = cy.ofs;
+    uint32_t hA[4], hB[4];
+    ResizeRaw ra = load_row(v), rb = load_row(v + 1);
+    auto emit = [&](const uint32_t* hp, const uint32_t* hc) {
+        while (cy.ofs < v) {
+            const uint32_t out = resize_pack4(resize_vblend(cy.b0s, hp[0], cy.b1s, hc[0]), resize_vblend(cy.b0s, hp[1], cy.b1s, hc[1]),
+                                              resize_vblend(cy.b0s, hp[2], cy.b1s, hc[2]), resize_vblend(cy.b0s, hp[3], cy.b1s, hc[3]));
+            __builtin_memcpy(d + (uint32_t)(dy * dstPitch + dx0), &out, 4);
+            ++dy;
+            cy = cn;
+            if (dy == dyEnd) cy.ofs = 0x7fffffff;
+            cn = resize_row_coef(ry, min(dy + 1, dh - 1));
+        }
+    };
+    resize_hrow<4>(ra, sel, coef, hA);
+    do {
+        ra = load_row(v + 2);
+        __builtin_amdgcn_sched_barrier(0);
+        resize_hrow<4>(rb, sel, coef, hB);
+        ++v;
+        emit(hA, hB);
+        rb = load_row(v + 2);
+        __builtin_amdgcn_sched_barrier(0);
+        resize_hrow<4>(ra, sel, coef, hA);
+        ++v;
+        emit(hB, hA);
+    } while (dy != dyEnd);
 }
 
 bool resize_strip_fits(const ResizeCoef* rx, int sw, int dw, int ncols)
diff --git a/orb_line_slam_amd/csrc/line_internal.hpp b/orb_line_slam_amd/csrc/line_internal.hpp
--- a/orb_line_slam_amd/csrc/line_internal.hpp
+++ b/orb_line_slam_amd/csrc/line_internal.hpp
@@ -87,6 +87,7 @@
     int groups = -1;
     int poolChunks = 0;
     int scatter = 0;
+    int keysGeneral = 0;
 };
 
 struct DeviceLimits { int nCU = 64, maxLds = 64 * 1024; };
@@ -95,6 +96,7 @@
     enum Resize { Upgrad, Tiled, Upsample } resize;
     enum Sort { Radix, Seed, Wide } sort;
     bool keysOwner, keysAll;
+    bool keysTiled;
     int sortWaves;
     bool sortTop; int sortGroups;
     int growWaves;
diff --git a/orb_line_slam_amd/csrc/lsd.hip b/orb_line_slam_amd/csrc/lsd.hip
--- a/orb_line_slam_amd/csrc/lsd.hip
+++ b/orb_line_slam_amd/csrc/lsd.hip
@@ -1,4 +1,5 @@
 #include "lsd_device.hpp"
+#include "resize_strip.hpp"
 
 namespace olf {
 
@@ -111,7 +112,101 @@
     }
 }
 
-constexpr int UG_ROWS = 8;
+__device__ __forceinline__ int lsd_norm24(int gx, int gy)
+{
+    int t, n;
+    asm("v_mul_i32_i24 %0, %1, %1" : "=v"(t) : "v"(gx));
+    asm("v_mad_i32_i24 %0, %1, %1, %2" : "=v"(n) : "v"(gy), "v"(t));
+    return n;
+}
+template <bool EDGE>
+__device__ __forceinline__ int lsd_upgrad_strip(const uint8_t* __restrict__ s, uint8_t* __restrict__ d, uint32_t* __restrict__ gout, int sw, int sh, int dw, int dh,
+                                                int srcPitch, int dstPitch, int nThr, const ResizeCoef* __restrict__ rx, const ResizeCoef* __restrict__ ry,
+                                                int dx0, int dy0, int writeScaled)
+{
+    uint32_t sel[5], coef[5];
+    const int base = min((int)rx[dx0].ofs, srcPitch - 8);
+#pragma unroll
+    for (int k = 0; k < 5; ++k) {
+        const ResizeCoef c = rx[min(dx0 + k, dw - 1)];
+        const int o0 = (int)c.ofs - base, o1 = min((int)c.ofs + 1, sw - 1) - base;
+        sel[k] = (uint32_t)o0 | 0x0c00u | ((uint32_t)o1 << 16) | 0x0c000000u;
+        coef[k] = (uint32_t)(uint16_t)c.a0 | ((uint32_t)(uint16_t)c.a1 << 16);
+    }
+    auto load_row = [&](int v) -> ResizeRaw {
+        ResizeRaw r;
+        __builtin_memcpy(r.w, s + (uint32_t)(min(max(v, 0), sh - 1) * srcPitch + base), 8);
+        return r;
+    };
+    auto store_row = [&](int y, const uint32_t* packed) {
+        uint32_t* o = reinterpret_cast<uint32_t*>(reinterpret_cast<uint8_t*>(gout) + (uint32_t)(y * dw + dx0) * 4u);
+        if (!EDGE || dx0 + 3 < dw) __builtin_memcpy(o, packed, 16);
+        else {
+#pragma unroll
+            for (int k = 0; k < 4; ++k) if (dx0 + k < dw) o[k] = packed[k];
+        }
+    };
+    const int dyLast = min(dy0 + UG_ROWS, dh - 1), dyStrip = min(dy0 + UG_ROWS, dh);
+    int dy = dy0;
+    ResizeRowCoef cy = resize_row_coef(ry, dy), cn = resize_row_coef(ry, min(dy + 1, dh - 1));
+    int v = cy.ofs;
+    uint32_t hA[5], hB[5];
+    ResizeRaw ra = load_row(v), rb = load_row(v + 1);
+    int prev[5] = {0, 0, 0, 0, 0};
+    int nmax = 0;
+    auto emit = [&](const uint32_t* hp, const uint32_t* hc) {
+        while (cy.ofs < v) {
+            uint32_t cw[5];
+            int cur[5];
+#pragma unroll
+            for (int k = 0; k < 5; ++k) { cw[k] = resize_vblend(cy.b0s, hp[k], cy.b1s, hc[k]); cur[k] = (int)(cw[k] & 0xffu); }
+            if (writeScaled && dy < dyStrip) {
+                const uint32_t out = resize_pack4(cw[0], cw[1], cw[2], cw[3]);
+                __builtin_memcpy(d + (uint32_t)(dy * dstPitch + dx0), &out, 4);
+            }
+            if (dy > dy0) {
+                uint32_t packed[4];
+#pragma unroll
+                for (int k = 0; k < 4; ++k) {
+                    const int A = prev[k], B = prev[k + 1], Cc = cur[k], D = cur[k + 1];
+                    const int DA = D - A, BC = B - Cc;
+                    const int gx = DA + BC, gy = DA - BC;
+                    int nn = lsd_norm24(gx, gy);
+                    uint32_t w = pack_g(gx, gy) | (nn >= nThr ? 0u : kNotDef);
+                    if (EDGE && dx0 + k >= dw - 1) { w = kNotDef; nn = 0; }
+                    packed[k] = w;
+                    nmax = max(nmax, nn);
+                }
+                store_row(dy - 1, packed);
+            }
+#pragma unroll
+            for (int k = 0; k < 5; ++k) prev[k] = cur[k];
+            ++dy;
+            cy = cn;
+            if (dy > dyLast) cy.ofs = 0x7fffffff;
+            cn = resize_row_coef(ry, min(dy + 1, dh - 1));
+        }
+    };
+    resize_hrow<5>(ra, sel, coef, hA);
+    do {
+        ra = load_row(v + 2);
+        __builtin_amdgcn_sched_barrier(0);
+        resize_hrow<5>(rb, sel, coef, hB);
+        ++v;
+        emit(hA, hB);
+        rb = load_row(v + 2);
+        __builtin_amdgcn_sched_barrier(0);
+        resize_hrow<5>(ra, sel, coef, hA);
+        ++v;
+        emit(hB, hA);
+    } while (dy <= dyLast);
+    if (dy0 + UG_ROWS >= dh) {
+        const uint32_t packed[4] = {kNotDef, kNotDef, kNotDef, kNotDef};
+        store_row(dh - 1, packed);
+    }
+    return nmax;
+}
+
 __global__ __launch_bounds__(64) void k_lsd_upgrad(const uint8_t* __restrict__ src, uint8_t* __restrict__ scaled, uint32_t* __restrict__ grad,
                                                    const LineGeom* __restrict__ gp, const ResizeCoef* __restrict__ rx, const ResizeCoef* __restrict__ ry,
                                                    int* __restrict__ maxN, int nsx, int writeScaled)
@@ -119,106 +214,20 @@
     const LineGeom& g = *gp;
     const int q = blockIdx.x * 64 + threadIdx.x;
     const int img = blockIdx.z;
-    const int sw = g.W, sh = g.H, dw = g.Ws, dh = g.Hs, srcPitch = g.pitchW;
+    const int nThr = g.nThr;
     int nmax = 0;
     if (q < nsx) {
         const int dx0 = 4 * q, dy0 = blockIdx.y * UG_ROWS;
         const uint8_t* s = src + (size_t)img * g.pitchW * g.H;
-        uint8_t* d = scaled + (size_t)img * g.pitchS * g.Hs + dx0;
+        uint8_t* d = scaled + (size_t)img * g.pitchS * g.Hs;
         uint32_t* gout = grad + (size_t)img * g.Ps;
-        typedef unsigned short us2 __attribute__((ext_vector_type(2)));
-        uint32_t sel[5], coef[5];
-        const int base = min((int)rx[dx0].ofs, srcPitch - 8);
-#pragma unroll
-        for (int k = 0; k < 5; ++k) {
-            const ResizeCoef c = rx[min(dx0 + k, dw - 1)];
-            const int o0 = (int)c.ofs - base, o1 = min((int)c.ofs + 1, sw - 1) - base;
-            sel[k] = (uint32_t)o0 | 0x0c00u | ((uint32_t)o1 << 16) | 0x0c000000u;
-            coef[k] = (uint32_t)(uint16_t)c.a0 | ((uint32_t)(uint16_t)c.a1 << 16);
-        }
-        struct Raw { uint32_t w[2]; };
-        auto load_row = [&](int r) -> Raw { Raw v; __builtin_memcpy(v.w, s + (size_t)r * srcPitch + base, 8); return v; };
-        auto hrow = [&](const Raw& v, uint32_t* h) {
-#pragma unroll
-            for (int k = 0; k < 5; ++k) {
-                const uint32_t pr = __builtin_amdgcn_perm(v.w[1], v.w[0], sel[k]);
-                us2 va, vb;
-                __builtin_memcpy(&va, &pr, 4); __builtin_memcpy(&vb, &coef[k], 4);
-                h[k] = __builtin_amdgcn_udot2(va, vb, 0u, false) >> 4;
-            }
-        };
-        auto rows_of = [&](int dy, int& r0, int& r1, uint32_t& b0, uint32_t& b1) {
-            const ResizeCoef cy = ry[min(dy, dh - 1)];
-            r0 = min(max((int)cy.ofs, 0), sh - 1); r1 = min(max((int)cy.ofs + 1, 0), sh - 1);
-            b0 = (uint32_t)cy.a0; b1 = (uint32_t)cy.a1;
-        };
-        int r0, r1, ra = -1, rb = -1;
-        uint32_t b0, b1;
-        rows_of(dy0, r0, r1, b0, b1);
-        Raw p0 = load_row(r0), p1 = load_row(r1);
-        uint32_t hA[5] = {0, 0, 0, 0, 0}, hB[5] = {0, 0, 0, 0, 0};
-        int prev[5] = {0, 0, 0, 0, 0};
-#pragma unroll
-        for (int rr = 0; rr <= UG_ROWS; ++rr) {
-            const int dy = dy0 + rr;
-            if (dy > dh || (rr > 0 && dy - 1 >= dh)) break;
-            int n0, n1;
-            uint32_t c0, c1;
-            rows_of(dy + 1, n0, n1, c0, c1);
-            Raw q0 = p0, q1 = p1;
-            if (rr < UG_ROWS) {
-                if (n0 != r0 && n0 != r1) q0 = load_row(n0);
-                if (n1 != n0 && n1 != r1) q1 = load_row(n1);
-                __builtin_amdgcn_sched_barrier(0);
-            }
-            uint32_t h0[5], h1[5];
-            if (r0 == ra) { for (int k = 0; k < 5; ++k) h0[k] = hA[k]; }
-            else if (r0 == rb) { for (int k = 0; k < 5; ++k) h0[k] = hB[k]; }
-            else hrow(p0, h0);
-            if (r1 == r0) { for (int k = 0; k < 5; ++k) h1[k] = h0[k]; }
-            else if (r1 == rb) { for (int k = 0; k < 5; ++k) h1[k] = hB[k]; }
-            else hrow(p1, h1);
-            int cur[5];
-#pragma unroll
-            for (int k = 0; k < 5; ++k) cur[k] = (int)(((((b0 * h0[k]) >> 16) + ((b1 * h1[k]) >> 16) + 2u) >> 2) & 0xffu);
-            if (writeScaled && rr < UG_ROWS && dy < dh) {
-                const uint32_t out = (uint32_t)cur[0] | ((uint32_t)cur[1] << 8) | ((uint32_t)cur[2] << 16) | ((uint32_t)cur[3] << 24);
-                __builtin_memcpy(d + (size_t)dy * g.pitchS, &out, 4);
-            }
-            if (rr > 0) {
-                const int y = dy - 1;
-                uint32_t packed[4];
-#pragma unroll
-                for (int k = 0; k < 4; ++k) {
-                    const int A = prev[k], B = prev[k + 1], Cc = cur[k], D = cur[k + 1];
-                    const int DA = D - A, BC = B - Cc;
-                    const int gx = DA + BC, gy = DA - BC;
-                    const int nn = gx * gx + gy * gy;
-                    const bool inside = dx0 + k < dw - 1 && y < dh - 1;
-                    packed[k] = inside ? (pack_g(gx, gy) | (nn >= g.nThr ? 0u : kNotDef)) : kNotDef;
-                    if (inside && nn >= g.nThr) nmax = max(nmax, nn);
-                }
-                uint32_t* o = gout + (size_t)y * dw + dx0;
-                const uintptr_t oa = reinterpret_cast<uintptr_t>(o);
-                if (dx0 + 3 < dw && (oa & 15) == 0) *reinterpret_cast<uint4*>(o) = make_uint4(packed[0], packed[1], packed[2], packed[3]);
-                else if (dx0 + 3 < dw && (oa & 7) == 0) {
-                    reinterpret_cast<uint2*>(o)[0] = make_uint2(packed[0], packed[1]); reinterpret_cast<uint2*>(o)[1] = make_uint2(packed[2], packed[3]);
-                } else {
-#pragma unroll
-                    for (int k = 0; k < 4; ++k) if (dx0 + k < dw) o[k] = packed[k];
-                }
-            }
-#pragma unroll
-            for (int k = 0; k < 5; ++k) prev[k] = cur[k];
-            ra = r0; rb = r1;
-#pragma unroll
-            for (int k = 0; k < 5; ++k) { hA[k] = h0[k]; hB[k] = h1[k]; }
-            r0 = n0; r1 = n1; b0 = c0; b1 = c1; p0 = q0; p1 = q1;
-        }
+        const bool edge = (int)blockIdx.x * 256 + 255 >= g.Ws - 1;
+        nmax = edge ? lsd_upgrad_strip<true>(s, d, gout, g.W, g.H, g.Ws, g.Hs, g.pitchW, g.pitchS, nThr, rx, ry, dx0, dy0, writeScaled)
+                    : lsd_upgrad_strip<false>(s, d, gout, g.W, g.H, g.Ws, g.Hs, g.pitchW, g.pitchS, nThr, rx, ry, dx0, dy0, writeScaled);
     }
 #pragma unroll
     for (int o = 32; o > 0; o >>= 1) nmax = max(nmax, __shfl_xor(nmax, o));
-    if (threadIdx.x == 0 && nmax > 0) atomicMax(&maxN[img * 32], nmax);
+    if (threadIdx.x == 0 && nmax > 0 && nmax >= nThr) atomicMax(&maxN[img * 32], nmax);
 }
 
 constexpr int KEYS_THREADS = 512;
@@ -259,49 +268,6 @@
     const double bin_coef = (max_grad > 0) ? (double)nBins1 / max_grad : 0;
     const float bin_coef_half_f = 0.5f * (float)bin_coef;
     constexpr int NB = 8;
-    constexpr bool SPLIT = ALLKEYS && !WIDE && CH == NB * KEYS_THREADS;
-    if (SPLIT) {
-        uint32_t* kall = keys + (size_t)img * Ps;
-        const int keyEnd = min(Ps, (Hs - 1) * Ws);
-        {
-            uint32_t p[NB];
-            float d[NB];
-#pragma unroll
-            for (int u = 0; u < NB; ++u) { const int idx = c0 + (int)threadIdx.x + u * KEYS_THREADS; p[u] = idx < Ps ? grad[idx] : kNotDef; }
-#pragma unroll
-            for (int u = 0; u < NB; ++u) d[u] = (p[u] & kNotDef) ? kNaN : angDeg[p[u] & 0x3fffffu];
-#pragma unroll
-            for (int u = 0; u < NB; ++u) s_deg[Ws + 1 + (int)threadIdx.x + u * KEYS_THREADS] = d[u];
-#pragma unroll
-            for (int u = 0; u < NB; ++u) {
-                const int idx = c0 + (int)threadIdx.x + u * KEYS_THREADS;
-                const int y = (int)(__umulhi((uint32_t)idx, divM) >> divS), x = idx - y * Ws;
-                const int gx = unpack_gx(p[u]), gy = unpack_gy(p[u]);
-                const int n = gx * gx + gy * gy;
-                const float tf = __builtin_amdgcn_sqrtf((float)n) * bin_coef_half_f;
-                int bin = (int)tf;
-                const float fr = tf - (float)bin;
-                const bool valid = (idx < keyEnd) & (x < Ws - 1);
-                if (valid & (n != 0) & ((fr < 1e-3f) | (fr > 0.999f))) bin = (int)(sqrt_quarter(n) * bin_coef);
-                if (valid) kall[(uint32_t)(idx - y)] = ((uint32_t)(nBins1 - bin) << 22) | (uint32_t)idx;
-            }
-        }
-#pragma unroll
-        for (int side = 0; side < 2; ++side) {
-            const int first = side ? c0 + CH : lo, qBase = side ? CH + Ws + 1 : 0;
-            constexpr int NH = 4;
-            for (int h0 = (int)threadIdx.x; h0 < Ws + 1; h0 += NH * KEYS_THREADS) {
-                uint32_t p[NH];
-                float d[NH];
-#pragma unroll
-                for (int u = 0; u < NH; ++u) { const int h = h0 + u * KEYS_THREADS, idx = first + h; p[u] = (h < Ws + 1) & ((unsigned)idx < (unsigned)Ps) ? grad[idx] : kNotDef; }
-#pragma unroll
-                for (int u = 0; u < NH; ++u) d[u] = (p[u] & kNotDef) ? kNaN : angDeg[p[u] & 0x3fffffu];
-#pragma unroll
-                for (int u = 0; u < NH; ++u) if (h0 + u * KEYS_THREADS < Ws + 1) s_deg[qBase + h0 + u * KEYS_THREADS] = d[u];
-            }
-        }
-    } else
     for (int i0 = lo + (int)threadIdx.x; i0 < hi; i0 += NB * KEYS_THREADS) {
         uint32_t p[NB];
         float d[NB];
@@ -406,6 +372,121 @@
                         else kout[t] = ((uint32_t)(nBins1 - bin) << 22) | (uint32_t)idx; }
     }
     if (!ALLKEYS && chunk == nChunks - 1 && threadIdx.x == 0) keyCount[img * 32] = s_base + n3;
+}
+
+constexpr int KT_W = 256, KT_H = 16, KT_SW = KT_W + 2, KT_RING = 2 * KT_SW + 2 * KT_H;
+template <bool OWNER>
+__global__ __launch_bounds__(KEYS_THREADS) void k_lsd_keys_tiled(uint32_t* __restrict__ gradAll, const LineGeom* __restrict__ gp, const int* __restrict__ maxN,
+                                                                 uint32_t* __restrict__ keys, uint32_t* __restrict__ owner, const float* __restrict__ angDeg,
+                                                                 int tilesX, int nTiles, int total)
+{
+    constexpr int NWV = KEYS_THREADS / 64, NB = 8;
+    static_assert(KT_W * KT_H == NB * KEYS_THREADS && KEYS_THREADS == 2 * KT_W && KT_W * KT_H <= 65536 && KT_RING <= 2 * KEYS_THREADS, "tile shape");
+    __shared__ float s_deg[(KT_H + 2) * KT_SW];
+    __shared__ uint16_t s_list[KT_W * KT_H];
+    __shared__ int s_wcnt[NWV];
+    const LineGeom& g = *gp;
+    const int lane = threadIdx.x & 63, wv = threadIdx.x >> 6;
+    const int L = blockIdx.x, per = total >> 3;
+    const int V = L < per * 8 ? (L & 7) * per + (L >> 3) : L;
+    const int img = V / nTiles, tile = V - img * nTiles;
+    const int tileY = tile / tilesX, x0 = (tile - tileY * tilesX) * KT_W, y0 = tileY * KT_H;
+    const int Ws = g.Ws, Hs = g.Hs, Ps = g.Ps, nBins1 = g.nBins - 1;
+    const float alignDeg = g.alignDeg;
+    const double precG = g.prec;
+    uint32_t* grad = gradAll + (size_t)img * Ps;
+    uint32_t* kall = keys + (size_t)img * Ps;
+    const float kNaN = __builtin_nanf("");
+    const double max_grad = sqrt((double)maxN[img * 32] / 4.0);
+    const double bin_coef = (max_grad > 0) ? (double)nBins1 / max_grad : 0;
+    const float bin_coef_half_f = 0.5f * (float)bin_coef;
+    const int tx = threadIdx.x & (KT_W - 1), X = x0 + tx;
+    const int th = __builtin_amdgcn_readfirstlane((int)(threadIdx.x >> 8));
+    unsigned long long defM[NB];
+    int wc = 0;
+    {
+        uint32_t p[NB];
+        float d[NB];
+#pragma unroll
+        for (int u = 0; u < NB; ++u) { const int Y = y0 + th + 2 * u; p[u] = ((X < Ws) & (Y < Hs)) ? grad[Y * Ws + X] : kNotDef; }
+#pragma unroll
+        for (int u = 0; u < NB; ++u) d[u] = (p[u] & kNotDef) ? kNaN : angDeg[p[u] & 0x3fffffu];
+#pragma unroll
+        for (int u = 0; u < NB; ++u) s_deg[(th + 2 * u + 1) * KT_SW + tx + 1] = d[u];
+#pragma unroll
+        for (int u = 0; u < NB; ++u) {
+            const int Y = y0 + th + 2 * u;
+            const int gx = unpack_gx(p[u]), gy = unpack_gy(p[u]);
+            const int n = gx * gx + gy * gy;
+            const float tf = __builtin_amdgcn_sqrtf((float)n) * bin_coef_half_f;
+            int bin = (int)tf;
+            const float fr = tf - (float)bin;
+            const bool valid = (X < Ws - 1) & (Y < Hs - 1);
+            if (valid & (n != 0) & ((fr < 1e-3f) | (fr > 0.999f))) bin = (int)(sqrt_quarter(n) * bin_coef);
+            if (valid) kall[Y * (Ws - 1) + X] = ((uint32_t)(nBins1 - bin) << 22) | (uint32_t)(Y * Ws + X);
+            defM[u] = wave_vote(d[u] == d[u]);
+            wc += __popcll(defM[u]);
+        }
+    }
+    if (lane == 0) s_wcnt[wv] = wc;
+    {
+        uint32_t p[2];
+        int at[2];
+#pragma unroll
+        for (int u = 0; u < 2; ++u) {
+            const int h = (int)threadIdx.x + u * KEYS_THREADS;
+            int ty, rx;
+            if (h < 2 * KT_SW) { const int below = h >= KT_SW; ty = below ? KT_H : -1; rx = h - (below ? KT_SW : 0) - 1; }
+            else { const int k = h - 2 * KT_SW; ty = k >> 1; rx = (k & 1) ? KT_W : -1; }
+            const int Xr = x0 + rx, Yr = y0 + ty;
+            at[u] = h < KT_RING ? (ty + 1) * KT_SW + rx + 1 : -1;
+            p[u] = ((h < KT_RING) & ((unsigned)Xr < (unsigned)Ws) & ((unsigned)Yr < (unsigned)Hs)) ? grad[Yr * Ws + Xr] : kNotDef;
+        }
+#pragma unroll
+        for (int u = 0; u < 2; ++u) if (at[u] >= 0) s_deg[at[u]] = (p[u] & kNotDef) ? kNaN : angDeg[p[u] & 0x3fffffu];
+    }
+    __syncthreads();
+    int n3 = 0, wbase = 0;
+#pragma unroll
+    for (int v = 0; v < NWV; ++v) { const int cv = s_wcnt[v]; if (v < wv) wbase += cv; n3 += cv; }
+#pragma unroll
+    for (int u = 0; u < NB; ++u) {
+        if (wave_bit(defM[u])) s_list[wbase + wave_rank_below(defM[u])] = (uint16_t)(((th + 2 * u) << 8) | tx);
+        wbase += __popcll(defM[u]);
+    }
+    __syncthreads();
+    for (int t = threadIdx.x; t < n3; t += KEYS_THREADS) {
+        const int li = s_list[t], ty = li >> 8, lx = li & (KT_W - 1);
+        const int idx = (y0 + ty) * Ws + x0 + lx;
+        const float* sd = s_deg + (ty + 1) * KT_SW + lx + 1;
+        const float deg0 = sd[0];
+        float dmax = -1.f, margin = 1.0f;
+#pragma unroll
+        for (int q = 0; q < 9; ++q) {
+            if (q == 4) continue;
+            const float dn = sd[((q / 3) - 1) * KT_SW + (q % 3) - 1];
+            const float dd = f_sub(fabsf(f_sub(fabsf(f_sub(deg0, dn)), 180.f)), alignDeg);
+            dmax = fmaxf(dmax, dd);
+            margin = fminf(margin, fabsf(dd));
+        }
+        bool iso = !(dmax >= 0.f);
+        if (margin < 1e-3f || alignDeg < 0.f) {
+            const double a0 = d_mul((double)deg0, kDegToRads);
+            iso = true;
+#pragma unroll
+            for (int q = 0; q < 9; ++q) {
+                if (q == 4) continue;
+                const float dn = sd[((q / 3) - 1) * KT_SW + (q % 3) - 1];
+                if (dn != dn) continue;
+                double n_theta = d_sub(a0, d_mul((double)dn, kDegToRads));
+                if (n_theta < 0) n_theta = -n_theta;
+                if (n_theta > kM32PI) { n_theta = d_sub(n_theta, kM2PI); if (n_theta < 0) n_theta = -n_theta; }
+                if (n_theta <= precG) iso = false;
+            }
+        }
+        if (iso) grad[idx] = grad[idx] | kIso;
+        if (OWNER) owner[(size_t)img * Ps + idx] = 0xffffffffu;
+    }
 }
 
 
@@ -1556,6 +1637,7 @@
     p.resize = (g.resizeTiled & 4) && g.seedOrder == 1 ? LsdPlan::Upgrad : g.resizeTiled ? LsdPlan::Tiled : LsdPlan::Upsample;
     p.sort = g.wide ? LsdPlan::Wide : g.seedOrder == 1 ? LsdPlan::Seed : LsdPlan::Radix;
     p.keysAll = g.seedOrder == 1;
+    p.keysTiled = p.keysAll && !g.wide && !o.keysGeneral;
 
     const int m = o.sortMode;
     p.sortWaves = m < 0 ? (n <= 256 ? 8 : n <= 640 ? 4 : n <= 1536 ? 2 : 1) : m == 2 ? 8 : m == 1 ? 4 : m == 5 ? 2 : 1;
@@ -1608,14 +1690,20 @@
     }
     if (p.resize != LsdPlan::Upgrad) hipLaunchKernelGGL(k_lsd_grad, dim3((g.Ps + LG_CHUNK - 1) / LG_CHUNK, n_images), dim3(256), 0, s, b.scaled, b.grad, b.geom, b.maxN, b.chunkCnt);
     {
-        const int nChunks = (g.Ps + LG_CHUNK - 1) / LG_CHUNK, total = nChunks * n_images;
-        const size_t lds = (size_t)(LG_CHUNK + 2 * g.Ws + 2) * sizeof(float);
-        if (lds > 60 * 1024) { set_error("LSD image wider than the key kernel's LDS window"); return OLF_ERR_CAPACITY; }
-        const auto keys = p.sort == LsdPlan::Wide ? (p.keysAll ? k_lsd_keys<false, true, LG_CHUNK, true> : k_lsd_keys<false, false, LG_CHUNK, true>)
-                        : p.keysAll ? (p.keysOwner ? k_lsd_keys<true, true, LG_CHUNK> : k_lsd_keys<false, true, LG_CHUNK>)
-                        : p.keysOwner ? k_lsd_keys<true, false, LG_CHUNK> : k_lsd_keys<false, false, LG_CHUNK>;
-        hipLaunchKernelGGL(keys, dim3(total), dim3(KEYS_THREADS), lds, s, b.grad, b.geom, b.maxN, b.chunkCnt, p.sort == LsdPlan::Radix ? b.keysB : b.keysA, b.keyCount,
-                           b.owner, b.angDeg, nChunks, total);
+        if (p.keysTiled) {
+            const int tilesX = (g.Ws + KT_W - 1) / KT_W, nTiles = tilesX * ((g.Hs + KT_H - 1) / KT_H), total = nTiles * n_images;
+            hipLaunchKernelGGL(p.keysOwner ? k_lsd_keys_tiled<true> : k_lsd_keys_tiled<false>, dim3(total), dim3(KEYS_THREADS), 0, s, b.grad, b.geom, b.maxN, b.keysA, b.owner,
+                               b.angDeg, tilesX, nTiles, total);
+        } else {
+            const int nChunks = (g.Ps + LG_CHUNK - 1) / LG_CHUNK, total = nChunks * n_images;
+            const size_t lds = (size_t)(LG_CHUNK + 2 * g.Ws + 2) * sizeof(float);
+            if (lds > 60 * 1024) { set_error("LSD image wider than the key kernel's LDS window"); return OLF_ERR_CAPACITY; }
+            const auto keys = p.sort == LsdPlan::Wide ? (p.keysAll ? k_lsd_keys<false, true, LG_CHUNK, true> : k_lsd_keys<false, false, LG_CHUNK, true>)
+                            : p.keysAll ? (p.keysOwner ? k_lsd_keys<true, true, LG_CHUNK> : k_lsd_keys<false, true, LG_CHUNK>)
+                            : p.keysOwner ? k_lsd_keys<true, false, LG_CHUNK> : k_lsd_keys<false, false, LG_CHUNK>;
+            hipLaunchKernelGGL(keys, dim3(total), dim3(KEYS_THREADS), lds, s, b.grad, b.geom, b.maxN, b.chunkCnt, p.sort == LsdPlan::Radix ? b.keysB : b.keysA, b.keyCount,
+                               b.owner, b.angDeg, nChunks, total);
+        }
     }
     OLF_HIP_CHECK(hipGetLastError());
     return OLF_OK;
diff --git a/orb_line_slam_amd/csrc/resize_strip.hpp b/orb_line_slam_amd/csrc/resize_strip.hpp
--- /dev/null
+++ b/orb_line_slam_amd/csrc/resize_strip.hpp
@@ -0,0 +1,60 @@
+#pragma once
+#include <cstdint>
+#include <hip/hip_runtime.h>
+#include "olf_internal.hpp"
+
+namespace olf {
+
+constexpr int RS_ROWS = 16;
+constexpr int UG_ROWS = 16;
+
+struct ResizeRaw { uint32_t w[2]; };
+template <int NC>
+__device__ __forceinline__ void resize_hrow(const ResizeRaw& v, const uint32_t* sel, const uint32_t* coef, uint32_t* h)
+{
+    typedef unsigned short us2 __attribute__((ext_vector_type(2)));
+    uint32_t pr[NC];
+#pragma unroll
+    for (int k = 0; k < NC; ++k) pr[k] = __builtin_amdgcn_perm(v.w[1], v.w[0], sel[k]);
+    __builtin_amdgcn_sched_barrier(0);
+#pragma unroll
+    for (int k = 0; k < NC; ++k) {
+        us2 va, vb;
+        __builtin_memcpy(&va, &pr[k], 4); __builtin_memcpy(&vb, &coef[k], 4);
+        pr[k] = __builtin_amdgcn_udot2(va, vb, 0u, false);
+    }
+    __builtin_amdgcn_sched_barrier(0);
+#pragma unroll
+    for (int k = 0; k < NC; ++k) h[k] = pr[k] & 0xfffff0u;
+}
+
+struct ResizeRowCoef { int ofs; uint32_t b0s, b1s; };
+__device__ __forceinline__ ResizeRowCoef resize_row_coef(const ResizeCoef* tab, int i)
+{
+    static_assert(sizeof(ResizeCoef) == 8, "ResizeCoef is read as one 64-bit word");
+    typedef const __attribute__((address_space(4))) uint8_t* cbytes;
+    const uint64_t w = *reinterpret_cast<const __attribute__((address_space(4))) uint64_t*>((cbytes)tab + (uint32_t)i * 8u);
+    const uint32_t w0 = (uint32_t)w, w1 = (uint32_t)(w >> 32);
+    ResizeRowCoef c;
+    c.ofs = (int)(int16_t)(uint16_t)w0;
+    c.b0s = (w0 >> 16) << 12;
+    c.b1s = (w1 & 0xffffu) << 12;
+    return c;
+}
+
+__device__ __forceinline__ uint32_t resize_mulhi24(uint32_t bs, uint32_t h)
+{
+    uint32_t r;
+    asm("v_mul_hi_u32_u24 %0, %1, %2" : "=v"(r) : "s"(bs), "v"(h));
+    return r;
+}
+__device__ __forceinline__ uint32_t resize_vblend(uint32_t b0s, uint32_t h0, uint32_t b1s, uint32_t h1)
+{
+    return (resize_mulhi24(b0s, h0) + resize_mulhi24(b1s, h1) + 2u) >> 2;
+}
+__device__ __forceinline__ uint32_t resize_pack4(uint32_t v0, uint32_t v1, uint32_t v2, uint32_t v3)
+{
+    return __builtin_amdgcn_perm(v1, v0, 0x0c0c0400u) | __builtin_amdgcn_perm(v3, v2, 0x04000c0cu);
+}
+
+}
```

After: 15450 stereo frames/s (median of 5 runs). 2.1% higher.
